# keonlee9420/Comprehensive-Transformer-TTS

Measured on AMD Instinct MI355X. Metric: mel-frames/sec (train step) LJSpeech batch=16, 1/2/4/8 MI355X, higher is better.
Workload: dtype f32; 1 GPU; LJSpeech transformer_fs2 batch=16/GPU seq<=128->mel<=1024x80; full train step fwd+loss+bwd+clip+Adam, dropout on; workload_detail=supervised durations (BASELINE configs[1]), global_batch=16, valid_frames_per_gpu=11992, padded_frames_per_gpu=16384, launch_mode=hipgraph(fwd+bwd | clip+adam), parallelism=dp1

## Files before the change

comprehensive-transformer-tts_amd/_lib.py:

```python
import ctypes as C
import os

_HERE = os.path.dirname(os.path.abspath(__file__))
LIB_PATH = os.environ.get("CTTS_LIB") or os.path.join(_HERE, "csrc", "libctts_hip.so")

_c_f32p = C.c_void_p
_i32, _i64, _f32, _u32, _vp = C.c_int32, C.c_int64, C.c_float, C.c_uint32, C.c_void_p


class GemmDesc(C.Structure):
    _fields_ = [
        ("A", _vp), ("B", _vp), ("C", _vp),
        ("M", _i32), ("N", _i32), ("K", _i32),
        ("lda", _i64), ("ldb", _i64), ("ldc", _i64),
        ("a_kc", _i32), ("b_kc", _i32),
        ("nb0", _i32), ("nb1", _i32),
        ("sA0", _i64), ("sA1", _i64), ("sB0", _i64), ("sB1", _i64), ("sC0", _i64), ("sC1", _i64),
        ("lens", _vp),
        ("lim_m", _i32), ("lim_n", _i32), ("lim_k", _i32),
        ("conv_T", _i32), ("conv_pad", _i32), ("conv_cin", _i32), ("conv_on_b", _i32),
        ("split_k", _i32),
        ("alpha", _f32),
        ("bias", _vp),
        ("Z", _vp), ("ldz", _i64),
        ("act", _i32),
        ("p_drop", _f32), ("seed", _vp), ("drop_offset", _u32),
        ("R", _vp), ("ldr", _i64),
        ("rowscale", _vp),
        ("row_lens", _vp), ("row_T", _i32), ("row_halo", _i32),
        ("tile_map", _vp),
        ("tile_group_n", _i32),
        ("E", _vp), ("rowsub", _vp),
        ("sk_ws", _vp), ("sk_ws_bytes", _i64),
        ("epi_bwd", _i32),
        ("split_out", _vp), ("split_out_floats", _i64),
        ("split_overwrite", _i32),
        ("bf16_split", _i32),
        ("A_planes", _vp),
        ("B_planes", _vp),
        ("C_planes", _vp),
    ]


class GemmRouteInfo(C.Structure):
    _fields_ = [("kind", _i32), ("tile_m", _i32), ("tile_n", _i32), ("split_k", _i32), ("k_granule", _i32)]


GEMM_KINDS = ("none", "planes", "planes_wgrad", "weight_stationary", "x6", "stream_k", "x6tn", "scalar64", "buf128", "buf_k2", "buf_narrow",
              "buf64", "vec128", "vec64")


class VconvDesc(C.Structure):
    _fields_ = [
        ("x", _vp), ("sxb", _i64), ("sxt", _i64), ("sxc", _i64),
        ("B", _i32), ("T", _i32), ("Cin", _i32), ("Cout", _i32), ("k", _i32), ("dil", _i32),
        ("transposed_u", _i32),
        ("act_in", _i32), ("slope", _f32),
        ("w", _vp), ("w_planes", _vp),
        ("bias", _vp),
        ("R", _vp),
        ("out", _vp),
        ("alpha", _f32), ("beta", _f32),
        ("bf16_split", _i32),
        ("lens", _vp), ("len_mul", _i32),
    ]


class VconvHDesc(C.Structure):
    _fields_ = [
        ("x", _vp), ("sxb", _i64), ("sxt", _i64), ("sxc", _i64),
        ("x_f32", _i32),
        ("B", _i32), ("T", _i32), ("Cin", _i32), ("Cout", _i32), ("k", _i32), ("dil", _i32),
        ("transposed_u", _i32),
        ("act_in", _i32), ("slope", _f32),
        ("w", _vp),
        ("bias", _vp),
        ("R", _vp),
        ("out", _vp),
        ("alpha", _f32), ("beta", _f32),
        ("lens", _vp), ("len_mul", _i32),
    ]


class PsumTask(C.Structure):
    _fields_ = [("src", _vp), ("dst", _vp), ("n", _i64), ("stride", _i64), ("count", _i32), ("alpha", _f32)]


class SplitTask(C.Structure):
    _fields_ = [("src", _vp), ("dst", _vp), ("rows", _i64), ("cols", _i64), ("ld", _i64)]


class RepackTask(C.Structure):
    _fields_ = [("src", _vp), ("dst", _vp), ("cout", _i32), ("cin", _i32), ("k", _i32)]


_SIGNATURES = {
    "ctts_conv_dgrad_weights": [C.POINTER(RepackTask), C.c_int, _vp],
    "ctts_gemm_split_plan": [C.POINTER(GemmDesc), C.POINTER(_i32), C.POINTER(_i64)],
    "ctts_gemm_route": [C.POINTER(GemmDesc), C.POINTER(GemmRouteInfo)],
    "ctts_partial_sums": [C.POINTER(PsumTask), C.c_int, _vp],
    "ctts_reduce_parts": [C.c_int, _i64, C.c_int],
    "ctts_xcd_probe": [_vp, C.c_int, _vp],
    "ctts_posembed_fwd": [_vp, _vp, _vp, _vp, _vp, _vp, _i64, C.c_int, _f32, _vp, _u32, _vp],
    "ctts_posembed_bwd": [_vp, _vp, _vp, _vp, _vp, _vp, _i64, C.c_int, _f32, _vp, _u32, C.c_int, _vp, _vp],
    "ctts_gemm": [C.POINTER(GemmDesc), _vp],
    "ctts_gemm_takes_persistent": [C.POINTER(GemmDesc)],
    "ctts_gemm_ws_enable": [C.c_int],
    "ctts_gemm_takes_weight_stationary": [C.POINTER(GemmDesc)],
    "ctts_gemm_takes_bf16_split": [C.POINTER(GemmDesc)],
    "ctts_gemm_takes_planes": [C.POINTER(GemmDesc)],
    "ctts_split_planes": [C.POINTER(SplitTask), C.c_int, _vp],
    "ctts_rowdot_heads": [_vp, _vp, _vp, C.c_int, C.c_int, C.c_int, C.c_int, _vp],
    "ctts_mel_prepare": [_vp, C.c_int, C.c_int, _vp, _vp],
    "ctts_mel_spectrogram": [_vp, _vp, _vp, _vp, _vp, _vp, _vp, _i64, C.c_int, C.c_int, C.c_int, C.c_int, C.c_int, _f32, C.c_int, _vp, _vp],
    "ctts_mha_fwd": [_vp, _vp, _vp, _vp, C.c_int, C.c_int, C.c_int, C.c_int, _f32, _vp],
    "ctts_mha_bwd": [_vp, _vp, _vp, _vp, _vp, _vp, _vp, _vp, _vp, C.c_int, C.c_int, C.c_int, C.c_int, _f32, C.c_int, _vp, _vp],
    "ctts_relmha_fwd": [_vp, _vp, _vp, _vp, _vp, _vp, C.c_int, C.c_int, C.c_int, C.c_int, _f32, _f32, _vp, _u32, _vp],
    "ctts_relmha_bwd": [_vp, _vp, _vp, _vp, _vp, _vp, _vp, _vp, _vp, _vp, _vp, _vp, _vp, C.c_int, C.c_int, C.c_int, C.c_int,
                        _f32, _f32, _vp, _u32, _vp],
    "ctts_weighted_colsum": [_vp, _vp, _vp, _i64, C.c_int, _f32, C.c_int, _vp, _vp, _vp],
    "ctts_epilogue_bwd": [_vp, _vp, _vp, _vp, _vp, _vp, _i64, C.c_int, C.c_int, _f32, _vp, _u32, _f32, C.c_int, _vp, _vp, _vp],
    "ctts_row_tile_map": [_vp, C.c_int, C.c_int, C.c_int, _vp, _vp],
    "ctts_conv_weight_repack": [_vp, _vp, C.c_int, C.c_int, C.c_int, C.c_int, _vp],
    "ctts_lr_index": [_vp, C.c_int, C.c_int, _vp, C.c_int, C.c_int, C.c_int, _vp, _vp, _vp, _vp],
    "ctts_lr_gather_fwd": [_vp, _vp, _vp, C.c_int, C.c_int, C.c_int, C.c_int, _vp],
    "ctts_lr_gather_bwd": [_vp, _vp, _vp, C.c_int, C.c_int, C.c_int, C.c_int, _vp],
    "ctts_embedding_fwd": [_vp, _vp, _vp, _i64, C.c_int, C.c_int, _vp],
    "ctts_embedding_bwd": [_vp, _vp, _vp, _i64, C.c_int, C.c_int, C.c_int, C.c_int, _vp, _vp],
    "ctts_positions": [_vp, C.c_int, _i64, C.c_int, C.c_int, _vp, _vp],
    "ctts_cwt_pitch": [_vp, _i64, C.c_int, _vp, _vp, _f32, _vp, C.c_int, _f32, _f32, _f32, C.c_int, _vp, _vp, _vp, C.c_int, C.c_int, C.c_int, _vp],
    "ctts_layernorm_fwd": [_vp, _vp, _vp, _vp, _vp, _vp, C.c_int, C.c_int, _f32, _f32, _vp, _u32, _vp, _vp, _vp],
    "ctts_layernorm_bwd": [_vp, _vp, _vp, _vp, _vp, _vp, _vp, _vp, C.c_int, C.c_int, _f32, _vp, _u32, _vp, C.c_int, _vp, _vp, _vp, _vp],
    "ctts_colstats": [_vp, _vp, C.c_int, C.c_int, _vp, _vp],
    "ctts_bn_finalize": [_vp, C.c_int, C.c_int, _f32, _f32, _vp, _vp, _vp, _vp, _vp, _vp],
    "ctts_bn_apply": [_vp, _vp, _vp, _vp, _vp, _vp, C.c_int, C.c_int, C.c_int, _f32, _vp, _u32, _vp, _vp],
    "ctts_bn_bwd_reduce": [_vp, _vp, _vp, _vp, _vp, _vp, _vp, C.c_int, C.c_int, C.c_int, _f32, _vp, _u32, _vp, _vp],
    "ctts_bn_bwd_apply": [_vp, _vp, _vp, _vp, _vp, _vp, _vp, _vp, _vp, _vp, C.c_int, C.c_int, C.c_int, _f32, _vp,
                          _u32, C.c_int, _vp, _vp],
    "ctts_softmax_fwd": [_vp, _vp, C.c_int, C.c_int, C.c_int, _i64, _vp],
    "ctts_softmax_bwd": [_vp, _vp, _vp, C.c_int, C.c_int, C.c_int, _i64, _vp],
    "ctts_act_dropout_bwd": [_vp, _vp, _vp, _i64, C.c_int, C.c_int, _f32, _f32, _vp, _u32, _vp],
    "ctts_rowscale_dropout": [_vp, _vp, _i64, C.c_int, _vp, _f32, _vp, _u32, _vp],
    "ctts_colsum": [_vp, _vp, _i64, C.c_int, _i64, _f32, C.c_int, _vp, _vp, _vp],
    "ctts_reflect_pad": [_vp, _vp, C.c_int, C.c_int, C.c_int, _i64, _vp],
    "ctts_stft_magnitude": [_vp, _i64, _vp, _i64, _vp, _i64, C.c_int, _vp],
    "ctts_log_clamp_transpose": [_vp, _vp, C.c_int, C.c_int, C.c_int, _f32, _vp],
    "ctts_relattn_split_fwd": [_vp, _vp, _vp, _vp, _vp, _vp, _i64, C.c_int, _vp],
    "ctts_relattn_split_bwd": [_vp, _vp, _vp, _vp, _i64, C.c_int, _vp],
    "ctts_glu_fwd": [_vp, _vp, _i64, C.c_int, _vp],
    "ctts_glu_bwd": [_vp, _vp, _vp, _i64, C.c_int, _vp],
    "ctts_dwconv_fwd": [_vp, _vp, _vp, C.c_int, C.c_int, C.c_int, C.c_int, C.c_int, _vp],
    "ctts_dwconv_wgrad": [_vp, _vp, _vp, _vp, C.c_int, C.c_int, C.c_int, C.c_int, C.c_int, _vp],
    "ctts_relpos_softmax_fwd": [_vp, _vp, _vp, C.c_int, C.c_int, _f32, _f32, _vp, _u32, _vp],
    "ctts_relpos_softmax_bwd": [_vp, _vp, C.c_int, C.c_int, _f32, _f32, _vp, _u32, _vp],
    "ctts_relshift_bwd": [_vp, _vp, C.c_int, C.c_int, _vp],
    "ctts_neg_sqdist": [_vp, _vp, _vp, C.c_int, C.c_int, C.c_int, C.c_int, _f32, _vp],
    "ctts_mas": [_vp, _vp, _vp, _vp, _vp, _vp, C.c_int, C.c_int, C.c_int, _vp],
    "ctts_forward_sum_fwd": [_vp, _vp, _vp, _f32, _vp, _vp, _vp, C.c_int, C.c_int, C.c_int, _vp],
    "ctts_forward_sum_bwd": [_vp, _vp, _vp, _f32, _vp, _vp, _vp, _vp, _vp, C.c_int, C.c_int, C.c_int, _vp],
    "ctts_var_loss_fwd": [_vp] * 2 + [C.c_int] + [_vp] * 12 + [C.c_int] * 3 + [_vp, C.c_int, _vp] + [_vp] * 4 + [_vp],
    "ctts_var_loss_bwd": [_vp] * 2 + [C.c_int] + [_vp] * 12 + [C.c_int] * 3 + [_vp, C.c_int, _vp] + [_vp] * 4 + [_vp] * 5 + [_vp],
    "ctts_bin_loss_fwd": [_vp, _vp, _i64, _vp, _vp, _vp],
    "ctts_bin_loss_bwd": [_vp, _vp, _vp, _vp, _vp, _i64, _vp],
    "ctts_masked_loss_fwd": [_vp, _vp, _vp, _i64, _i32, _vp, _vp, _vp],
    "ctts_masked_loss_bwd": [_vp, _vp, _vp, _vp, _vp, _vp, _i64, _i32, _vp],
    "ctts_mel_l1_fwd": [_vp, _vp, _vp, _vp, _vp, _vp, _i64, C.c_int, _vp, _vp],
    "ctts_mel_l1_bwd": [_vp, _vp, _vp, _vp, _vp, _vp, _vp, _vp, _i64, C.c_int, _vp],
    "ctts_adam_clip_step": [_vp, _vp, _vp, _vp, C.c_int64, _vp, _f32, _f32, _f32, _f32, _f32, _vp, _vp],
    "ctts_im2col_3x3s2": [_vp, _vp, C.c_int, C.c_int, C.c_int, C.c_int, _vp],
    "ctts_col2im_3x3s2": [_vp, _vp, C.c_int, C.c_int, C.c_int, C.c_int, _vp],
    "ctts_gru_fwd": [_vp, _vp, _vp, _vp, _vp, C.c_int, C.c_int, C.c_int, C.c_int, C.c_int, _vp],
    "ctts_gru_bwd": [_vp, _vp, _vp, _vp, _vp, _vp, _vp, C.c_int, C.c_int, C.c_int, C.c_int, C.c_int, _vp],
    "ctts_softmax_rect_fwd": [_vp, _vp, _vp, C.c_int, C.c_int, C.c_int, _vp],
    "ctts_softmax_rect_bwd": [_vp, _vp, _vp, _vp, C.c_int, C.c_int, C.c_int, _vp],
    "ctts_vocoder_conv": [C.POINTER(VconvDesc), _vp],
    "ctts_vocoder_post": [_vp, C.c_int, C.c_int, C.c_int, C.c_int, _vp, _vp, _f32, _vp, _vp],
    "ctts_vocoder_post_ragged": [_vp, C.c_int, C.c_int, C.c_int, C.c_int, _vp, _vp, _f32, _vp, _vp, C.c_int, _vp],
    "ctts_vocoder_conv_h": [C.POINTER(VconvHDesc), _vp],
    "ctts_vocoder_post_h": [_vp, C.c_int, C.c_int, C.c_int, C.c_int, _vp, _vp, _f32, _vp, _vp, C.c_int, _vp],
    "ctts_fastformer_pool_fwd": [_vp, _i64, _vp, _i64, _vp, _vp, _vp, _vp, C.c_int, C.c_int, C.c_int, C.c_int, _f32, _vp],
    "ctts_fastformer_pool_bwd": [_vp, _vp, _vp, _vp, _i64, _vp, _i64, _vp, _vp, _vp, _vp, C.c_int, C.c_int, C.c_int, C.c_int, _f32, _vp],
    "ctts_fastformer_bcast": [_vp, _i64, _vp, _vp, C.c_int, C.c_int, C.c_int, _vp],
    "ctts_fastformer_bcast_bwd": [_vp, _vp, _vp, _i64, _vp, _vp, _vp, _vp, _vp, C.c_int, C.c_int, C.c_int, _vp],
    "ctts_fastformer_resdrop": [_vp, _vp, _vp, _vp, _i64, C.c_int, _vp, _f32, _vp, _u32, C.c_int, _vp],
    "ctts_griffinlim_prepare": [_vp, C.c_int, C.c_int, _vp, _vp],
    "ctts_stft_transform": [_vp, _vp, _vp, _vp, _vp, _i64, _i64, _i64, C.c_int, C.c_int, C.c_int, C.c_int, _vp],
    "ctts_istft_frames": [_vp, _vp, _i64, _i64, _i64, _vp, _vp, _vp, _vp, C.c_int, C.c_int, C.c_int, C.c_int, _vp],
    "ctts_griffinlim_iter": [_vp, _vp, _vp, _vp, _vp, C.c_int, C.c_int, C.c_int, C.c_int, _vp],
    "ctts_istft_ola": [_vp, _vp, _vp, _vp, _i64, C.c_int, C.c_int, C.c_int, C.c_int, _vp],
    "ctts_griffinlim_iter_momentum": [_vp, _vp, _vp, _vp, _vp, _vp, _f32, C.c_int, C.c_int, C.c_int, C.c_int, C.c_int, _vp],
    "ctts_istft_frames_seeded": [_vp, _i64, _i64, _i64, _vp, _vp, _vp, _vp, _vp, C.c_int, C.c_int, C.c_int, C.c_int, _vp],
    "ctts_pitch_track_prepare": [_vp, _vp],
    "ctts_pitch_track": [_vp, _vp, _vp, _vp, _vp, _vp, C.c_int, C.c_int, C.c_int, C.c_int, _f32, _f32, _f32, _f32, _vp],
    "ctts_f0_targets": [_vp, _vp, _vp, _vp, _vp, _vp, _vp, C.c_int, C.c_int, _vp],
    "ctts_norm_interp_f0": [_vp, _vp, _vp, _vp, C.c_int, C.c_int, _f32, _vp],
    "ctts_trim_silence": [_vp, _vp, _vp, _vp, _vp, C.c_int, C.c_int, _f32, C.c_int, C.c_int, _vp],
    "ctts_attn_prior": [_vp, _vp, _vp, C.c_int, C.c_int, C.c_int, _i64, _i64, _f32, _vp],
    "ctts_outlier_stats": [_vp, _vp, _vp, _vp, _vp, _vp, _vp, _vp, C.c_int, C.c_int, _vp],
    "ctts_mel_cepstrum": [_vp, _vp, _vp, C.c_int, C.c_int, C.c_int, C.c_int, _vp],
    "ctts_dtw": [_vp, _vp, _vp, _vp, _vp, _vp, _vp, _vp, C.c_int, C.c_int, C.c_int, C.c_int, C.c_int, _vp],
    "ctts_path_metrics": [_vp, _vp, _vp, _vp, _vp, C.c_int, C.c_int, C.c_int, C.c_int, _vp],
    "ctts_resample": [_vp, _vp, _vp, _vp, _vp, C.c_int, C.c_int, C.c_int, C.c_int, C.c_int, C.c_int, _vp],
    "ctts_peak_normalize": [_vp, _vp, _vp, _vp, _vp, _vp, C.c_int, C.c_int, _f32, _vp],
    "ctts_resample_tile": [C.c_int, C.c_int, C.c_int, C.c_int],
    "ctts_loudness_chunk": [],
    "ctts_loudness_tile_slots": [],
    "ctts_loudness_coef_doubles": [],
    "ctts_loudness_max_segments": [],
    "ctts_kweight_energy": [_vp, _vp, _vp, _vp, _vp, _vp, _vp, C.c_int, C.c_int, C.c_int, C.c_int, _vp, _vp],
    "ctts_loudness_gate": [_vp, _vp, _vp, _vp, _vp, _vp, _vp, _vp, _vp, _vp, _vp, C.c_int, C.c_int, C.c_int, C.c_int, C.c_int, C.c_double,
                           C.c_double, C.c_int, _vp],
    "ctts_apply_gain": [_vp, _vp, _vp, _vp, C.c_int, C.c_int, _vp],
    "ctts_stoi_max_frames": [],
    "ctts_stoi": [_vp, _vp, _vp, _vp, _vp, _vp, _vp, C.c_int, C.c_int, _vp, _vp],
    "ctts_si_sdr": [_vp, _vp, _vp, _vp, C.c_int, C.c_int, _vp, _vp],
    "ctts_mr_stft": [_vp, _vp, _vp, _vp, _vp, _vp, C.c_int, C.c_int, C.c_int, C.c_int, C.c_int, _vp, _vp],
    "ctts_comm_unique_id": [_vp],
    "ctts_comm_create": [C.POINTER(_vp), _i32, _i32, _vp],
    "ctts_comm_destroy": [_vp],
    "ctts_allreduce_mean": [_vp, _i64, _vp, _vp],
}
COMM_ID_BYTES = 128
EXPORTED_SYMBOLS = sorted(list(_SIGNATURES) + ["ctts_last_error", "ctts_version", "ctts_mha_supported", "ctts_relmha_workspace_floats",
                                               "ctts_mel_spectrogram_workspace_bytes", "ctts_gemm_workspace_bytes", "ctts_workspace_bytes",
                                               "ctts_workspace_error_word", "ctts_fastformer_workspace_floats",
                                               "ctts_griffinlim_workspace_bytes", "ctts_griffinlim_state_floats",
                                               "ctts_pitch_track_workspace_bytes", "ctts_trim_silence_workspace_bytes",
                                               "ctts_dtw_workspace_bytes", "ctts_loudness_workspace_bytes", "ctts_stoi_workspace_bytes",
                                               "ctts_si_sdr_workspace_bytes", "ctts_mr_stft_workspace_bytes"])
ADAM_STATE_FLOATS = 3 + 2048
ABI_VERSION = 2

_lib = None


class CttsError(RuntimeError):
    pass


def load():
    global _lib
    if _lib is not None:
        return _lib
    if not os.path.exists(LIB_PATH):
        raise CttsError(
            f"{LIB_PATH} not found - build it with comprehensive-transformer-tts_amd/csrc/build.sh "
            "(or __graft_entry__.build()).  There is no CPU / PyTorch fallback for the hot path."
        )
    lib = C.CDLL(LIB_PATH)
    lib.ctts_version.restype = C.c_int
    lib.ctts_version.argtypes = []
    if lib.ctts_version() != ABI_VERSION:
        raise CttsError(f"{LIB_PATH} has ABI version {lib.ctts_version()}, this package needs {ABI_VERSION} - rebuild it with "
                        "comprehensive-transformer-tts_amd/csrc/build.sh (or __graft_entry__.build())")
    for name, argtypes in _SIGNATURES.items():
        fn = getattr(lib, name)
        fn.argtypes = argtypes
        fn.restype = C.c_int
# ... 43 lines not shown
```

comprehensive-transformer-tts_amd/csrc/elementwise.hip:

```cpp
#include "ctts_common.h"

namespace {
__global__ void zero_u32_kernel(uint32_t* __restrict__ p, size_t n) {
  for (size_t i = (size_t)blockIdx.x * blockDim.x + threadIdx.x; i < n; i += (size_t)gridDim.x * blockDim.x) p[i] = 0u;
}
}

int ctts_zero_async(void* p, size_t bytes, hipStream_t st) {
  if (bytes == 0) return 0;
  const size_t n = (bytes + 3) / 4;
  const unsigned blocks = (unsigned)((n + 255) / 256 > 2048 ? 2048 : (n + 255) / 256);
  hipLaunchKernelGGL(zero_u32_kernel, dim3(blocks), dim3(256), 0, st, (uint32_t*)p, n);
  return hipGetLastError() == hipSuccess ? 0 : -1;
}

namespace {

__global__ void act_dropout_bwd_kernel(const float* __restrict__ dg, const float* __restrict__ z, float* __restrict__ dz,
                                       long total, int act, float p_drop, const uint64_t* seed, uint32_t drop_offset) {
  const bool do_drop = p_drop > 0.f;
  uint32_t dkey = 0; float inv_keep = 1.f;
  if (do_drop) { dkey = ctts_drop_key(seed, drop_offset); inv_keep = 1.f / (1.f - p_drop); }
  if (total & 3) {
    for (long i = (long)blockIdx.x * blockDim.x + threadIdx.x; i < total; i += (long)gridDim.x * blockDim.x) {
      float g = dg[i];
      if (do_drop) g *= ctts_drop_scale(dkey, (uint32_t)i, p_drop, inv_keep);
      dz[i] = g * ctts_act_grad(z[i], act);
    }
    return;
  }
  const long n4 = total >> 2;
  for (long i = (long)blockIdx.x * blockDim.x + threadIdx.x; i < n4; i += (long)gridDim.x * blockDim.x) {
    const float4 g = reinterpret_cast<const float4*>(dg)[i];
    const float4 zz = reinterpret_cast<const float4*>(z)[i];
    float ga[4] = {g.x, g.y, g.z, g.w};
    const float za[4] = {zz.x, zz.y, zz.z, zz.w};
#pragma unroll
    for (int e = 0; e < 4; ++e) {
      if (do_drop) ga[e] *= ctts_drop_scale(dkey, (uint32_t)(i * 4 + e), p_drop, inv_keep);
      ga[e] *= ctts_act_grad(za[e], act);
    }
    reinterpret_cast<float4*>(dz)[i] = make_float4(ga[0], ga[1], ga[2], ga[3]);
  }
}

__global__ void rowscale_dropout_kernel(const float* __restrict__ x, float* __restrict__ y, long total, int C,
                                        const float* __restrict__ rowscale, float p_drop, const uint64_t* seed,
                                        uint32_t drop_offset) {
  const bool do_drop = p_drop > 0.f;
  uint32_t dkey = 0; float inv_keep = 1.f;
  if (do_drop) { dkey = ctts_drop_key(seed, drop_offset); inv_keep = 1.f / (1.f - p_drop); }
  if (C & 3) {
    for (long i = (long)blockIdx.x * blockDim.x + threadIdx.x; i < total; i += (long)gridDim.x * blockDim.x) {
      float a = x[i];
      if (do_drop) a *= ctts_drop_scale(dkey, (uint32_t)i, p_drop, inv_keep);
      y[i] = a * (rowscale ? rowscale[i / C] : 1.f);
    }
    return;
  }
  const long n4 = total >> 2;
  const int C4 = C >> 2;
  for (long i = (long)blockIdx.x * blockDim.x + threadIdx.x; i < n4; i += (long)gridDim.x * blockDim.x) {
    const float4 v = reinterpret_cast<const float4*>(x)[i];
    float a[4] = {v.x, v.y, v.z, v.w};
    const float sc = rowscale ? rowscale[i / C4] : 1.f;
#pragma unroll
    for (int e = 0; e < 4; ++e) {
      if (do_drop) a[e] *= ctts_drop_scale(dkey, (uint32_t)(i * 4 + e), p_drop, inv_keep);
      a[e] *= sc;
    }
    reinterpret_cast<float4*>(y)[i] = make_float4(a[0], a[1], a[2], a[3]);
  }
}

__device__ __forceinline__ void ctts_colsum_emit(float tot, float* s64, float* __restrict__ out, int c, int C, int creal, float scale,
                                                 int accumulate) {
  const int ty = threadIdx.x >> 6, l = threadIdx.x & 63;
  if (C != creal) {
    __syncthreads();
    if (ty == 0) s64[l] = c < C ? tot : 0.f;
    __syncthreads();
    if (ty == 0 && l < creal) {
      float a = 0.f;
      for (int j = l; j < C; j += creal) a += s64[j];
      out[l] = accumulate ? out[l] + scale * a : scale * a;
    }
    return;
  }
  if (ty == 0 && c < C) out[c] = accumulate ? out[c] + scale * tot : scale * tot;
}

__global__ __launch_bounds__(256) void colsum_kernel(const float* __restrict__ x, float* __restrict__ out, long rows, int C,
                                                      int creal, long ld, float scale, unsigned char* ws, int G, int accumulate,
                                                      float* __restrict__ parts) {
  __shared__ float s[4][64];
  const int c = blockIdx.x * 64 + (threadIdx.x & 63), ty = threadIdx.x >> 6;
  const long stripe = (rows + gridDim.y - 1) / gridDim.y;
  const long r0 = blockIdx.y * stripe, r1 = min(rows, r0 + stripe);
  float a = 0.f;
  if (c < C) {
#pragma unroll 4
    for (long r = r0 + ty; r < r1; r += 4) a += x[r * ld + c];
  }
  s[ty][threadIdx.x & 63] = a;
  __syncthreads();
  float tot[1] = {0.f};
  if (ty == 0) { const int l = threadIdx.x; tot[0] = s[0][l] + s[1][l] + s[2][l] + s[3][l]; }
  if (parts) {
    if (ty == 0 && c < C) parts[(long)blockIdx.y * C + c] = tot[0];
    return;
  }
  if (!ctts_ordered_colsum<float, 1>(tot, ws, blockIdx.x, blockIdx.y, gridDim.y, G)) return;
  ctts_colsum_emit(tot[0], s[0], out, c, C, creal, scale, accumulate);
}

__global__ __launch_bounds__(256) void epilogue_bwd_kernel(const float* __restrict__ dy, const float* __restrict__ rowscale,
                                                            const float* __restrict__ z, float* __restrict__ dz, float* __restrict__ gm,
                                                            float* __restrict__ dbias, long rows, int C, int act, float p_drop,
                                                            const uint64_t* seed, uint32_t drop_offset, float bias_scale,
                                                            unsigned char* ws, int G, int accumulate, float* __restrict__ parts) {
  __shared__ float s[4][64];
  const int c = blockIdx.x * 64 + (threadIdx.x & 63), ty = threadIdx.x >> 6;
  const long stripe = (rows + gridDim.y - 1) / gridDim.y;
  const long r0 = blockIdx.y * stripe, r1 = min(rows, r0 + stripe);
  const bool do_drop = p_drop > 0.f;
  uint32_t dkey = 0; float inv_keep = 1.f;
  if (do_drop) { dkey = ctts_drop_key(seed, drop_offset); inv_keep = 1.f / (1.f - p_drop); }
  float a = 0.f;
  if (c < C) {
#pragma unroll 4
    for (long r = r0 + ty; r < r1; r += 4) {
      const long e = r * C + c;
      float g = dy[e];
      if (rowscale) g *= rowscale[r];
      if (gm) gm[e] = g;
      if (do_drop) g *= ctts_drop_scale(dkey, (uint32_t)e, p_drop, inv_keep);
      if (z) g *= ctts_act_grad(z[e], act);
      dz[e] = g;
      a += g;
    }
  }
  if (!dbias && !parts) return;
  s[ty][threadIdx.x & 63] = a;
  __syncthreads();
  float tot[1] = {0.f};
  if (ty == 0) { const int l = threadIdx.x; tot[0] = s[0][l] + s[1][l] + s[2][l] + s[3][l]; }
  if (parts) {
    if (ty == 0 && c < C) parts[(long)blockIdx.y * C + c] = tot[0];
    return;
  }
  if (!ctts_ordered_colsum<float, 1>(tot, ws, blockIdx.x, blockIdx.y, gridDim.y, G)) return;
  ctts_colsum_emit(tot[0], s[0], dbias, c, C, C, bias_scale, accumulate);
}

__global__ void conv_weight_repack_kernel(const float* __restrict__ src, float* __restrict__ dst, int cout, int cin, int k,
                                          int mode, long total) {
  for (long e = (long)blockIdx.x * blockDim.x + threadIdx.x; e < total; e += (long)gridDim.x * blockDim.x) {
    if (mode == 0) {
      const int ci = (int)(e % cin); const long t = e / cin; const int kk = (int)(t % k); const int co = (int)(t / k);
      dst[e] = src[((long)co * cin + ci) * k + kk];
    } else if (mode == 1) {
      const int co = (int)(e % cout); const long t = e / cout; const int kk = (int)(t % k); const int ci = (int)(t / k);
      dst[e] = src[((long)co * cin + ci) * k + (k - 1 - kk)];
    } else if (mode == 4) {
      const int co = (int)(e % cout); const long t = e / cout; const int kk = (int)(t % k); const int ci = (int)(t / k);
      dst[e] = src[((long)co * k + (k - 1 - kk)) * cin + ci];
    } else {
      const int kk = (int)(e % k); const long t = e / k; const int ci = (int)(t % cin); const int co = (int)(t / cin);
      const float v = src[((long)co * k + kk) * cin + ci];
      dst[e] = mode == 3 ? dst[e] + v : v;
    }
  }
}

__global__ void reflect_pad_kernel(const float* __restrict__ y, float* __restrict__ ypad, int N, int pad, long ld_out,
                                   long total) {
  const int W = N + 2 * pad;
  for (long e = (long)blockIdx.x * blockDim.x + threadIdx.x; e < total; e += (long)gridDim.x * blockDim.x) {
    const long b = e / ld_out;
    const int j = (int)(e - b * ld_out);
    float v = 0.f;
    if (j < W) {
      int i = j - pad;
      if (i < 0) i = -i;
      if (i >= N) i = 2 * (N - 1) - i;
      v = y[b * N + i];
    }
    ypad[e] = v;
  }
}

__global__ __launch_bounds__(256) void stft_magnitude_kernel(const float* __restrict__ reim, long ld_reim,
                                                              float* __restrict__ mag, long ld_mag,
                                                              float* __restrict__ energy, long frames, int nbins) {
  const int lane = threadIdx.x & 63, wave = threadIdx.x >> 6;
  for (long f = (long)blockIdx.x * 4 + wave; f < frames; f += (long)gridDim.x * 4) {
    const float* r = reim + f * ld_reim;
    float acc = 0.f;
    for (int k = lane; k < ld_mag; k += 64) {
      float m = 0.f;
      if (k < nbins) {
        const float re = r[k], im = r[nbins + k];
        const float p = re * re + im * im;
        acc += p;
        m = sqrtf(p);
      }
      mag[f * ld_mag + k] = m;
    }
    acc = ctts_wave_sum(acc);
    if (lane == 0) energy[f] = sqrtf(acc);
  }
}

__global__ void log_clamp_transpose_kernel(const float* __restrict__ in, float* __restrict__ out, int F, int n_mel,
                                           float clip, long total) {
  for (long e = (long)blockIdx.x * blockDim.x + threadIdx.x; e < total; e += (long)gridDim.x * blockDim.x) {
    const int f = (int)(e % F); const long t = e / F; const int m = (int)(t % n_mel); const long b = t / n_mel;
    out[e] = logf(fmaxf(in[(b * F + f) * n_mel + m], clip));
  }
}

inline int grid_for(long n, int cap = 4096) { return (int)min((n + 255) / 256, (long)cap); }

}

extern "C" int ctts_act_dropout_bwd(const float* dg, const float* z, float* dz, int64_t rows, int C, int act,
                                    float alpha_unused, float p_drop, const uint64_t* seed, uint32_t drop_offset,
                                    void* stream) {
  (void)alpha_unused;
  CTTS_REQUIRE(dg && z && dz && C > 0, "ctts_act_dropout_bwd: bad arguments");
  const long total = (long)rows * C;
  if (total == 0) return 0;
  hipLaunchKernelGGL(act_dropout_bwd_kernel, dim3(grid_for((total & 3) ? total : (total >> 2))), dim3(256), 0, (hipStream_t)stream, dg, z, dz, total,
                     act, p_drop, seed, drop_offset);
  CTTS_CHECK_LAUNCH("ctts_act_dropout_bwd");
  return 0;
}

extern "C" int ctts_rowscale_dropout(const float* x, float* y, int64_t rows, int C, const float* rowscale, float p_drop,
                                     const uint64_t* seed, uint32_t drop_offset, void* stream) {
  CTTS_REQUIRE(x && y && C > 0, "ctts_rowscale_dropout: bad arguments");
  const long total = (long)rows * C;
  if (total == 0) return 0;
  hipLaunchKernelGGL(rowscale_dropout_kernel, dim3(grid_for((C & 3) ? total : (total >> 2))), dim3(256), 0, (hipStream_t)stream, x, y, total, C,
                     rowscale, p_drop, seed, drop_offset);
  CTTS_CHECK_LAUNCH("ctts_rowscale_dropout");
  return 0;
}

namespace {
__global__ __launch_bounds__(256) void weighted_colsum_kernel(const float* __restrict__ x, const float* __restrict__ w,
                                                               float* __restrict__ out, long rows, int C, float scale,
                                                               unsigned char* ws, int G, int accumulate, float* __restrict__ parts) {
  __shared__ float s[4][64];
  const int c = blockIdx.x * 64 + (threadIdx.x & 63), ty = threadIdx.x >> 6;
  const long stripe = (rows + gridDim.y - 1) / gridDim.y;
  const long r0 = blockIdx.y * stripe, r1 = min(rows, r0 + stripe);
  float a = 0.f;
  if (c < C) {
#pragma unroll 4
    for (long r = r0 + ty; r < r1; r += 4) a = fmaf(w[r], x[r * C + c], a);
  }
  s[ty][threadIdx.x & 63] = a;
  __syncthreads();
  float tot[1] = {0.f};
  if (ty == 0) { const int l = threadIdx.x; tot[0] = s[0][l] + s[1][l] + s[2][l] + s[3][l]; }
  if (parts) {
    if (ty == 0 && c < C) parts[(long)blockIdx.y * C + c] = tot[0];
    return;
  }
  if (!ctts_ordered_colsum<float, 1>(tot, ws, blockIdx.x, blockIdx.y, gridDim.y, G)) return;
  ctts_colsum_emit(tot[0], s[0], out, c, C, C, scale, accumulate);
}
}

static int colsum_stripes(int gx, long want, bool have_ws) {
  if (!have_ws) return 1;
  const long cap = (long)(CTTS_WS_RED_P1_BYTES / (64 * sizeof(float))) / gx;
  return (int)max((long)1, min(want, min(cap, (long)CTTS_RED_MAX_GROUPS * 64)));
}

int ctts_layernorm_bwd_blocks(int rows, int C);

extern "C" int ctts_reduce_parts(int kind, int64_t rows, int C) {
  if (rows <= 0 || C <= 0) return 0;
  const int gx = (C + 63) / 64;
  if (gx > CTTS_RED_MAX_COLBLOCKS) return 0;
  switch (kind) {
    case 0: if (C * 2 <= 64 && rows % 2 == 0) return 0;
            return colsum_stripes(gx, min((long)max(1, 1024 / gx), (long)rows / 64), true);
    case 1: return colsum_stripes(gx, min((long)max(1, 1024 / gx), (long)rows / 64), true);
    case 2: return colsum_stripes(gx, min((long)max(1, 2048 / gx), (long)rows / 32), true);
    case 3: return ctts_layernorm_bwd_blocks((int)rows, C);
    default: return 0;
  }
}

extern "C" int ctts_weighted_colsum(const float* x, const float* w, float* out, int64_t rows, int C, float scale, int accumulate,
                                    void* ws, float* parts, void* stream) {
  CTTS_REQUIRE(x && w && (out || parts) && C > 0 && (C + 63) / 64 <= CTTS_RED_MAX_COLBLOCKS, "ctts_weighted_colsum: bad arguments");
  CTTS_REQUIRE(!parts || rows > 0, "ctts_weighted_colsum: deferred mode needs rows > 0");
  hipStream_t st = (hipStream_t)stream;
  if (rows == 0) {
    if (!accumulate && ctts_zero_async(out, sizeof(float) * C, st) != 0) { ctts_set_error("ctts_weighted_colsum: zero fill failed"); return -2; }
    return 0;
  }
  const int gx = (C + 63) / 64;
  const int gy = colsum_stripes(gx, min((long)max(1, 1024 / gx), (long)rows / 64), ws != nullptr || parts != nullptr);
  hipLaunchKernelGGL(weighted_colsum_kernel, dim3(gx, gy), dim3(256), 0, st, x, w, out, (long)rows, C, scale, (unsigned char*)ws,
                     ctts_red_group(gy), accumulate, parts);
  CTTS_CHECK_LAUNCH("ctts_weighted_colsum");
  return 0;
}

extern "C" int ctts_colsum(const float* x, float* out, int64_t rows, int C, int64_t ld, float scale, int accumulate, void* ws,
                           float* parts, void* stream) {
  CTTS_REQUIRE(x && (out || parts) && C > 0 && (C + 63) / 64 <= CTTS_RED_MAX_COLBLOCKS, "ctts_colsum: bad arguments");
  CTTS_REQUIRE(!parts || ctts_reduce_parts(0, rows, C) > 0, "ctts_colsum: this shape has no deferred mode (ctts_reduce_parts = 0)");
  hipStream_t st = (hipStream_t)stream;
  if (rows == 0) {
    if (!accumulate && ctts_zero_async(out, sizeof(float) * C, st) != 0) { ctts_set_error("ctts_colsum: zero fill failed"); return -2; }
    return 0;
  }
  int k = 1;
  if (ld == C && !parts)
    while (C * k * 2 <= 64 && rows % (k * 2) == 0) k *= 2;
  const int Cv = C * k, gx = (Cv + 63) / 64;
  const long Rv = rows / k;
  const int gy = colsum_stripes(gx, min((long)max(1, 1024 / gx), Rv / 64), ws != nullptr || parts != nullptr);
  hipLaunchKernelGGL(colsum_kernel, dim3(gx, gy), dim3(256), 0, st, x, out, Rv, Cv, C, (long)ld * k, scale, (unsigned char*)ws,
                     ctts_red_group(gy), accumulate, parts);
  CTTS_CHECK_LAUNCH("ctts_colsum");
  return 0;
}

extern "C" int ctts_epilogue_bwd(const float* dy, const float* rowscale, const float* z, float* dz, float* gm, float* dbias,
                                 int64_t rows, int C, int act, float p_drop, const uint64_t* seed, uint32_t drop_offset, float bias_scale,
                                 int accumulate_bias, void* ws, float* parts, void* stream) {
  CTTS_REQUIRE(dy && dz && rows >= 0 && C > 0 && p_drop >= 0.f && p_drop < 1.f && (p_drop == 0.f || seed), "ctts_epilogue_bwd: bad arguments");
  CTTS_REQUIRE(!dbias || (C + 63) / 64 <= CTTS_RED_MAX_COLBLOCKS, "ctts_epilogue_bwd: C too large for the bias-gradient reduction");
  hipStream_t st = (hipStream_t)stream;
  if (rows == 0) {
    if (dbias && !accumulate_bias && ctts_zero_async(dbias, sizeof(float) * C, st) != 0) { ctts_set_error("ctts_epilogue_bwd: zero fill failed"); return -2; }
    return 0;
  }
  const int gx = (C + 63) / 64;
  const long want = min((long)max(1, 2048 / gx), (long)rows / 32);
  CTTS_REQUIRE(!parts || rows > 0, "ctts_epilogue_bwd: deferred bias gradient needs rows > 0");
  const int gy = (dbias || parts) ? colsum_stripes(gx, want, ws != nullptr || parts != nullptr) : (int)max((long)1, want);
  hipLaunchKernelGGL(epilogue_bwd_kernel, dim3(gx, gy), dim3(256), 0, st, dy, rowscale, act ? z : nullptr, dz, gm, dbias, (long)rows, C, act,
                     p_drop, seed, drop_offset, bias_scale, (unsigned char*)ws, ctts_red_group(gy), accumulate_bias, parts);
  CTTS_CHECK_LAUNCH("ctts_epilogue_bwd");
  return 0;
}

extern "C" int ctts_conv_weight_repack(const float* src, float* dst, int cout, int cin, int k, int mode, void* stream) {
  CTTS_REQUIRE(src && dst && mode >= 0 && mode <= 4, "ctts_conv_weight_repack: bad arguments");
  const long total = (long)cout * cin * k;
  if (total == 0) return 0;
  hipLaunchKernelGGL(conv_weight_repack_kernel, dim3(grid_for(total)), dim3(256), 0, (hipStream_t)stream, src, dst, cout, cin, k,
                     mode, total);
  CTTS_CHECK_LAUNCH("ctts_conv_weight_repack");
  return 0;
}

extern "C" int ctts_reflect_pad(const float* y, float* ypad, int B, int N, int pad, int64_t ld_out, void* stream) {
  CTTS_REQUIRE(y && ypad && N > pad && ld_out >= N + 2 * pad, "ctts_reflect_pad: need N > pad and ld_out >= N + 2*pad");
  const long total = (long)B * ld_out;
  if (total == 0) return 0;
  hipLaunchKernelGGL(reflect_pad_kernel, dim3(grid_for(total)), dim3(256), 0, (hipStream_t)stream, y, ypad, N, pad, (long)ld_out, total);
  CTTS_CHECK_LAUNCH("ctts_reflect_pad");
  return 0;
}

extern "C" int ctts_stft_magnitude(const float* reim, int64_t ld_reim, float* mag, int64_t ld_mag, float* energy,
                                   int64_t frames, int nbins, void* stream) {
  CTTS_REQUIRE(reim && mag && energy && ld_mag >= nbins, "ctts_stft_magnitude: bad arguments");
  if (frames == 0) return 0;
  const int blocks = (int)min((frames + 3) / 4, (int64_t)4096);
  hipLaunchKernelGGL(stft_magnitude_kernel, dim3(blocks), dim3(256), 0, (hipStream_t)stream, reim, (long)ld_reim, mag,
                     (long)ld_mag, energy, (long)frames, nbins);
  CTTS_CHECK_LAUNCH("ctts_stft_magnitude");
  return 0;
}

extern "C" int ctts_log_clamp_transpose(const float* mel_fm, float* out, int B, int F, int n_mel, float clip, void* stream) {
  CTTS_REQUIRE(mel_fm && out, "ctts_log_clamp_transpose: null pointer");
  const long total = (long)B * F * n_mel;
  if (total == 0) return 0;
  hipLaunchKernelGGL(log_clamp_transpose_kernel, dim3(grid_for(total)), dim3(256), 0, (hipStream_t)stream, mel_fm, out, F, n_mel,
                     clip, total);
  CTTS_CHECK_LAUNCH("ctts_log_clamp_transpose");
  return 0;
}


namespace {
constexpr int RPK_BATCH = 32;
struct RepackBatch {
  const float* src[RPK_BATCH];
  float* dst[RPK_BATCH];
  int cout[RPK_BATCH], cin[RPK_BATCH], k[RPK_BATCH];
  int first_block[RPK_BATCH + 1];
  int ntasks;
};

__global__ __launch_bounds__(256) void conv_dgrad_weights_kernel(const RepackBatch b) {
  __shared__ float tile[32][33];
  int t = 0;
  while (t + 1 < b.ntasks && (int)blockIdx.x >= b.first_block[t + 1]) ++t;
  const float* __restrict__ src = b.src[t];
  float* __restrict__ dst = b.dst[t];
  const int cout = b.cout[t], cin = b.cin[t], k = b.k[t];
  const int tco = (cout + 31) / 32, tci = (cin + 31) / 32;
  int blk = (int)blockIdx.x - b.first_block[t];
  const int kk = blk / (tco * tci);
  blk -= kk * tco * tci;
  const int co0 = (blk / tci) * 32, ci0 = (blk % tci) * 32;
  const int tx = threadIdx.x & 31, ty = threadIdx.x >> 5;
#pragma unroll
  for (int r = ty; r < 32; r += 8) {
    const int co = co0 + r, ci = ci0 + tx;
    tile[r][tx] = (co < cout && ci < cin) ? src[((long)co * k + (k - 1 - kk)) * cin + ci] : 0.f;
  }
  __syncthreads();
#pragma unroll
  for (int r = ty; r < 32; r += 8) {
    const int ci = ci0 + r, co = co0 + tx;
    if (ci < cin && co < cout) dst[((long)ci * k + kk) * cout + co] = tile[tx][r];
  }
}
}

extern "C" int ctts_conv_dgrad_weights(const ctts_repack_task* tasks, int ntasks, void* stream) {
  CTTS_REQUIRE(ntasks >= 0 && (tasks || ntasks == 0), "ctts_conv_dgrad_weights: bad arguments");
  hipStream_t st = (hipStream_t)stream;
  for (int t0 = 0; t0 < ntasks; t0 += RPK_BATCH) {
    RepackBatch b;
    b.ntasks = 0;
    int blocks = 0;
    for (int t = t0; t < ntasks && t < t0 + RPK_BATCH; ++t) {
      const ctts_repack_task& q = tasks[t];
      CTTS_REQUIRE(q.src && q.dst && q.cout > 0 && q.cin > 0 && q.k > 0, "ctts_conv_dgrad_weights: bad task %d", t);
      const int i = b.ntasks++;
      b.src[i] = q.src; b.dst[i] = q.dst; b.cout[i] = q.cout; b.cin[i] = q.cin; b.k[i] = q.k;
      b.first_block[i] = blocks;
      blocks += ((q.cout + 31) / 32) * ((q.cin + 31) / 32) * q.k;
    }
    if (b.ntasks == 0) continue;
    b.first_block[b.ntasks] = blocks;
    hipLaunchKernelGGL(conv_dgrad_weights_kernel, dim3(blocks), dim3(256), 0, st, b);
    CTTS_CHECK_LAUNCH("ctts_conv_dgrad_weights");
  }
  return 0;
}

namespace {
__global__ __launch_bounds__(256) void posembed_fwd_kernel(const float4* __restrict__ x, const int32_t* __restrict__ pos, const float4* __restrict__ table,
                                                            const float* __restrict__ alpha, const float* __restrict__ rowscale, float4* __restrict__ y,
                                                            long n4, int C4, float p_drop, const uint64_t* seed, uint32_t drop_offset) {
#pragma clang fp contract(off)
  const bool do_drop = p_drop > 0.f;
  uint32_t dkey = 0; float inv_keep = 1.f;
  if (do_drop) { dkey = ctts_drop_key(seed, drop_offset); inv_keep = 1.f / (1.f - p_drop); }
  const float a = alpha ? alpha[0] : 1.f;
  for (long i = (long)blockIdx.x * blockDim.x + threadIdx.x; i < n4; i += (long)gridDim.x * blockDim.x) {
    const long row = i / C4;
    const int c = (int)(i - row * C4);
    const float4 xv = x[i], tv = table[(long)pos[row] * C4 + c];
    float v[4] = {xv.x + a * tv.x, xv.y + a * tv.y, xv.z + a * tv.z, xv.w + a * tv.w};
    const float sc = rowscale ? rowscale[row] : 1.f;
#pragma unroll
    for (int e = 0; e < 4; ++e) {
      if (do_drop) v[e] *= ctts_drop_scale(dkey, (uint32_t)(i * 4 + e), p_drop, inv_keep);
      v[e] *= sc;
    }
    y[i] = make_float4(v[0], v[1], v[2], v[3]);
  }
}

__global__ __launch_bounds__(256) void posembed_bwd_kernel(const float4* __restrict__ dy, const int32_t* __restrict__ pos, const float4* __restrict__ table,
                                                            const float* __restrict__ rowscale, float4* __restrict__ dx, float* __restrict__ dalpha,
                                                            long n4, int C4, float p_drop, const uint64_t* seed, uint32_t drop_offset,
                                                            unsigned char* ws, int G, int accumulate) {
  __shared__ float s_w[4];
  const bool do_drop = p_drop > 0.f;
  uint32_t dkey = 0; float inv_keep = 1.f;
  if (do_drop) { dkey = ctts_drop_key(seed, drop_offset); inv_keep = 1.f / (1.f - p_drop); }
// ... 139 lines not shown
```

comprehensive-transformer-tts_amd/csrc/gemm.hip:

```cpp
#include "ctts_common.h"
#include "gemm_common.h"
#include <stdlib.h>
#include <type_traits>

namespace {

#ifndef CTTS_BK
#define CTTS_BK 32
#endif
#ifndef CTTS_GEMM_WAVES
#define CTTS_GEMM_WAVES 2
#endif
constexpr int BK = CTTS_BK;
constexpr int KC_LD = BK + 4;
constexpr int KCH = BK / 4;
static_assert(BK == 32 || BK == 64, "BK must be 32 or 64");


__device__ __forceinline__ bool rows_in_padding(const int32_t* row_lens, int row_T, int row_halo, int first, int last) {
  const int b0 = first / row_T;
  return b0 == last / row_T && (first - b0 * row_T) >= row_lens[b0] + row_halo;
}

__device__ __forceinline__ void batch_limits(const ctts_gemm_desc& d, int z0, bool apply, int& Mv, int& Nv, int& Kv) {
  Mv = d.M; Nv = d.N; Kv = d.K;
  if (apply && d.lens) {
    const int L = d.lens[z0];
    if (d.lim_m) Mv = min(Mv, L);
    if (d.lim_n) Nv = min(Nv, L);
    if (d.lim_k) Kv = min(Kv, L);
  }
}

__device__ __forceinline__ bool split_k_range(const ctts_gemm_desc& d, int Kv, int granule, int split, int& k_begin, int& k_end) {
  k_begin = 0; k_end = Kv;
  if (d.split_k > 1) {
    const GemmSplitRange s = gemm_split_range(Kv, d.split_k, granule, split);
    k_begin = s.k_begin; k_end = s.k_end;
    if (k_begin >= k_end) return false;
  }
  return true;
}

__device__ __forceinline__ void xcd_tile_order(int nwg, int tiles_n, bool scramble, int& wg, int& tm) {
  const int q8 = nwg >> 3, r8 = nwg & 7, xcd = blockIdx.x & 7, slot = blockIdx.x >> 3;
  wg = (xcd < r8 ? xcd * (q8 + 1) : r8 * (q8 + 1) + (xcd - r8) * q8) + slot;
  const int tiles_m = nwg / tiles_n;
  tm = wg / tiles_n;
  if (scramble) {
    const int P = (tiles_m % 37) ? 37 : ((tiles_m % 41) ? 41 : 43);
    tm = (int)(((long)tm * P) % tiles_m);
  }
}

__device__ __forceinline__ bool natural_order(const ctts_gemm_desc& d) { return d.tile_map == reinterpret_cast<const int32_t*>(1); }

__device__ __forceinline__ void zero_tile(const ctts_gemm_desc& d, float* C, int row0, int col0, int nrows, int ncols) {
  for (int e = threadIdx.x; e < nrows * ncols; e += 256) {
    const int r = e / ncols, c = e - r * ncols;
    C[(long)(row0 + r) * d.ldc + col0 + c] = 0.f;
    if (d.Z && !d.epi_bwd) d.Z[(long)(row0 + r) * d.ldz + col0 + c] = 0.f;
  }
}

__device__ __forceinline__ bool padded_tile_zeroed(const ctts_gemm_desc& d, float* C, int row0, int col0, int BM, int ncols, int Mv) {
  const int last = min(row0 + BM, Mv) - 1;
  if (!rows_in_padding(d.row_lens, d.row_T, d.row_halo, row0, last)) return false;
  zero_tile(d, C, row0, col0, last - row0 + 1, ncols);
  return true;
}

__device__ __forceinline__ void zero_outside_limits(const ctts_gemm_desc& d, float* C, int row0, int col0, int BM, int BN, int Mv, int Nv,
                                                    bool whole) {
  const int nrows = min(BM, d.M - row0), ncols = min(BN, d.N - col0);
  for (int e = threadIdx.x; e < nrows * ncols; e += 256) {
    const int r = e / ncols, c = e - r * ncols;
    if (whole || row0 + r >= Mv || col0 + c >= Nv) C[(long)(row0 + r) * d.ldc + col0 + c] = 0.f;
  }
}

struct ConvView {
  int T, pad, cin;
};

template <int ROWS, bool CONV>
struct LoaderKC {
  static constexpr int NV = ROWS * BK / 4 / 256;
  const float* base;
  long ld;
  int row0, row_lim, kq, tid;
  ConvView cv;
  int trow[NV];
  __device__ __forceinline__ void init(const float* p, long ld_, int row0_, int row_lim_, ConvView cv_, int tid_) {
    base = CONV ? p - (long)cv_.pad * cv_.cin : p;
    ld = ld_; row0 = row0_; row_lim = row_lim_; cv = cv_; tid = tid_;
    kq = (tid % KCH) << 2;
    if (CONV) {
#pragma unroll
      for (int i = 0; i < NV; ++i) {
        int gr = row0 + ((tid + i * 256) / KCH);
        trow[i] = gr % cv.T;
      }
    }
  }
  __device__ __forceinline__ void load(int k0, int k_end, float4 (&r)[NV]) const {
    const int gk = k0 + kq;
#pragma unroll
    for (int i = 0; i < NV; ++i) {
      const int gr = row0 + ((tid + i * 256) / KCH);
      float4 v = make_float4(0.f, 0.f, 0.f, 0.f);
      if (gr < row_lim && gk < k_end) {
        const float* p = base + (long)gr * ld + gk;
        float e[4] = {0.f, 0.f, 0.f, 0.f};
#pragma unroll
        for (int q = 0; q < 4; ++q) {
          bool okq = (gk + q < k_end);
          if (CONV && okq) { int tt = trow[i] + (gk + q) / cv.cin - cv.pad; okq = (tt >= 0) && (tt < cv.T); }
          if (okq) e[q] = p[q];
        }
        v = make_float4(e[0], e[1], e[2], e[3]);
      }
      r[i] = v;
    }
  }
  __device__ __forceinline__ void store(float* s, const float4 (&r)[NV]) const {
#pragma unroll
    for (int i = 0; i < NV; ++i) {
      const int row = (tid + i * 256) / KCH;
      *reinterpret_cast<float4*>(s + row * KC_LD + kq) = r[i];
    }
  }
};

template <int COLS, bool CONV>
struct LoaderRC {
  static constexpr int NV = COLS * BK / 4 / 256;
  static constexpr int LD = COLS + 4;
  const float* base;
  long ld;
  int col0, col_lim, tid;
  ConvView cv;
  __device__ __forceinline__ void init(const float* p, long ld_, int col0_, int col_lim_, ConvView cv_, int tid_) {
    base = CONV ? p - (long)cv_.pad * cv_.cin : p;
    ld = ld_; col0 = col0_; col_lim = col_lim_; cv = cv_; tid = tid_;
  }
  __device__ __forceinline__ void load(int k0, int k_end, float4 (&r)[NV]) const {
#pragma unroll
    for (int i = 0; i < NV; ++i) {
      const int f = tid + i * 256;
      const int k = f / (COLS / 4);
      const int cq = (f % (COLS / 4)) << 2;
      const int gk = k0 + k, gc = col0 + cq;
      float4 v = make_float4(0.f, 0.f, 0.f, 0.f);
      if (gk < k_end && gc < col_lim) {
        const float* p = base + (long)gk * ld + gc;
        int trow = 0;
        if (CONV) trow = gk % cv.T;
        float e[4] = {0.f, 0.f, 0.f, 0.f};
#pragma unroll
        for (int q = 0; q < 4; ++q) {
          bool okq = (gc + q < col_lim);
          if (CONV && okq) { int tt = trow + (gc + q) / cv.cin - cv.pad; okq = (tt >= 0) && (tt < cv.T); }
          if (okq) e[q] = p[q];
        }
        v = make_float4(e[0], e[1], e[2], e[3]);
      }
      r[i] = v;
    }
  }
  __device__ __forceinline__ void store(float* s, const float4 (&r)[NV]) const {
#pragma unroll
    for (int i = 0; i < NV; ++i) {
      const int f = tid + i * 256;
      const int k = f / (COLS / 4);
      const int cq = (f % (COLS / 4)) << 2;
      *reinterpret_cast<float4*>(s + k * LD + cq) = r[i];
    }
  }
};


__device__ __forceinline__ float4 mask4(float4 v, int nv) {
  v.x = nv > 0 ? v.x : 0.f; v.y = nv > 1 ? v.y : 0.f; v.z = nv > 2 ? v.z : 0.f; v.w = nv > 3 ? v.w : 0.f;
  return v;
}

template <int ROWS, bool CONV>
struct VLoaderKC {
  static constexpr int NV = ROWS * BK / 4 / 256;
  const float* base; const float* safe;
  long ld;
  int row0, row_lim, kq, tid;
  ConvView cv;
  int trow[NV];
  int nval[NV];
  __device__ __forceinline__ void init(const float* p, long ld_, int row0_, int row_lim_, ConvView cv_, int tid_) {
    safe = p;
    base = CONV ? p - (long)cv_.pad * cv_.cin : p;
// ... 62 lines not shown
    }
  }
  __device__ __forceinline__ void store(float* s, const float4 (&r)[NV]) const {
#pragma unroll
    for (int i = 0; i < NV; ++i) {
      const int f = tid + i * 256;
      const int k = f / (COLS / 4);
      const int cq = (f % (COLS / 4)) << 2;
      *reinterpret_cast<float4*>(s + k * LD + cq) = mask4(r[i], nval[i]);
    }
  }
};

typedef unsigned int ctts_u32x4 __attribute__((ext_vector_type(4)));
constexpr unsigned CTTS_OOB = 0x80000000u;

__device__ __forceinline__ float4 buf_load16(__amdgpu_buffer_rsrc_t rsrc, unsigned off) {
  ctts_u32x4 v = __builtin_amdgcn_raw_buffer_load_b128(rsrc, off, 0, 0);
  return *reinterpret_cast<float4*>(&v);
}

template <int ROWS, bool CONV, bool PARTIAL>
struct BLoaderKC {
  static constexpr int NV = ROWS * BK / 4 / 256;
  __amdgpu_buffer_rsrc_t rsrc;
  unsigned boff[NV];
  int trow[NV];
  int kq, tid, T, cin, pad;
  int nk_cur;
  __device__ __forceinline__ void init(const float* p, long ld, int row0, int row_lim, ConvView cv, int tid_) {
    rsrc = __builtin_amdgcn_make_buffer_rsrc((void*)p, 0, 0x7FFFFFFE, 0x00020000);
    tid = tid_; T = cv.T; cin = cv.cin; pad = cv.pad;
    kq = (tid % KCH) << 2;
#pragma unroll
    for (int i = 0; i < NV; ++i) {
      const int gr = row0 + ((tid + i * 256) / KCH);
      const long e = (long)(CONV ? gr - cv.pad : gr) * ld + kq;
      boff[i] = gr < row_lim ? (unsigned)(e * 4) : CTTS_OOB;
      trow[i] = CONV ? gr % cv.T : 0;
    }
    nk_cur = 4;
  }
  __device__ __forceinline__ void load(int k0, int k_end, float4 (&r)[NV]) {
    const int gk = k0 + kq;
    const bool kok = gk < k_end;
    if (PARTIAL) nk_cur = min(4, k_end - gk);
    const unsigned koff = (unsigned)k0 * 4u;
    int tap = 0;
    if (CONV) tap = gk / cin - pad;
#pragma unroll
    for (int i = 0; i < NV; ++i) {
      bool ok = kok && (boff[i] != CTTS_OOB);
      if (CONV) ok = ok && ((unsigned)(trow[i] + tap) < (unsigned)T);
      const unsigned off = ok ? boff[i] + koff : CTTS_OOB;
      r[i] = buf_load16(rsrc, off);
    }
  }
  __device__ __forceinline__ void store(float* s, const float4 (&r)[NV]) const {
#pragma unroll
    for (int i = 0; i < NV; ++i) {
      const int row = (tid + i * 256) / KCH;
      *reinterpret_cast<float4*>(s + row * KC_LD + kq) = PARTIAL ? mask4(r[i], nk_cur) : r[i];
    }
  }
};

template <int COLS, bool CONV, bool PARTIAL>
struct BLoaderRC {
  static constexpr int NV = COLS * BK / 4 / 256;
  static constexpr int LD = COLS + 4;
  __amdgpu_buffer_rsrc_t rsrc;
  unsigned boff[NV];
  int ctap[NV];
  unsigned ldb4;
  int tid, T;
  int ncol[NV];
  __device__ __forceinline__ void init(const float* p, long ld, int col0, int col_lim, ConvView cv, int tid_) {
    rsrc = __builtin_amdgcn_make_buffer_rsrc((void*)p, 0, 0x7FFFFFFE, 0x00020000);
    tid = tid_; T = cv.T; ldb4 = (unsigned)(ld * 4);
#pragma unroll
    for (int i = 0; i < NV; ++i) {
      const int f = tid + i * 256;
      const int k = f / (COLS / 4);
      const int gc = col0 + ((f % (COLS / 4)) << 2);
      const long e = (long)(CONV ? k - cv.pad : k) * ld + gc;
      boff[i] = gc < col_lim ? (unsigned)(e * 4) : CTTS_OOB;
      ctap[i] = CONV ? gc / cv.cin - cv.pad : 0;
      ncol[i] = PARTIAL ? min(4, col_lim - gc) : 4;
    }
  }
  __device__ __forceinline__ void load(int k0, int k_end, float4 (&r)[NV]) const {
    const unsigned k0off = (unsigned)k0 * ldb4;
#pragma unroll
    for (int i = 0; i < NV; ++i) {
      const int gk = k0 + (tid + i * 256) / (COLS / 4);
      unsigned off = boff[i] + k0off;
      bool ok = (boff[i] != CTTS_OOB) && (gk < k_end);
      if (CONV) ok = ok && ((unsigned)(gk % T + ctap[i]) < (unsigned)T);
      r[i] = buf_load16(rsrc, ok ? off : CTTS_OOB);
    }
  }
  __device__ __forceinline__ void store(float* s, const float4 (&r)[NV]) const {
#pragma unroll
    for (int i = 0; i < NV; ++i) {
      const int f = tid + i * 256;
      *reinterpret_cast<float4*>(s + (f / (COLS / 4)) * LD + ((f % (COLS / 4)) << 2)) = PARTIAL ? mask4(r[i], ncol[i]) : r[i];
    }
  }
};

enum class Fetch {
  Scalar,
  Vec,
  Buffer,
  BufferPartial,
};

template <Fetch F>
struct FetchTraits {
  static constexpr bool kBuffer = F == Fetch::Buffer || F == Fetch::BufferPartial;
  static constexpr bool kLensLimits = F != Fetch::Buffer;
  static constexpr bool kLensGiven = F == Fetch::BufferPartial;
  static constexpr bool kTileOrders = kBuffer;
  static constexpr bool kNaturalOrder = F == Fetch::BufferPartial;
  static constexpr bool kTrustSchedule = kTileOrders;
  static constexpr bool kMaskAtStore = F == Fetch::Vec || F == Fetch::BufferPartial;
  static constexpr bool kPadFillOwnSplit = kBuffer;
};

template <Fetch F, bool KC, int EXT, bool CONV>
using Loader = std::conditional_t<
    FetchTraits<F>::kBuffer,
    std::conditional_t<KC, BLoaderKC<EXT, CONV, FetchTraits<F>::kMaskAtStore>, BLoaderRC<EXT, CONV, FetchTraits<F>::kMaskAtStore>>,
    std::conditional_t<F == Fetch::Vec, std::conditional_t<KC, VLoaderKC<EXT, CONV>, VLoaderRC<EXT, CONV>>,
                       std::conditional_t<KC, LoaderKC<EXT, CONV>, LoaderRC<EXT, CONV>>>>;

template <bool KC, int LD>
__device__ __forceinline__ void fetch_frag(const float* s, int ext0, int l31, int h, int ksub, float (&f)[16]) {
  if (KC) {
    const float4* p = reinterpret_cast<const float4*>(s + (ext0 + l31) * LD + ksub + h * 16);
#pragma unroll
    for (int q = 0; q < 4; ++q) {
      float4 v = p[q];
      f[4 * q + 0] = v.x; f[4 * q + 1] = v.y; f[4 * q + 2] = v.z; f[4 * q + 3] = v.w;
    }
  } else {
    const float* p = s + (ksub + h * 16) * LD + ext0 + l31;
#pragma unroll
    for (int j = 0; j < 16; ++j) f[j] = p[j * LD];
  }
}

template <int BM, int BN, bool A_KC, bool B_KC, bool CONV, Fetch FETCH>
__global__ __launch_bounds__(256, CTTS_GEMM_WAVES) void gemm_tile_kernel(const ctts_gemm_desc d) {
  using FT = FetchTraits<FETCH>;
  constexpr int WAVES_N = BN >= 64 ? 2 : 1, WAVES_M = 4 / WAVES_N;
  constexpr int WM = BM / WAVES_M, WN = BN / WAVES_N, MT = WM / 32, NT = WN / 32;
  constexpr int A_LD = A_KC ? KC_LD : BM + 4;
  constexpr int B_LD = B_KC ? KC_LD : BN + 4;
  constexpr int A_SZ = A_KC ? BM * KC_LD : BK * (BM + 4);
  constexpr int B_SZ = B_KC ? BN * KC_LD : BK * (BN + 4);
  __shared__ __attribute__((aligned(16))) float smem[A_SZ + B_SZ];
  float* sA = smem;
  float* sB = smem + A_SZ;
  const int z = blockIdx.z;
  const int split = blockIdx.y;
  const int z0 = z / d.nb1, z1 = z - z0 * d.nb1;
  const bool limited = FT::kLensLimits && (FT::kLensGiven || d.lens);
  int Mv, Nv, Kv;
  batch_limits(d, z0, limited, Mv, Nv, Kv);
  const int tiles_n = (d.N + BN - 1) / BN;
  int wg, tm;
  bool scheduled_active = false;
  if (FT::kTileOrders && BM == 64 && A_KC && d.tile_map && !natural_order(d)) {
    wg = blockIdx.x;
    int r = wg / tiles_n;
    if (d.tile_group_n > 0) {
      const int g = d.tile_group_n, ngroups = tiles_n / g, mways = 8 / ngroups;
      const int x = blockIdx.x & 7, i = blockIdx.x >> 3;
      r = (i / g) * mways + x / ngroups;
      wg = r * tiles_n + (x % ngroups) * g + i % g;
    }
    tm = d.tile_map[1 + r];
    scheduled_active = FT::kTrustSchedule && r < d.tile_map[0];
  } else if (FT::kNaturalOrder || (FT::kTileOrders && natural_order(d))) {
    wg = blockIdx.x;
    tm = wg / tiles_n;
  } else {
    xcd_tile_order(gridDim.x, tiles_n, true, wg, tm);
  }
  const int row0 = tm * BM, col0 = (wg % tiles_n) * BN;
  float* Cb = d.C + z0 * d.sC0 + z1 * d.sC1;
  const bool zero_outside = limited && d.split_overwrite && d.split_k <= 1;
  if (row0 >= Mv || col0 >= Nv) {
    if (zero_outside && row0 < d.M && col0 < d.N) zero_outside_limits(d, Cb, row0, col0, BM, BN, Mv, Nv, true);
    return;
  }
  if (zero_outside && (row0 + BM > Mv || col0 + BN > Nv)) zero_outside_limits(d, Cb, row0, col0, BM, BN, Mv, Nv, false);
  float* Cs = Cb;
  if (d.split_k > 1) Cs += (long)split * d.M * d.ldc;
  if (A_KC && d.row_lens && !scheduled_active &&
      padded_tile_zeroed(d, FT::kPadFillOwnSplit ? Cs : Cb, row0, col0, BM, min(BN, Nv - col0), Mv)) return;
  int k_begin, k_end;
  if (!split_k_range(d, Kv, BK, split, k_begin, k_end)) return;

  ConvView cv{d.conv_T, d.conv_pad, d.conv_cin};
  ConvView nocv{1, 0, 1};
  constexpr bool CONV_A = CONV && A_KC;
  constexpr bool CONV_B = CONV && !A_KC && !B_KC;
  using LA = Loader<FETCH, A_KC, BM, CONV_A>;
  using LB = Loader<FETCH, B_KC, BN, CONV_B>;
  LA la; LB lb;
  la.init(d.A + z0 * d.sA0 + z1 * d.sA1, d.lda, row0, Mv, CONV_A ? cv : nocv, threadIdx.x);
  lb.init(d.B + z0 * d.sB0 + z1 * d.sB1, d.ldb, col0, Nv, CONV_B ? cv : nocv, threadIdx.x);

  const int lane = threadIdx.x & 63, wave = threadIdx.x >> 6;
  const int l31 = lane & 31, h = lane >> 5;
  const int wm0 = (wave / WAVES_N) * WM, wn0 = (wave % WAVES_N) * WN;
  floatx16 acc[MT][NT];
#pragma unroll
  for (int i = 0; i < MT; ++i)
#pragma unroll
    for (int j = 0; j < NT; ++j)
#pragma unroll
      for (int r = 0; r < 16; ++r) acc[i][j][r] = 0.f;

  constexpr bool KSKIP = !A_KC && !B_KC;
  auto kblock_active = [&](int k0) -> bool {
    if (!KSKIP || !d.row_lens) return true;
    return !rows_in_padding(d.row_lens, d.row_T, d.row_halo, k0, min(k0 + BK, k_end) - 1);
  };
  float4 ra[LA::NV], rb[LB::NV];
  bool act_cur = kblock_active(k_begin);
  if (act_cur) {
    la.load(k_begin, k_end, ra);
    lb.load(k_begin, k_end, rb);
    la.store(sA, ra);
    lb.store(sB, rb);
  }
  __syncthreads();
  for (int k0 = k_begin; k0 < k_end; k0 += BK) {
    const bool has_next = (k0 + BK) < k_end;
    const bool act_next = has_next && kblock_active(k0 + BK);
    if (act_next) {
      la.load(k0 + BK, k_end, ra);
      lb.load(k0 + BK, k_end, rb);
    }
    if (act_cur) {
#pragma unroll
      for (int ksub = 0; ksub < BK; ksub += 32) {
        float fa[MT][16], fb[NT][16];
#pragma unroll
        for (int i = 0; i < MT; ++i) fetch_frag<A_KC, A_LD>(sA, wm0 + i * 32, l31, h, ksub, fa[i]);
#pragma unroll
        for (int j = 0; j < NT; ++j) fetch_frag<B_KC, B_LD>(sB, wn0 + j * 32, l31, h, ksub, fb[j]);
#ifdef CTTS_GEMM_SETPRIO
        __builtin_amdgcn_s_setprio(CTTS_GEMM_SETPRIO);
#endif
#pragma unroll
        for (int kk = 0; kk < 16; ++kk)
#pragma unroll
          for (int i = 0; i < MT; ++i)
#pragma unroll
            for (int j = 0; j < NT; ++j)
              acc[i][j] = __builtin_amdgcn_mfma_f32_32x32x2f32(fa[i][kk], fb[j][kk], acc[i][j], 0, 0, 0);
#ifdef CTTS_GEMM_SETPRIO
        __builtin_amdgcn_s_setprio(0);
#endif
      }
    }
    if (KSKIP && !act_cur && !act_next) continue;
    __syncthreads();
    if (act_next) {
      la.store(sA, ra);
      lb.store(sB, rb);
    }
    __syncthreads();
    act_cur = act_next;
  }
  gemm_epilogue_auto<MT, NT>(d, acc, Cs, z, row0, col0, wm0, wn0, l31, h, Mv, Nv);
}

constexpr int X6_PROW = 64, X6_PLANE = 128 * X6_PROW;
__device__ __forceinline__ int x6_chunk(int row, int c) { return c ^ ((row >> 2) & 3); }
typedef __bf16 x6_bf16x8 __attribute__((ext_vector_type(8)));

typedef __bf16 x6_bf16x2 __attribute__((ext_vector_type(2)));
typedef float x6_floatx2 __attribute__((ext_vector_type(2)));
__device__ __forceinline__ unsigned x6_round_pair(float& a, float& b) {
  const x6_floatx2 v = {a, b};
  const unsigned p = __builtin_bit_cast(unsigned, __builtin_convertvector(v, x6_bf16x2));
  a -= __uint_as_float(p << 16);
  b -= __uint_as_float(p & 0xFFFF0000u);
  return p;
}

__device__ __forceinline__ void x6_split_store(const float4 v, unsigned char* base) {
  float x0 = v.x, x1 = v.y, x2 = v.z, x3 = v.w;
  uint2 hi, mid, lo;
  hi.x = x6_round_pair(x0, x1);  hi.y = x6_round_pair(x2, x3);
  mid.x = x6_round_pair(x0, x1); mid.y = x6_round_pair(x2, x3);
  lo.x = x6_round_pair(x0, x1);  lo.y = x6_round_pair(x2, x3);
  *reinterpret_cast<uint2*>(base) = hi;
  *reinterpret_cast<uint2*>(base + X6_PLANE) = mid;
  *reinterpret_cast<uint2*>(base + 2 * X6_PLANE) = lo;
}

__device__ __forceinline__ floatx16 x6_mma(const ctts_u32x4 a, const ctts_u32x4 b, const floatx16 c) {
  return __builtin_amdgcn_mfma_f32_32x32x16_bf16(__builtin_bit_cast(x6_bf16x8, a), __builtin_bit_cast(x6_bf16x8, b), c, 0, 0, 0);
}

template <bool CONV>
__global__ __launch_bounds__(256, 2) void gemm_x6_kernel(const ctts_gemm_desc d) {
  static_assert(BK == 32, "the bf16 planes hold 32-deep K-blocks");
  constexpr int BM = 128, BN = 128, MT = 2, NT = 2;
  __shared__ __attribute__((aligned(16))) unsigned char smem[6 * X6_PLANE];
  const int Mv = d.M, Nv = d.N, Kv = d.K;
  const int tiles_n = d.N / BN;
  int wg, tm;
  if (natural_order(d)) {
    wg = blockIdx.x; tm = wg / tiles_n;
  } else {
    xcd_tile_order(gridDim.x, tiles_n, true, wg, tm);
  }
  const int row0 = tm * BM, col0 = (wg % tiles_n) * BN;
  float* Cb = d.C;
  if (d.row_lens && padded_tile_zeroed(d, Cb, row0, col0, BM, BN, Mv)) return;
  const bool pad_hi = d.row_lens && row0 + 64 < Mv && rows_in_padding(d.row_lens, d.row_T, d.row_halo, row0 + 64, min(row0 + BM, Mv) - 1);
  ConvView cv{d.conv_T, d.conv_pad, d.conv_cin};
  ConvView nocv{1, 0, 1};
  Loader<Fetch::Buffer, true, BM, CONV> la;
  Loader<Fetch::Buffer, true, BN, false> lb;
  la.init(d.A, d.lda, row0, Mv, CONV ? cv : nocv, threadIdx.x);
  lb.init(d.B, d.ldb, col0, Nv, nocv, threadIdx.x);
  const int lane = threadIdx.x & 63, wave = threadIdx.x >> 6;
  const int l31 = lane & 31, h = lane >> 5;
  const int wm0 = (wave >> 1) * 64, wn0 = (wave & 1) * 64;
  floatx16 acc[MT][NT];
#pragma unroll
  for (int i = 0; i < MT; ++i)
#pragma unroll
    for (int j = 0; j < NT; ++j)
#pragma unroll
      for (int r = 0; r < 16; ++r) acc[i][j][r] = 0.f;
  float4 ra[4], rb[4];
  const int srow = threadIdx.x >> 3, sc8 = threadIdx.x & 7;
  unsigned char* st_a = smem + srow * X6_PROW + x6_chunk(srow, sc8 >> 1) * 16 + (sc8 & 1) * 8;
  unsigned char* st_b = st_a + 3 * X6_PLANE;
  const unsigned char* fr_a = smem + (wm0 + l31) * X6_PROW;
  const unsigned char* fr_b = smem + 3 * X6_PLANE + (wn0 + l31) * X6_PROW;
  const int fc0 = x6_chunk(l31, h) * 16, fc1 = x6_chunk(l31, 2 + h) * 16;
  la.load(0, Kv, ra);
  lb.load(0, Kv, rb);
#pragma unroll
  for (int i = 0; i < 4; ++i) { x6_split_store(ra[i], st_a + 32 * i * X6_PROW); x6_split_store(rb[i], st_b + 32 * i * X6_PROW); }
  __syncthreads();
  for (int k0 = 0; k0 < Kv; k0 += BK) {
    {
      const int kn = k0 + BK < Kv ? k0 + BK : k0;
      la.load(kn, Kv, ra);
      lb.load(kn, Kv, rb);
    }
    ctts_u32x4 fa[2][MT][3], fb[2][NT][3];
#pragma unroll
    for (int ks = 0; ks < 2; ++ks) {
#pragma unroll
      for (int i = 0; i < MT; ++i)
#pragma unroll
        for (int p = 0; p < 3; ++p) fa[ks][i][p] = *reinterpret_cast<const ctts_u32x4*>(fr_a + p * X6_PLANE + 32 * i * X6_PROW + (ks ? fc1 : fc0));
#pragma unroll
      for (int j = 0; j < NT; ++j)
#pragma unroll
        for (int p = 0; p < 3; ++p) fb[ks][j][p] = *reinterpret_cast<const ctts_u32x4*>(fr_b + p * X6_PLANE + 32 * j * X6_PROW + (ks ? fc1 : fc0));
    }
#pragma unroll
    for (int ks = 0; ks < 2; ++ks)
#pragma unroll
      for (int t = 0; t < 6; ++t) {
        constexpr int PA[6] = {2, 0, 1, 1, 0, 0}, PB[6] = {0, 2, 1, 0, 1, 0};
#pragma unroll
        for (int i = 0; i < MT; ++i)
#pragma unroll
          for (int j = 0; j < NT; ++j) acc[i][j] = x6_mma(fa[ks][i][PA[t]], fb[ks][j][PB[t]], acc[i][j]);
      }
    __syncthreads();
#pragma unroll
    for (int i = 0; i < 4; ++i) { x6_split_store(ra[i], st_a + 32 * i * X6_PROW); x6_split_store(rb[i], st_b + 32 * i * X6_PROW); }
    __syncthreads();
  }
  if (pad_hi && wm0 == 64) {
    const int nrows = min(row0 + BM, Mv) - (row0 + 64);
    for (int e = lane; e < nrows * 64; e += 64) {
      const int r = e >> 6, c = e & 63;
      Cb[(long)(row0 + 64 + r) * d.ldc + col0 + wn0 + c] = 0.f;
      if (d.Z && !d.epi_bwd) d.Z[(long)(row0 + 64 + r) * d.ldz + col0 + wn0 + c] = 0.f;
    }
    return;
  }
  gemm_epilogue_auto<MT, NT>(d, acc, Cb, 0, row0, col0, wm0, wn0, l31, h, Mv, Nv);
}

template <bool CONV>
__global__ __launch_bounds__(256, 2) void gemm_x6tn_kernel(const ctts_gemm_desc d) {
  static_assert(BK == 32, "the bf16 planes hold 32-deep K-blocks");
  constexpr int BM = 128, BN = 128, MT = 2, NT = 2;
  __shared__ __attribute__((aligned(16))) unsigned char smem[6 * X6_PLANE];
  const int Mv = d.M, Nv = d.N, Kv = d.K;
  const int tiles_n = d.N / BN, split = blockIdx.y;
  int wg, tm;
  xcd_tile_order(gridDim.x, tiles_n, false, wg, tm);
  const int row0 = tm * BM, col0 = (wg % tiles_n) * BN;
  float* Cb = d.C;
  if (d.split_k > 1) Cb += (long)split * d.M * d.ldc;
  int k_begin, k_end;
  if (!split_k_range(d, Kv, BK, split, k_begin, k_end)) return;
  auto kblock_active = [&](int k0) -> bool {
    return !d.row_lens || !rows_in_padding(d.row_lens, d.row_T, d.row_halo, k0, min(k0 + BK, k_end) - 1);
  };
  auto next_active = [&](int k0) -> int { while (k0 < k_end && !kblock_active(k0)) k0 += BK; return k0; };
  const __amdgpu_buffer_rsrc_t ra_src = __builtin_amdgcn_make_buffer_rsrc((void*)d.A, 0, 0x7FFFFFFE, 0x00020000);
  const __amdgpu_buffer_rsrc_t rb_src = __builtin_amdgcn_make_buffer_rsrc((void*)d.B, 0, 0x7FFFFFFE, 0x00020000);
  const int lane = threadIdx.x & 63, wave = threadIdx.x >> 6;
  const int l31 = lane & 31, h = lane >> 5;
  const int wm0 = (wave >> 1) * 64, wn0 = (wave & 1) * 64;
  const int scol = threadIdx.x & 127, og = threadIdx.x >> 7;
  const unsigned a_col = (unsigned)(row0 + scol) * 4u, b_col = (unsigned)(col0 + scol) * 4u;
  const unsigned lda4 = (unsigned)(d.lda * 4), ldb4 = (unsigned)(d.ldb * 4);
  const int tapb = CONV ? (col0 + scol) / d.conv_cin - d.conv_pad : 0;
  floatx16 acc[MT][NT];
#pragma unroll
  for (int i = 0; i < MT; ++i)
#pragma unroll
    for (int j = 0; j < NT; ++j)
#pragma unroll
      for (int r = 0; r < 16; ++r) acc[i][j][r] = 0.f;
  float va[2][8], vb[2][8];
  auto gload = [&](int k0) {
#pragma unroll
    for (int o = 0; o < 2; ++o) {
      const int kk0 = k0 + (og + 2 * o) * 8;
      const int t0 = CONV ? kk0 % d.conv_T + tapb : 0;
#pragma unroll
      for (int j = 0; j < 8; ++j) {
        const int k = kk0 + j;
        const bool ok = k < k_end;
        const unsigned offa = ok ? (unsigned)k * lda4 + a_col : CTTS_OOB;
        bool okb = ok;
        if (CONV) okb = okb && ((unsigned)(t0 + j) < (unsigned)d.conv_T);
        const unsigned offb = okb ? (unsigned)(CONV ? k - d.conv_pad : k) * ldb4 + b_col : CTTS_OOB;
        va[o][j] = __builtin_bit_cast(float, __builtin_amdgcn_raw_buffer_load_b32(ra_src, offa, 0, 0));
        vb[o][j] = __builtin_bit_cast(float, __builtin_amdgcn_raw_buffer_load_b32(rb_src, offb, 0, 0));
      }
    }
  };
  auto split_store8 = [&](const float (&xin)[8], unsigned char* base) {
    float x[8];
#pragma unroll
    for (int i = 0; i < 8; ++i) x[i] = xin[i];
    ctts_u32x4 hi, mid, lo;
#pragma unroll
    for (int q = 0; q < 4; ++q) hi[q] = x6_round_pair(x[2 * q], x[2 * q + 1]);
#pragma unroll
    for (int q = 0; q < 4; ++q) mid[q] = x6_round_pair(x[2 * q], x[2 * q + 1]);
#pragma unroll
    for (int q = 0; q < 4; ++q) lo[q] = x6_round_pair(x[2 * q], x[2 * q + 1]);
    *reinterpret_cast<ctts_u32x4*>(base) = hi;
    *reinterpret_cast<ctts_u32x4*>(base + X6_PLANE) = mid;
    *reinterpret_cast<ctts_u32x4*>(base + 2 * X6_PLANE) = lo;
  };
  auto lstore = [&]() {
#pragma unroll
    for (int o = 0; o < 2; ++o) {
      unsigned char* pa = smem + scol * X6_PROW + x6_chunk(scol, og + 2 * o) * 16;
      split_store8(va[o], pa);
      split_store8(vb[o], pa + 3 * X6_PLANE);
    }
  };
  const unsigned char* fr_a = smem + (wm0 + l31) * X6_PROW;
  const unsigned char* fr_b = smem + 3 * X6_PLANE + (wn0 + l31) * X6_PROW;
  const int fc0 = x6_chunk(l31, h) * 16, fc1 = x6_chunk(l31, 2 + h) * 16;
  int k_cur = next_active(k_begin);
  if (k_cur < k_end) {
    gload(k_cur);
    lstore();
  }
  __syncthreads();
  while (k_cur < k_end) {
    const int k_nxt = next_active(k_cur + BK);
    gload(k_nxt < k_end ? k_nxt : k_cur);
    ctts_u32x4 fa[2][MT][3], fb[2][NT][3];
#pragma unroll
    for (int ks = 0; ks < 2; ++ks) {
#pragma unroll
      for (int i = 0; i < MT; ++i)
#pragma unroll
        for (int p = 0; p < 3; ++p) fa[ks][i][p] = *reinterpret_cast<const ctts_u32x4*>(fr_a + p * X6_PLANE + 32 * i * X6_PROW + (ks ? fc1 : fc0));
#pragma unroll
      for (int j = 0; j < NT; ++j)
#pragma unroll
        for (int p = 0; p < 3; ++p) fb[ks][j][p] = *reinterpret_cast<const ctts_u32x4*>(fr_b + p * X6_PLANE + 32 * j * X6_PROW + (ks ? fc1 : fc0));
    }
#pragma unroll
    for (int ks = 0; ks < 2; ++ks)
#pragma unroll
      for (int t = 0; t < 6; ++t) {
        constexpr int PA[6] = {2, 0, 1, 1, 0, 0}, PB[6] = {0, 2, 1, 0, 1, 0};
#pragma unroll
        for (int i = 0; i < MT; ++i)
#pragma unroll
          for (int j = 0; j < NT; ++j) acc[i][j] = x6_mma(fa[ks][i][PA[t]], fb[ks][j][PB[t]], acc[i][j]);
      }
    __syncthreads();
    lstore();
    __syncthreads();
    k_cur = k_nxt;
  }
  gemm_epilogue_auto<MT, NT>(d, acc, Cb, 0, row0, col0, wm0, wn0, l31, h, Mv, Nv);
}

template <bool A_KC, bool B_KC, bool CONV>
__global__ __launch_bounds__(256, CTTS_GEMM_WAVES) void gemm_buf_k2_kernel(const ctts_gemm_desc d) {
  constexpr int BM = 32, BN = 64;
  constexpr int A_LD = A_KC ? KC_LD : BM + 4;
  constexpr int B_LD = B_KC ? KC_LD : BN + 4;
  constexpr int A_SZ = A_KC ? BM * KC_LD : BK * (BM + 4);
  constexpr int B_SZ = B_KC ? BN * KC_LD : BK * (BN + 4);
  static_assert(BK == 32, "the two-group kernel stages two 32-deep K-blocks per round");
  __shared__ __attribute__((aligned(16))) float smem[2 * (A_SZ + B_SZ)];
  const int z = blockIdx.z, split = blockIdx.y;
  const int z0 = z / d.nb1, z1 = z - z0 * d.nb1;
  const int Mv = d.M, Nv = d.N, Kv = d.K;
  const int tiles_n = (d.N + BN - 1) / BN;
  const int tm = blockIdx.x / tiles_n;
  const int row0 = tm * BM, col0 = (blockIdx.x - tm * tiles_n) * BN;
  if (row0 >= Mv || col0 >= Nv) return;
  float* Cb = d.C + z0 * d.sC0 + z1 * d.sC1;
  if (d.split_k > 1) Cb += (long)split * d.M * d.ldc;
  if (A_KC && d.row_lens && padded_tile_zeroed(d, Cb, row0, col0, BM, min(BN, Nv - col0), Mv)) return;
  int k_begin, k_end;
  if (!split_k_range(d, Kv, 2 * BK, split, k_begin, k_end)) return;
  ConvView cv{d.conv_T, d.conv_pad, d.conv_cin};
  ConvView nocv{1, 0, 1};
  constexpr bool CONV_A = CONV && A_KC;
  constexpr bool CONV_B = CONV && !A_KC && !B_KC;
  using LA = Loader<Fetch::Buffer, A_KC, BM, CONV_A>;
  using LB = Loader<Fetch::Buffer, B_KC, BN, CONV_B>;
  LA la; LB lb;
  la.init(d.A + z0 * d.sA0 + z1 * d.sA1, d.lda, row0, Mv, CONV_A ? cv : nocv, threadIdx.x);
  lb.init(d.B + z0 * d.sB0 + z1 * d.sB1, d.ldb, col0, Nv, CONV_B ? cv : nocv, threadIdx.x);
  const int lane = threadIdx.x & 63, wave = threadIdx.x >> 6;
  const int l31 = lane & 31, h = lane >> 5;
  const int grp = wave >> 1, wn0 = (wave & 1) * 32;
  float* sA = smem + grp * (A_SZ + B_SZ);
  float* sB = sA + A_SZ;
  floatx16 acc[1][1];
#pragma unroll
  for (int r = 0; r < 16; ++r) acc[0][0][r] = 0.f;
  float4 ra[2][LA::NV], rb[2][LB::NV];
  auto load_round = [&](int k0) {
    la.load(k0, k_end, ra[0]);      lb.load(k0, k_end, rb[0]);
    la.load(k0 + BK, k_end, ra[1]); lb.load(k0 + BK, k_end, rb[1]);
  };
  auto store_round = [&]() {
    la.store(smem, ra[0]);                  lb.store(smem + A_SZ, rb[0]);
    la.store(smem + A_SZ + B_SZ, ra[1]);    lb.store(smem + 2 * A_SZ + B_SZ, rb[1]);
  };
  load_round(k_begin);
  store_round();
  __syncthreads();
  for (int k0 = k_begin; k0 < k_end; k0 += 2 * BK) {
    const bool has_next = (k0 + 2 * BK) < k_end;
    if (has_next) load_round(k0 + 2 * BK);
    {
      float fa[16], fb[16];
      fetch_frag<A_KC, A_LD>(sA, 0, l31, h, 0, fa);
      fetch_frag<B_KC, B_LD>(sB, wn0, l31, h, 0, fb);
#pragma unroll
      for (int kk = 0; kk < 16; ++kk) acc[0][0] = __builtin_amdgcn_mfma_f32_32x32x2f32(fa[kk], fb[kk], acc[0][0], 0, 0, 0);
    }
    __syncthreads();
    if (has_next) store_round();
    __syncthreads();
  }
  float* red = smem + (wave & 1) * 1024 + lane;
  if (grp == 1) {
#pragma unroll
    for (int r = 0; r < 16; ++r) red[r * 64] = acc[0][0][r];
  }
  __syncthreads();
  if (grp == 0) {
#pragma unroll
    for (int r = 0; r < 16; ++r) acc[0][0][r] += red[r * 64];
  }
  if (grp == 0) gemm_epilogue_auto<1, 1>(d, acc, Cb, z, row0, col0, 0, wn0, l31, h, Mv, Nv);
}

template <bool A_KC, bool B_KC, bool CONV>
int launch_buf_k2(const ctts_gemm_desc& d, hipStream_t st) {
  const int tiles = ((d.M + 31) / 32) * ((d.N + 63) / 64);
  const int nz = d.nb0 * d.nb1, ny = d.split_k > 1 ? d.split_k : 1;
  hipLaunchKernelGGL((gemm_buf_k2_kernel<A_KC, B_KC, CONV>), dim3(tiles, ny, nz), dim3(256), 0, st, d);
  CTTS_CHECK_LAUNCH("ctts_gemm(buf,k2)");
  return 0;
}

template <bool WITH_CONV, class F>
int for_layout(const ctts_gemm_desc& d, F f) {
  auto go = [&](auto a, auto b) {
    if constexpr (WITH_CONV) {
      if (d.conv_T > 0) return f(a, b, std::true_type{});
    }
    return f(a, b, std::false_type{});
  };
  if (d.a_kc && d.b_kc) return go(std::true_type{}, std::true_type{});
  if (d.a_kc && !d.b_kc) return go(std::true_type{}, std::false_type{});
  if (!d.a_kc && !d.b_kc) return go(std::false_type{}, std::false_type{});
  ctts_set_error("ctts_gemm: layout a_kc=0,b_kc=1 is not instantiated");
  return -1;
}

template <int BM, int BN, bool A_KC, bool B_KC, bool CONV, Fetch FETCH>
int launch_tile(const ctts_gemm_desc& d, hipStream_t st) {
  if constexpr (FETCH == Fetch::Buffer) {
    if (d.lens && (d.lim_m || d.lim_n || d.lim_k)) {
      if constexpr (!CONV) {
        return launch_tile<BM, BN, A_KC, B_KC, false, Fetch::BufferPartial>(d, st);
      } else {
        ctts_set_error("ctts_gemm: per-batch length limits together with a conv view are not supported");
        return -1;
      }
    }
  }
  const int tiles = ((d.M + BM - 1) / BM) * ((d.N + BN - 1) / BN);
  const int nz = d.nb0 * d.nb1, ny = d.split_k > 1 ? d.split_k : 1;
  hipLaunchKernelGGL((gemm_tile_kernel<BM, BN, A_KC, B_KC, CONV, FETCH>), dim3(tiles, ny, nz), dim3(256), 0, st, d);
  CTTS_CHECK_LAUNCH(FETCH == Fetch::BufferPartial ? "ctts_gemm(buf,partial)" : FETCH == Fetch::Buffer ? "ctts_gemm(buf)" : "ctts_gemm");
  return 0;
}

bool buf_ok(const ctts_gemm_desc& d) {
  if (d.lens && (d.lim_m || d.lim_n || d.lim_k) && d.conv_T > 0) return false;
  const long a_ext = d.a_kc ? ((long)d.M * d.lda + d.K) : ((long)d.K * d.lda + d.M);
  const long b_ext = d.b_kc ? ((long)d.N * d.ldb + d.K) : ((long)d.K * d.ldb + d.N);
  return a_ext * 4 < 0x7FFF0000L && b_ext * 4 < 0x7FFF0000L;
}

bool chunks_ok(const ctts_gemm_desc& d) {
  const bool a_ext = d.a_kc ? (d.K % 4 == 0) : (d.M % 4 == 0);
  const bool b_ext = d.b_kc ? (d.K % 4 == 0) : (d.N % 4 == 0);
  return a_ext && b_ext;
}
bool vec_ok(const ctts_gemm_desc& d) {
  auto al16 = [](const void* p) { return (reinterpret_cast<uintptr_t>(p) & 15) == 0; };
  const bool strides = !((d.lda | d.ldb | d.sA0 | d.sA1 | d.sB0 | d.sB1) & 3);
  return strides && chunks_ok(d) && al16(d.A) && al16(d.B);
}

__global__ __launch_bounds__(64) void row_tile_map_kernel(const int32_t* __restrict__ row_lens, int row_T, int row_halo, int M,
                                                            int32_t* __restrict__ map) {
  const int tiles = (M + 63) / 64, lane = threadIdx.x;
  auto inactive = [&](int tm) -> bool { return rows_in_padding(row_lens, row_T, row_halo, tm * 64, min(tm * 64 + 64, M) - 1); };
  int n_act = 0;
  for (int base = 0; base < tiles; base += 64) {
    const int tm = base + lane;
    const bool a = tm < tiles && !inactive(tm);
    const unsigned long long m = __ballot(a);
    if (a) map[1 + n_act + __popcll(m & ((1ULL << lane) - 1ULL))] = tm;
    n_act += __popcll(m);
  }
  int n_in = 0;
  for (int base = 0; base < tiles; base += 64) {
    const int tm = base + lane;
    const bool a = tm < tiles && inactive(tm);
    const unsigned long long m = __ballot(a);
    if (a) map[1 + n_act + n_in + __popcll(m & ((1ULL << lane) - 1ULL))] = tm;
    n_in += __popcll(m);
  }
  if (lane == 0) map[0] = n_act;
}

__global__ __launch_bounds__(256) void splitk_reduce_kernel(const ctts_gemm_desc d, int BM, int kround) {
  const int z = blockIdx.z, z0 = z / d.nb1, z1 = z - z0 * d.nb1;
  int Mv, Nv, Kv;
  batch_limits(d, z0, true, Mv, Nv, Kv);
  const bool ow = d.split_overwrite != 0;
  const int nact = Kv > 0 ? gemm_split_range(Kv, d.split_k, kround, 0).nonempty : 0;
  if (nact == 0 && !ow) return;
  const long ldp = gemm_partial_ld(d.N);
  const int n4 = (int)(ldp >> 2);
  const long e = (long)blockIdx.x * 256 + threadIdx.x;
  const int m = (int)(e / n4), n = (int)(e - (long)m * n4) * 4;
  if (m >= d.M || n >= d.N) return;
  bool live = m < Mv && n < Nv && nact > 0;
  if (live && d.a_kc && d.row_lens) {
    const int row0 = m / BM * BM;
    if (rows_in_padding(d.row_lens, d.row_T, d.row_halo, row0, min(row0 + BM, Mv) - 1)) live = false;
  }
  if (!live && !ow) return;
  float4 a = make_float4(0.f, 0.f, 0.f, 0.f);
  if (live) {
    const float4* P = reinterpret_cast<const float4*>(gemm_partial_base(d, z, 0) + (long)m * ldp + n);
    const long sstride = (long)d.M * ldp / 4;
    for (int s = 0; s < nact; s += 8) {
      float4 v[8];
#pragma unroll
      for (int u = 0; u < 8; ++u) v[u] = (s + u < nact) ? P[(long)(s + u) * sstride] : make_float4(0.f, 0.f, 0.f, 0.f);
#pragma unroll
      for (int u = 0; u < 8; ++u) { a.x += v[u].x; a.y += v[u].y; a.z += v[u].z; a.w += v[u].w; }
    }
  }
  float* Cr = d.C + z0 * d.sC0 + z1 * d.sC1 + (long)m * d.ldc + n;
  const float al = d.alpha;
  const int ncols = ow ? d.N : Nv;
  if (n + 4 <= Nv && ((reinterpret_cast<uintptr_t>(Cr) & 15) == 0)) {
    float4 c = ow ? make_float4(0.f, 0.f, 0.f, 0.f) : *reinterpret_cast<float4*>(Cr);
    c.x += al * a.x; c.y += al * a.y; c.z += al * a.z; c.w += al * a.w;
    *reinterpret_cast<float4*>(Cr) = c;
  } else {
    const float av[4] = {a.x, a.y, a.z, a.w};
#pragma unroll
    for (int q = 0; q < 4; ++q)
      if (n + q < ncols) Cr[q] = (ow ? 0.f : Cr[q]) + ((live && n + q < Nv) ? al * av[q] : 0.f);
  }
}

int splitk_reduce(const ctts_gemm_desc& d, int BM, int kround, hipStream_t st) {
  const long e = (long)d.M * (gemm_partial_ld(d.N) / 4);
  hipLaunchKernelGGL(splitk_reduce_kernel, dim3((unsigned)((e + 255) / 256), 1, d.nb0 * d.nb1), dim3(256), 0, st, d, BM, kround);
  CTTS_CHECK_LAUNCH("ctts_gemm(split-K reduce)");
  return 0;
}
}

extern "C" int ctts_row_tile_map(const int32_t* row_lens, int row_T, int row_halo, int M, int32_t* tile_map, void* stream) {
  CTTS_REQUIRE(row_lens && tile_map && row_T > 0 && M >= 0, "ctts_row_tile_map: bad arguments");
  hipLaunchKernelGGL(row_tile_map_kernel, dim3(1), dim3(64), 0, (hipStream_t)stream, row_lens, row_T, row_halo, M, tile_map);
  CTTS_CHECK_LAUNCH("ctts_row_tile_map");
  return 0;
}

static bool x6_plan(const ctts_gemm_desc& d) {
  const int on = d.bf16_split;
  static const long min_tiles = ctts_env_int("CTTS_X6_MIN_TILES", 384);
  if (on < 1 || !d.a_kc || !d.b_kc || d.nb0 * d.nb1 != 1 || d.split_k > 1 || d.E || d.lens || d.conv_on_b) return false;
  if (d.K < 256 || d.K % BK || d.N % 128 || d.M < 1024) return false;
  if (d.conv_T > 0 && d.conv_cin % 4) return false;
  if (on != 2 && on != 4 && (long)((d.M + 127) / 128) * (d.N / 128) < min_tiles) return false;
  return vec_ok(d) && buf_ok(d);
}

static bool x6tn_plan(const ctts_gemm_desc& d) {
  static const int tn = ctts_env_int("CTTS_X6_TN", 1);
  static const long min_wg = ctts_env_int("CTTS_X6_TN_MIN_WG", 384);
  if (d.bf16_split < 1 || !tn || d.a_kc || d.b_kc || d.nb0 * d.nb1 != 1 || d.E || d.lens || d.epi_bwd) return false;
  if (d.M % 128 || d.N % 128 || d.K % BK || d.K < 2048) return false;
  if (d.conv_T > 0 && (!d.conv_on_b || d.conv_T % 8 || d.conv_cin % 4)) return false;
  if (d.bf16_split != 2 && d.bf16_split != 4 && (long)(d.M / 128) * (d.N / 128) * (d.split_k > 1 ? d.split_k : 1) < min_wg) return false;
  return vec_ok(d) && buf_ok(d);
}

static int x6tn_launch(const ctts_gemm_desc& d, hipStream_t st) {
  const dim3 grid((d.M / 128) * (d.N / 128), d.split_k > 1 ? d.split_k : 1, 1);
  if (d.conv_T > 0) hipLaunchKernelGGL(gemm_x6tn_kernel<true>, grid, dim3(256), 0, st, d);
  else hipLaunchKernelGGL(gemm_x6tn_kernel<false>, grid, dim3(256), 0, st, d);
  CTTS_CHECK_LAUNCH("ctts_gemm(x6tn)");
  return 0;
}

static int x6_launch(const ctts_gemm_desc& d, hipStream_t st) {
  const int tiles = ((d.M + 127) / 128) * (d.N / 128);
  if (d.conv_T > 0) hipLaunchKernelGGL(gemm_x6_kernel<true>, dim3(tiles), dim3(256), 0, st, d);
  else hipLaunchKernelGGL(gemm_x6_kernel<false>, dim3(tiles), dim3(256), 0, st, d);
  CTTS_CHECK_LAUNCH("ctts_gemm(x6)");
  return 0;
}

struct GemmRoute {
  ctts_gemm_route_info info;
  bool split_fits;
  int tile_group_n;
  bool natural_order;
  union { PlArgs pl; PlwArgs plw; WsArgs ws; SkArgs sk; };
  GemmGrid grid;
};

static void tile_plan(const ctts_gemm_desc& d, bool x6tn, GemmRoute& r) {
  const long tiles128 = (long)((d.M + 127) / 128) * ((d.N + 127) / 128) * (d.split_k > 1 ? d.split_k : 1) * d.nb0 * d.nb1;
  static const int force_tile = ctts_env_int("CTTS_FORCE_TILE", 0);
  static const bool natural = getenv("CTTS_NATURAL_ORDER") != nullptr;
  static const int tile_group = ctts_env_int("CTTS_TILE_GROUP", -1);
  if (tile_group != 0 && d.tile_map && d.tile_map != reinterpret_cast<const int32_t*>(1)) {
    const int tn = (d.N + 63) / 64, tmn = (d.M + 63) / 64;
    const int g = tile_group > 0 ? tile_group : ((tn >= 8 && tn % 4 == 0) ? tn / 4 : 0);
    if (g > 0 && tn % g == 0) {
      const int ng = tn / g;
      if ((ng == 1 || ng == 2 || ng == 4 || ng == 8) && tmn % (8 / ng) == 0 && ((long)tmn * tn) % 8 == 0) r.tile_group_n = g;
    }
  }
  static const bool tn_natural = getenv("CTTS_TN_NATURAL") != nullptr;
  r.natural_order = (natural || (tn_natural && !d.a_kc && !d.b_kc)) && !d.tile_map;
  const bool aligned = vec_ok(d);
#ifdef CTTS_NO_BUF
  const bool buf_unaligned = false;
#else
  const bool buf_unaligned = !aligned && chunks_ok(d) && d.conv_T <= 0 && !(d.lens && (d.lim_m || d.lim_n || d.lim_k));
#endif
  r.info.tile_m = r.info.tile_n = 64;
  if (x6tn) { r.info.kind = CTTS_GEMM_X6TN; r.info.tile_m = r.info.tile_n = 128; }
  else if (!aligned && !(buf_unaligned && buf_ok(d))) r.info.kind = CTTS_GEMM_SCALAR64;
#ifndef CTTS_NO_BUF
  else if (buf_ok(d)) {
    static const int k2 = ctts_env_int("CTTS_K2_TILE", 640);
    static const int k2_mink = ctts_env_int("CTTS_K2_MIN_K", 256);
    static const int k2_tn = ctts_env_int("CTTS_K2_TN", 1);
    static const bool narrow = ctts_env_int("CTTS_NARROW_TILE", 1) != 0;
    if (force_tile == 128) { r.info.kind = CTTS_GEMM_BUF128; r.info.tile_m = r.info.tile_n = 128; }
    else if (k2 && (d.a_kc || (k2_tn && !d.b_kc)) && d.nb0 * d.nb1 == 1 && !d.lens && d.N >= 64 && d.M >= 256 && d.K >= k2_mink &&
             (long)((d.M + 63) / 64) * ((d.N + 63) / 64) * (d.split_k > 1 ? d.split_k : 1) <= k2) { r.info.kind = CTTS_GEMM_BUF_K2; r.info.tile_m = 32; }
    else if (narrow && d.N <= 32 && d.M >= 256 && d.conv_T <= 0 && !d.tile_map && !r.natural_order && !d.row_lens) { r.info.kind = CTTS_GEMM_BUF_NARROW; r.info.tile_m = 128; r.info.tile_n = 32; }
    else r.info.kind = CTTS_GEMM_BUF64;
  }
#endif
  else if (tiles128 >= 256 && d.N > 64 && (d.a_kc || d.b_kc)) { r.info.kind = CTTS_GEMM_VEC128; r.info.tile_m = r.info.tile_n = 128; }
  else r.info.kind = CTTS_GEMM_VEC64;
  r.info.k_granule = r.info.kind == CTTS_GEMM_BUF_K2 ? 2 * BK : BK;
}

static void gemm_route(const ctts_gemm_desc& d, GemmRoute& r, bool unbounded_room = false) {
  r.info = ctts_gemm_route_info{CTTS_GEMM_NONE, 128, 128, 1, 32};
  r.split_fits = true;
  r.tile_group_n = 0;
  r.natural_order = false;
  bool x6tn = false;
  if (ctts_gemm_pl_plan(d, r.pl, r.grid)) r.info.kind = CTTS_GEMM_PLANES;
  else if (ctts_gemm_plw_plan(d, r.plw, r.grid)) r.info.kind = CTTS_GEMM_PLANES_WGRAD;
  else if (ctts_gemm_ws_plan(d, r.ws, r.grid)) r.info.kind = CTTS_GEMM_WEIGHT_STATIONARY;
  else if (x6_plan(d)) { r.info.kind = CTTS_GEMM_X6; return; }
  else if (!(x6tn = x6tn_plan(d)) && ctts_gemm_sk_plan(d, r.sk, r.grid)) r.info.kind = CTTS_GEMM_STREAM_K;
  if (r.info.kind != CTTS_GEMM_NONE) { r.info.tile_m = r.grid.tile_m; r.info.tile_n = r.grid.tile_n; return; }
  tile_plan(d, x6tn, r);
  if (d.split_k > 1) {
    const long per_split = (long)d.nb0 * d.nb1 * d.M * gemm_partial_ld(d.N);
    const long room = unbounded_room ? (1L << 60) : (d.split_out ? d.split_out_floats : (long)CTTS_WS_SLAB_FLOATS);
    const long cap = per_split > 0 ? room / per_split : 0;
    r.split_fits = cap >= 2 && (long)d.M * gemm_partial_ld(d.N) * 4 < 0x7FFF0000L;
    r.info.split_k = d.split_k > cap ? (int)cap : d.split_k;
  }
}

static int gemm_validate(const ctts_gemm_desc* dp, ctts_gemm_desc& d) {
  CTTS_REQUIRE(dp != nullptr, "ctts_gemm: null descriptor");
  d = gemm_normalized(*dp);
  CTTS_REQUIRE(d.A && d.B && d.C, "ctts_gemm: null operand pointer");
  CTTS_REQUIRE(d.M >= 0 && d.N >= 0 && d.K >= 0, "ctts_gemm: negative dimension");
  if (d.M == 0 || d.N == 0) return 1;
  if (d.conv_T > 0) {
    CTTS_REQUIRE(d.conv_cin > 0 && (d.conv_cin % 4) == 0, "ctts_gemm: conv view needs cin %% 4 == 0 (got %d)", d.conv_cin);
    CTTS_REQUIRE(d.conv_on_b ? (!d.a_kc && !d.b_kc) : (d.a_kc != 0), "ctts_gemm: conv view on an unsupported operand layout");
  }
  CTTS_REQUIRE(d.p_drop >= 0.f && d.p_drop < 1.f, "ctts_gemm: p_drop out of range");
  CTTS_REQUIRE(!d.epi_bwd || (d.split_k <= 1 && !d.bias && !d.R && !d.rowscale && !d.E && (!d.act || d.Z)),
               "ctts_gemm: epi_bwd excludes bias, residual, rowscale, E and split-K, and needs Z when an activation is given");
  CTTS_REQUIRE(!d.E || (d.rowsub && d.split_k <= 1 && !d.bias && !d.act && d.p_drop == 0.f && !d.R && !d.rowscale && !d.Z),
               "ctts_gemm: the E/rowsub epilogue excludes bias, activation, dropout, residual, rowscale and split-K");
  return 0;
}

static int gemm_plan(const ctts_gemm_desc* dp, ctts_gemm_desc& d, GemmRoute& r) {
  const int rc = gemm_validate(dp, d);
  if (rc != 0) return rc;
  gemm_route(d, r);
  if (r.info.kind < CTTS_GEMM_X6TN || d.split_k <= 1) return 0;
  CTTS_REQUIRE(d.split_out || (d.sk_ws && d.sk_ws_bytes >= (int64_t)CTTS_WS_BYTES),
               "ctts_gemm: split_k > 1 needs the workspace (ctts_workspace_bytes() bytes, zero-filled once) in sk_ws - partial sums "
               "are added in a fixed order through it, the library has no floating-point atomics");
  CTTS_REQUIRE(r.split_fits, "ctts_gemm: split-K output [%d, %d] x %d batches does not fit the %s", d.M, d.N, d.nb0 * d.nb1,
               d.split_out ? "caller's split_out buffer" : "workspace");
  return 0;
}

extern "C" int ctts_gemm(const ctts_gemm_desc* dp, void* stream) {
  ctts_gemm_desc d;
  GemmRoute r;
  int rc = gemm_plan(dp, d, r);
  if (rc != 0) return rc < 0 ? rc : 0;
  hipStream_t st = reinterpret_cast<hipStream_t>(stream);
  const bool split = r.info.split_k > 1;
  ctts_gemm_desc t = d;
  t.tile_group_n = r.tile_group_n;
  if (r.natural_order) t.tile_map = reinterpret_cast<const int32_t*>(1);
  if (d.split_k > 1) t.split_k = r.info.split_k;
  const ctts_gemm_desc d_user = t;
  if (split) {
    const long ldp = gemm_partial_ld(d.N);
    t.C = d.split_out ? d.split_out : reinterpret_cast<float*>(reinterpret_cast<unsigned char*>(d.sk_ws) + CTTS_WS_SLABS);
    t.ldc = ldp;
    t.sC1 = (long)t.split_k * d.M * ldp;
    t.sC0 = (long)d.nb1 * t.sC1;
    t.alpha = 1.f; t.bias = nullptr; t.Z = nullptr; t.act = 0; t.p_drop = 0.f; t.R = nullptr; t.rowscale = nullptr;
  }
  switch (r.info.kind) {
    case CTTS_GEMM_PLANES: return ctts_gemm_pl_launch(d, r.pl, r.grid, st);
    case CTTS_GEMM_PLANES_WGRAD: return ctts_gemm_plw_launch(d, r.plw, r.grid, st);
    case CTTS_GEMM_WEIGHT_STATIONARY: return ctts_gemm_ws_launch(d, r.ws, r.grid, st);
    case CTTS_GEMM_X6: return x6_launch(d, st);
    case CTTS_GEMM_STREAM_K: return ctts_gemm_sk_launch(d, r.sk, r.grid, st);
    case CTTS_GEMM_SCALAR64: rc = for_layout<true>(t, [&](auto a, auto b, auto c) { return launch_tile<64, 64, a(), b(), c(), Fetch::Scalar>(t, st); }); break;
#ifndef CTTS_NO_BUF
    case CTTS_GEMM_BUF128: rc = for_layout<true>(t, [&](auto a, auto b, auto c) { return launch_tile<128, 128, a(), b(), c(), Fetch::Buffer>(t, st); }); break;
    case CTTS_GEMM_BUF_K2: rc = for_layout<true>(t, [&](auto a, auto b, auto c) { return launch_buf_k2<a(), b(), c()>(t, st); }); break;
    case CTTS_GEMM_BUF_NARROW: rc = for_layout<false>(t, [&](auto a, auto b, auto c) { return launch_tile<128, 32, a(), b(), c(), Fetch::Buffer>(t, st); }); break;
    case CTTS_GEMM_BUF64: rc = for_layout<true>(t, [&](auto a, auto b, auto c) { return launch_tile<64, 64, a(), b(), c(), Fetch::Buffer>(t, st); }); break;
#endif
    case CTTS_GEMM_VEC128: rc = for_layout<true>(t, [&](auto a, auto b, auto c) { return launch_tile<128, 128, a(), b(), c(), Fetch::Vec>(t, st); }); break;
    case CTTS_GEMM_X6TN: rc = x6tn_launch(t, st); break;
    default: rc = for_layout<true>(t, [&](auto a, auto b, auto c) { return launch_tile<64, 64, a(), b(), c(), Fetch::Vec>(t, st); }); break;
  }
  if (rc != 0 || !split || d.split_out) return rc;
  return splitk_reduce(d_user, r.info.tile_m, r.info.k_granule, st);
}

extern "C" int ctts_gemm_route(const ctts_gemm_desc* dp, ctts_gemm_route_info* info) {
  CTTS_REQUIRE(info != nullptr, "ctts_gemm_route: null info");
  *info = ctts_gemm_route_info{CTTS_GEMM_NONE, 0, 0, 0, 0};
  ctts_gemm_desc d;
  GemmRoute r;
  const int rc = gemm_plan(dp, d, r);
  if (rc == 0) *info = r.info;
  return rc < 0 ? rc : 0;
}

static int route_kind(const ctts_gemm_desc* dp) {
  if (!dp) return CTTS_GEMM_NONE;
  const ctts_gemm_desc d = gemm_normalized(*dp);
  GemmRoute r;
  gemm_route(d, r);
  return r.info.kind;
}
extern "C" int ctts_gemm_takes_planes(const ctts_gemm_desc* d) {
  const int kind = route_kind(d);
  return kind == CTTS_GEMM_PLANES || kind == CTTS_GEMM_PLANES_WGRAD;
}
extern "C" int ctts_gemm_takes_bf16_split(const ctts_gemm_desc* d) {
  const int kind = route_kind(d);
  return kind == CTTS_GEMM_X6 || kind == CTTS_GEMM_X6TN;
}

extern "C" int ctts_gemm_split_plan(const ctts_gemm_desc* dp, int32_t* count, int64_t* stride) {
  ctts_gemm_desc d;
  GemmRoute r;
  if (gemm_validate(dp, d) != 0 || d.split_k <= 1) return 0;
  d.split_out = nullptr;
  if (d.a_kc) d.A_planes = nullptr;
  gemm_route(d, r, true);
  if (r.info.kind < CTTS_GEMM_X6TN || !r.split_fits) return 0;
  if (d.nb0 * d.nb1 != 1 || d.lens || d.K <= 0 || (d.a_kc && d.row_lens)) return 0;
  if (count) *count = gemm_split_range(d.K, r.info.split_k, r.info.k_granule, 0).nonempty;
  if (stride) *stride = (long)d.M * gemm_partial_ld(d.N);
  return 1;
}
```

comprehensive-transformer-tts_amd/kernels.py:

```python
import collections
import ctypes as C

import torch

from . import _lib
from ._lib import GemmDesc

ACT_NONE, ACT_RELU, ACT_GELU, ACT_TANH, ACT_SWISH = 0, 1, 2, 3, 4


def _stream():
    return C.c_void_p(torch.cuda.current_stream().cuda_stream)


def _p(t, offset=0):
    if t is None:
        return None
    if not t.is_cuda:
        raise _lib.CttsError("ctts kernels need device (HIP) tensors; got a CPU tensor - no CPU fallback exists")
    return t.data_ptr() + offset * t.element_size()


def _f32c(t, name):
    if t.dtype != torch.float32 or not t.is_contiguous():
        raise _lib.CttsError(f"{name}: expected contiguous float32 tensor, got {t.dtype} contiguous={t.is_contiguous()}")
    return t


def _dp_rank():
    import os
    import torch.distributed as dist
    if dist.is_available() and dist.is_initialized():
        return dist.get_rank()
    return int(os.environ.get("RANK", "0"))


class DropCtx:

    def __init__(self, device, seed=None):
        if seed is None:
            seed = (torch.initial_seed() + 0x51ED27 * _dp_rank()) & 0x3FFFFFFFFFFF
        self.seed = torch.tensor([(int(seed) * 0x9E3779B1 + 0x7F4A7C15) & 0x7FFFFFFFFFFFFFFF], dtype=torch.int64, device=device)
        self.counter = 0

    def next_offset(self):
        self.counter = (self.counter + 1) & 0x7FFFFFFF
        return self.counter

    def begin_step(self):
        self.counter = 0

    def advance(self):
        self.seed.add_(0x632BE5AB)


import os as _os

SK_ENABLED = _os.environ.get("CTTS_SK", "1") != "0"
BF16_SPLIT = 0 if _os.environ.get("CTTS_X6", "1") == "0" else 1
PLW_ENABLED = _os.environ.get("CTTS_PLW", "1") != "0"
PLANES_ENABLED = _os.environ.get("CTTS_PL", "1") != "0"
PLANES_MIN_UNITS = int(_os.environ.get("CTTS_PL_MIN_UNITS", "4096"))
PLANES_MIN_TILES = int(_os.environ.get("CTTS_PL_MIN_TILES", "64"))
_SK_WS = {}


def gemm_workspace(device):
    key = (device.index if device.index is not None else torch.cuda.current_device(), torch.cuda.current_stream().cuda_stream)
    ws = _SK_WS.get(key)
    if ws is None:
        if SK_ENABLED and not torch.cuda.is_current_stream_capturing():
            check_xcd_dispatch(device)
        ws = torch.zeros(_lib.load().ctts_workspace_bytes(), dtype=torch.uint8, device=device)
        _SK_WS[key] = ws
    return ws


_XCD_OK = {}


def check_xcd_dispatch(device):
    global SK_ENABLED
    idx = device.index if device.index is not None else torch.cuda.current_device()
    if idx in _XCD_OK:
        return _XCD_OK[idx]
    out = torch.full((64,), -1, dtype=torch.int32, device=device)
    _lib.check(_lib.load().ctts_xcd_probe(_p(out), 64, _stream()), "ctts_xcd_probe")
    got = out.cpu().tolist()
    ok = got == [b % 8 for b in range(64)]
    _XCD_OK[idx] = ok
    if not ok:
        import warnings
        SK_ENABLED = False
        warnings.warn(f"ctts_amd: workgroups are not dispatched round-robin over 8 XCDs on cuda:{idx} (XCC_ID of workgroups 0..15: {got[:16]}) - "
                      "not the SPX partition mode; the persistent stream-K GEMM is disabled, the tile kernels take its launches")
    return ok


workspace = gemm_workspace


def _ws(t):
    return gemm_workspace(t.device).data_ptr()


class WorkspaceErrorProbe:

    def __init__(self):
        self._pending = []

    def poll(self):
        lib = _lib.load()
        self._pending = []
        for ws in list(_SK_WS.values()):
            off = lib.ctts_workspace_error_word(C.c_void_p(ws.data_ptr())) - ws.data_ptr()
            host = torch.empty(4, dtype=torch.uint8, pin_memory=True)
            with torch.cuda.device(ws.device):
                host.copy_(ws[off:off + 4], non_blocking=True)
                ev = torch.cuda.Event()
                ev.record()
            self._pending.append((ws, host, ev))

    def check(self):
        bad = []
        for ws, host, ev in self._pending:
            ev.synchronize()
            word = int(host.view(torch.int32)[0])
            if word != 0:
                bad.append((ws, word))
        self._pending = []
        for ws, word in bad:
            torch.cuda.synchronize(ws.device)
            ws.zero_()
        if bad:
            raise _lib.CttsError("stream-K GEMM hand-off failed: an owner workgroup gave up waiting for workgroup "
                                 f"{bad[0][1] - 1}'s partial tile - the results of that launch are invalid (workspace re-zeroed)")

    def poll_and_check(self):
        self.poll()
        self.check()


class PartialSink:

    FLUSH_BYTES = int(float(_os.environ.get("CTTS_DEFER_FLUSH_MB", "256")) * (1 << 20))

    def __init__(self):
        self.tasks = []
        self.keep = []
        self.pending = 0
        self.streams = []

    def add(self, src, count, stride, n, dst, alpha, src_off=0, dst_off=0):
        d0 = dst.data_ptr() + 4 * int(dst_off)
        if any(d0 < t[1] + 4 * t[2] and t[1] < d0 + 4 * int(n) for t in self.tasks):
            self.flush()
        self.tasks.append((src.data_ptr() + 4 * int(src_off), d0, int(n), int(stride), int(count), float(alpha)))
        self.keep.append((src, dst))
        if src.is_cuda:
            st = torch.cuda.current_stream(src.device)
            if st not in self.streams:
                self.streams.append(st)
        self.pending += 4 * int(count) * int(n)
        if self.FLUSH_BYTES and self.pending >= self.FLUSH_BYTES:
            self.flush()

    def flush(self):
        if not self.tasks:
            return
        arr = (_lib.PsumTask * len(self.tasks))()
        for t, (src, dst, n, stride, count, alpha) in zip(arr, self.tasks):
            t.src, t.dst, t.n, t.stride, t.count, t.alpha = src, dst, n, stride, count, alpha
        self.tasks = []
        self.pending = 0
        producers, self.streams = self.streams, []
        try:
            cur = torch.cuda.current_stream()
            for st in producers:
                if st != cur:
                    cur.wait_stream(st)
            _lib.check(_lib.load().ctts_partial_sums(arr, len(arr), _stream()), "ctts_partial_sums")
            for src, _ in self.keep:
                if src.is_cuda:
                    src.record_stream(cur)
        finally:
            self.keep = []


WEIGHTS_EPOCH = [0]

_SINK = None
DEFER_ENABLED = _os.environ.get("CTTS_DEFER_SUMS", "1") != "0"


def set_partial_sink(sink):
    global _SINK
    prev, _SINK = _SINK, (sink if DEFER_ENABLED else None)
    return prev


def _sink_for(dst):
    if _SINK is None or dst is None or not dst.is_contiguous():
        return None
    return _SINK


def _gemm_desc(A, B, Cout, M, N, K, lda, ldb, ldc, a_kc=True, b_kc=True, a_off=0, b_off=0, c_off=0, nb0=1, nb1=1,
               sA=(0, 0), sB=(0, 0), sC=(0, 0), lens=None, lim=(0, 0, 0), conv=None, conv_on_b=False, split_k=1, alpha=1.0,
               bias=None, Z=None, ldz=0, act=ACT_NONE, p_drop=0.0, seed=None, drop_offset=0, R=None, ldr=0, rowscale=None,
               row_lens=None, row_T=0, row_halo=0, tile_map=None, E=None, rowsub=None, use_sk=None, epi_bwd=False, split_overwrite=False,
               bf16_split=None, a_planes=None, b_planes=None, c_planes=None):
    d = GemmDesc()
    if c_planes is not None:
        d.C_planes = c_planes.data_ptr()
    d.bf16_split = int(BF16_SPLIT if bf16_split is None else bf16_split)
    if a_planes is not None and b_planes is not None:
        d.A_planes, d.B_planes = a_planes.data_ptr(), b_planes.data_ptr()
    d.A, d.B, d.C = _p(A, a_off), _p(B, b_off), _p(Cout, c_off)
    d.M, d.N, d.K = int(M), int(N), int(K)
    d.lda, d.ldb, d.ldc = int(lda), int(ldb), int(ldc)
    d.a_kc, d.b_kc = int(a_kc), int(b_kc)
    d.nb0, d.nb1 = int(nb0), int(nb1)
    d.sA0, d.sA1 = int(sA[0]), int(sA[1])
    d.sB0, d.sB1 = int(sB[0]), int(sB[1])
    d.sC0, d.sC1 = int(sC[0]), int(sC[1])
    d.lens = _p(lens)
    d.lim_m, d.lim_n, d.lim_k = int(lim[0]), int(lim[1]), int(lim[2])
    if conv is not None:
        d.conv_T, d.conv_pad, d.conv_cin = int(conv[0]), int(conv[1]), int(conv[2])
        d.conv_on_b = int(conv_on_b)
    d.split_k = int(split_k)
    d.alpha = float(alpha)
    d.bias = _p(bias)
    d.Z, d.ldz = _p(Z), int(ldz)
    d.act = int(act)
    d.p_drop = float(p_drop)
    d.seed = _p(seed)
    d.drop_offset = int(drop_offset)
    d.R, d.ldr = _p(R), int(ldr)
    d.rowscale = _p(rowscale)
    if row_lens is not None:
        d.row_lens, d.row_T, d.row_halo = _p(row_lens), int(row_T), int(row_halo)
        d.tile_map = _p(tile_map)
    d.E, d.rowsub = _p(E), _p(rowsub)
    d.epi_bwd = int(bool(epi_bwd))
    d.split_overwrite = int(bool(split_overwrite))
    if int(split_k) > 1 or a_planes is not None or ((SK_ENABLED if use_sk is None else use_sk) and nb0 * nb1 == 1 and M * N * K >= (1 << 24)):
        ws = gemm_workspace(A.device)
        d.sk_ws, d.sk_ws_bytes = ws.data_ptr(), ws.numel()
    return d


def gemm(A, B, Cout, M, N, K, lda, ldb, ldc, a_kc=True, b_kc=True, defer=False, **kw):
    d = _gemm_desc(A, B, Cout, M, N, K, lda, ldb, ldc, a_kc, b_kc, **kw)
    lib = _lib.load()
    if defer and _SINK is not None and d.split_k > 1 and d.nb0 * d.nb1 == 1 and ldc == N and N % 4 == 0:
        cnt, stride = C.c_int32(0), C.c_int64(0)
        if lib.ctts_gemm_split_plan(C.byref(d), C.byref(cnt), C.byref(stride)) == 1:
            P = torch.empty(d.split_k * stride.value, dtype=torch.float32, device=A.device)
            d.split_out, d.split_out_floats = P.data_ptr(), P.numel()
            _lib.check(lib.ctts_gemm(C.byref(d), _stream()), "ctts_gemm")
            _SINK.add(P, cnt.value, stride.value, M * N, Cout, d.alpha, dst_off=kw.get("c_off", 0))
            return Cout
    _lib.check(lib.ctts_gemm(C.byref(d), _stream()), "ctts_gemm")
    return Cout


def _matrix_view(t, name, nb):
    if t.dtype != torch.float32 or t.dim() < 2 or t.dim() - 2 > len(nb):
        raise _lib.CttsError(f"{name}: expected a float32 matrix view with at most {len(nb)} batch dimensions, got {t.dtype} {tuple(t.shape)}")
    (R, Cc), (sr, sc), lead = t.shape[-2:], t.stride()[-2:], t.shape[:-2]
    if sc == 1 or Cc == 1:
        row_major, ld = True, (sr if R > 1 else Cc)
    elif sr == 1 or R == 1:
        row_major, ld = False, sc
    else:
        raise _lib.CttsError(f"{name}: neither rows nor columns are contiguous (shape {tuple(t.shape)}, strides {t.stride()})")
    if any(n not in (1, want) for n, want in zip(lead, nb[len(nb) - len(lead):])):
        raise _lib.CttsError(f"{name}: batch sizes {tuple(lead)} neither equal nor broadcast to the output's {tuple(nb)}")
    strides = [0] * (len(nb) - len(lead)) + [s if n > 1 else 0 for n, s in zip(lead, t.stride())]
    return row_major, ld, tuple(strides + [0] * (2 - len(nb)))


def gemm_views(A, B, Cout, E=None, lens=None):
    nb = tuple(Cout.shape[:-2])
    if len(nb) > 2:
        raise _lib.CttsError(f"C: at most two batch dimensions, got shape {tuple(Cout.shape)}")
    (a_rm, lda, sA), (b_rm, ldb, sB), (c_rm, ldc, sC) = (_matrix_view(t, n, nb) for t, n in ((A, "A"), (B, "B"), (Cout, "C")))
    (M, Kd), N = A.shape[-2:], B.shape[-1]
    if B.shape[-2] != Kd or tuple(Cout.shape[-2:]) != (M, N):
        raise _lib.CttsError(f"inner extents disagree: A {tuple(A.shape)} @ B {tuple(B.shape)} -> C {tuple(Cout.shape)}")
    if not c_rm or (N > 1 and Cout.stride(-1) != 1):
        raise _lib.CttsError(f"C: the output needs unit column stride, got strides {Cout.stride()}")
    if E is not None and (E.shape != Cout.shape or _matrix_view(E, "E", nb) != (c_rm, ldc, sC)):
        raise _lib.CttsError(f"E: must be laid out exactly like C {tuple(Cout.shape)} {Cout.stride()}, got {tuple(E.shape)} {E.stride()}")
    nb0, nb1 = nb + (1,) * (2 - len(nb))
    if lens is not None and lens.numel() != nb0:
        raise _lib.CttsError(f"lens: {lens.numel()} lengths for nb0 = {nb0} batches")
    return (A, B, Cout, M, N, Kd, lda, ldb, ldc, a_rm, not b_rm), dict(nb0=nb0, nb1=nb1, sA=sA, sB=sB, sC=sC)


def bgemm(A, B, Cout, **kw):
    args, views = gemm_views(A, B, Cout, kw.get("E"), kw.get("lens"))
    return gemm(*args, **views, **kw)


GemmRoute =collections.namedtuple("GemmRoute", "kind tile_m tile_n split_k k_granule")


def gemm_route(A, B, Cout, M, N, K, lda, ldb, ldc, a_kc=True, b_kc=True, **kw):
    d, info = _gemm_desc(A, B, Cout, M, N, K, lda, ldb, ldc, a_kc, b_kc, **kw), _lib.GemmRouteInfo()
    _lib.check(_lib.load().ctts_gemm_route(C.byref(d), C.byref(info)), "ctts_gemm_route")
    return GemmRoute(_lib.GEMM_KINDS[info.kind], info.tile_m, info.tile_n, info.split_k, info.k_granule)


def _gemm_takes(what, args, kw):
    return bool(getattr(_lib.load(), "ctts_gemm_takes_" + what)(C.byref(_gemm_desc(*args, **kw))))


def gemm_takes_persistent(A, B, Cout, M, N, K, lda, ldb, ldc, a_kc=True, b_kc=True, **kw):
    return SK_ENABLED and _gemm_takes("persistent", (A, B, Cout, M, N, K, lda, ldb, ldc, a_kc, b_kc), kw)


def gemm_takes_bf16_split(A, B, Cout, M, N, K, lda, ldb, ldc, a_kc=True, b_kc=True, **kw):
    return _gemm_takes("bf16_split", (A, B, Cout, M, N, K, lda, ldb, ldc, a_kc, b_kc), kw)


def gemm_bf16_split_enable(on):
    global BF16_SPLIT
    prev = BF16_SPLIT
    BF16_SPLIT = 3 if on == "amp" else (int(on) if on in (2, 3, 4) else int(bool(on)))
    return prev


def amp_split():
    if BF16_SPLIT < 1:
        return None
    return 4 if BF16_SPLIT in (2, 4) else 3


def gemm_takes_planes(A, B, Cout, M, N, K, lda, ldb, ldc, a_kc=True, b_kc=True, **kw):
    return _gemm_takes("planes", (A, B, Cout, M, N, K, lda, ldb, ldc, a_kc, b_kc), kw)


def plane_shape_ok(M, N, K, conv_cin=None):
    if not PLANES_ENABLED or BF16_SPLIT < 1 or not SK_ENABLED:
        return False
    if K % 32 or K < 64 or N % 128 or N < 256 or M < 128:
        return False
    if conv_cin is not None and (conv_cin % 32 or K % conv_cin):
        return False
    tiles = -(-M // 128) * -(-N // 256)
    return BF16_SPLIT in (2, 4) or (tiles * (K // 32) >= PLANES_MIN_UNITS and tiles >= PLANES_MIN_TILES)


def plane_wgrad_shape_ok(Mo, No, Kred, cin=None):
    if not PLANES_ENABLED or not PLW_ENABLED or BF16_SPLIT < 1 or not SK_ENABLED:
        return False
    if Mo % 128 or No % 256 or Kred < 64:
        return False
    if cin is not None and (cin % 256 or No % cin):
        return False
    tiles = (Mo // 128) * (No // 256)
    return BF16_SPLIT in (2, 4) or (tiles >= 32 and tiles * (-(-Kred // 32)) >= PLANES_MIN_UNITS)


def split_planes(mats):
    if not mats:
        return []
    outs = []
    arr = (_lib.SplitTask * len(mats))()
    for t, m in zip(arr, mats):
        _f32c(m, "split_planes operand")
        rows, cols = m.shape
        if cols % 32:
            raise _lib.CttsError(f"split_planes: cols = {cols} is not a multiple of 32")
        o = torch.empty(rows, cols // 32, 3, 32, dtype=torch.bfloat16, device=m.device)
        outs.append(o)
        t.src, t.dst, t.rows, t.cols, t.ld = _p(m), o.data_ptr(), int(rows), int(cols), int(cols)
    _lib.check(_lib.load().ctts_split_planes(arr, len(arr), _stream()), "ctts_split_planes")
    return outs


PRODUCER_PLANES = _os.environ.get("CTTS_PRODUCER_PLANES", "1") != "0"


def _al16(*ts):
    return all(t.data_ptr() % 16 == 0 for t in ts)


def new_planes(rows, cols, device):
    return torch.empty(rows, cols // 32, 3, 32, dtype=torch.bfloat16, device=device)


def attach_planes(t, pl):
    t._ctts_planes = (pl, t.data_ptr(), t._version, t.numel())
    return t


def planes_of(t):
    ent = getattr(t, "_ctts_planes", None)
    if ent is None:
        return None
    pl, ptr, ver, n = ent
    if ptr != t.data_ptr() or ver != t._version or n != t.numel() or pl.numel() != 3 * n:
        return None
    return pl


def planes_piece(pl, q):
    return pl[:, :, q, :].reshape(pl.shape[0], -1)


def gemm_takes_weight_stationary(A, B, Cout, M, N, K, lda, ldb, ldc, a_kc=True, b_kc=True, **kw):
# ... 96 lines not shown
    rows = x.numel() // Cc
    y = torch.empty_like(x)
    mean = torch.empty(rows, dtype=torch.float32, device=x.device)
    rstd = torch.empty(rows, dtype=torch.float32, device=x.device)
    pl = new_planes(rows, Cc, x.device) if (want_planes and PRODUCER_PLANES and Cc % 32 == 0 and x.is_cuda) else None
    lib = _lib.load()
    _lib.check(lib.ctts_layernorm_fwd(_p(_f32c(x, "x")), _p(gamma), _p(beta), _p(y), _p(mean), _p(rstd), rows, Cc, eps,
                                      p_drop, _p(seed), drop_offset, _p(rowscale), _p(pl), _stream()), "ctts_layernorm_fwd")
    if pl is not None:
        attach_planes(y, pl)
    return y, mean, rstd


def layernorm_bwd(dy, x, gamma, mean, rstd, p_drop=0.0, seed=None, drop_offset=0, rowscale=None, acc_into=None, dres=None):
    Cc = x.shape[-1]
    rows = x.numel() // Cc
    dx = torch.empty_like(x)
    if acc_into is None:
        dgamma = torch.empty(Cc, dtype=torch.float32, device=x.device)
        dbeta = torch.empty(Cc, dtype=torch.float32, device=x.device)
    else:
        dgamma, dbeta = acc_into
    lib = _lib.load()
    sink = _sink_for(dgamma) if (acc_into is not None and dbeta.is_contiguous()) else None
    nparts = lib.ctts_reduce_parts(3, rows, Cc) if sink is not None else 0
    if nparts > 1:
        parts = torch.empty(nparts, 2 * Cc, dtype=torch.float32, device=x.device)
        _lib.check(lib.ctts_layernorm_bwd(_p(_f32c(dy, "dy")), _p(x), _p(gamma), _p(mean), _p(rstd), _p(dx), None, None, rows, Cc, p_drop,
                                          _p(seed), drop_offset, _p(rowscale), 1, _p(dres), None, _p(parts), _stream()), "ctts_layernorm_bwd")
        sink.add(parts, nparts, 2 * Cc, Cc, dgamma, 1.0)
        sink.add(parts, nparts, 2 * Cc, Cc, dbeta, 1.0, src_off=Cc)
        return dx, dgamma, dbeta
    _lib.check(lib.ctts_layernorm_bwd(_p(_f32c(dy, "dy")), _p(x), _p(gamma), _p(mean), _p(rstd), _p(dx), _p(dgamma),
                                      _p(dbeta), rows, Cc, p_drop, _p(seed), drop_offset, _p(rowscale), int(acc_into is not None),
                                      _p(dres), _ws(dy), None, _stream()), "ctts_layernorm_bwd")
    return dx, dgamma, dbeta


def colstats(x2d):
    rows, Cc = x2d.shape
    sums = torch.empty(2 * Cc, dtype=torch.float64, device=x2d.device)
    lib = _lib.load()
    _lib.check(lib.ctts_colstats(_p(_f32c(x2d, "x")), _p(sums), rows, Cc, _ws(x2d), _stream()), "ctts_colstats")
    return sums


def bn_batch_stats(x2d, eps, momentum, running_mean, running_var, num_batches):
    rows, Cc = x2d.shape
    sums = colstats(x2d)
    mean = torch.empty(Cc, dtype=torch.float32, device=x2d.device)
    rstd = torch.empty_like(mean)
    lib = _lib.load()
    _lib.check(lib.ctts_bn_finalize(_p(sums), rows, Cc, float(eps), float(momentum), _p(mean), _p(rstd), _p(running_mean),
                                    _p(running_var), _p(num_batches), _stream()), "ctts_bn_finalize")
    return mean, rstd


def bn_apply(x2d, mean, rstd, gamma, beta, act, p_drop=0.0, seed=None, drop_offset=0, want_planes=False):
    rows, Cc = x2d.shape
    y = torch.empty_like(x2d)
    pl = (new_planes(rows, Cc, x2d.device) if (want_planes and PRODUCER_PLANES and Cc % 32 == 0 and x2d.is_cuda and rows > 0
                                               and _al16(x2d, mean, rstd, gamma, beta)) else None)
    lib = _lib.load()
    _lib.check(lib.ctts_bn_apply(_p(_f32c(x2d, "x")), _p(mean), _p(rstd), _p(gamma), _p(beta), _p(y), rows, Cc, act, p_drop,
                                 _p(seed), drop_offset, _p(pl), _stream()), "ctts_bn_apply")
    return (y, pl) if want_planes else y


def bn_bwd(dy, x2d, mean, rstd, gamma, beta, act, p_drop, seed, drop_offset, batch_stats, acc_into=None, want_planes=False):
    rows, Cc = x2d.shape
    pl = (new_planes(rows, Cc, x2d.device) if (want_planes and PRODUCER_PLANES and Cc % 32 == 0 and x2d.is_cuda and rows > 0
                                               and _al16(dy, x2d, mean, rstd, gamma, beta)) else None)
    sums = torch.empty(2 * Cc, dtype=torch.float64, device=x2d.device)
    dx = torch.empty_like(x2d)
    if acc_into is not None:
        dgamma, dbeta = _f32c(acc_into[0], "dgamma"), _f32c(acc_into[1], "dbeta")
        batch_stats = int(batch_stats) | 2
    else:
        dgamma = torch.empty(Cc, dtype=torch.float32, device=x2d.device)
        dbeta = torch.empty(Cc, dtype=torch.float32, device=x2d.device)
    lib = _lib.load()
    _lib.check(lib.ctts_bn_bwd_reduce(_p(_f32c(dy, "dy")), _p(x2d), _p(mean), _p(rstd), _p(gamma), _p(beta), _p(sums), rows,
                                      Cc, act, p_drop, _p(seed), drop_offset, _ws(dy), _stream()), "ctts_bn_bwd_reduce")
    _lib.check(lib.ctts_bn_bwd_apply(_p(dy), _p(x2d), _p(mean), _p(rstd), _p(gamma), _p(beta), _p(sums), _p(dx), _p(dgamma),
                                     _p(dbeta), rows, Cc, act, p_drop, _p(seed), drop_offset, int(batch_stats), _p(pl), _stream()),
               "ctts_bn_bwd_apply")
    if pl is not None:
        attach_planes(dx, pl)
    return (dx, None, None) if acc_into is not None else (dx, dgamma, dbeta)


def softmax_fwd(S, lens, nb0, nb1, T):
    lib = _lib.load()
    _lib.check(lib.ctts_softmax_fwd(_p(S), _p(lens), nb0, nb1, T, T, _stream()), "ctts_softmax_fwd")
    return S


def softmax_bwd(P, dP, lens, nb0, nb1, T):
    lib = _lib.load()
    _lib.check(lib.ctts_softmax_bwd(_p(P), _p(dP), _p(lens), nb0, nb1, T, T, _stream()), "ctts_softmax_bwd")
    return dP


def act_dropout_bwd(dg, z, act, p_drop=0.0, seed=None, drop_offset=0):
    Cc = z.shape[-1]
    rows = z.numel() // Cc
    dz = torch.empty_like(z)
    lib = _lib.load()
    _lib.check(lib.ctts_act_dropout_bwd(_p(_f32c(dg, "dg")), _p(z), _p(dz), rows, Cc, act, 1.0, p_drop, _p(seed),
                                        drop_offset, _stream()), "ctts_act_dropout_bwd")
    return dz


def rowscale_dropout(x, rowscale=None, p_drop=0.0, seed=None, drop_offset=0):
    Cc = x.shape[-1]
    rows = x.numel() // Cc
    y = torch.empty_like(x)
    lib = _lib.load()
    _lib.check(lib.ctts_rowscale_dropout(_p(_f32c(x, "x")), _p(y), rows, Cc, _p(rowscale), p_drop, _p(seed), drop_offset,
                                         _stream()), "ctts_rowscale_dropout")
    return y


def posembed_fwd(x, pos, table, alpha=None, rowscale=None, p_drop=0.0, seed=None, drop_offset=0):
    Cc = x.shape[-1]
    rows = x.numel() // Cc
    y = torch.empty_like(x)
    _lib.check(_lib.load().ctts_posembed_fwd(_p(_f32c(x, "x")), _p(pos), _p(_f32c(table, "table")), _p(alpha), _p(rowscale), _p(y), rows, Cc,
                                             float(p_drop), _p(seed), int(drop_offset), _stream()), "ctts_posembed_fwd")
    return y


def posembed_bwd(dy, pos, table, rowscale=None, p_drop=0.0, seed=None, drop_offset=0, want_alpha=True, alpha_acc_into=None):
    Cc = dy.shape[-1]
    rows = dy.numel() // Cc
    dx = torch.empty_like(dy)
    dalpha = None
    if want_alpha:
        dalpha = alpha_acc_into if alpha_acc_into is not None else torch.empty(1, dtype=torch.float32, device=dy.device)
    _lib.check(_lib.load().ctts_posembed_bwd(_p(_f32c(dy, "dy")), _p(pos), _p(table), _p(rowscale), _p(dx), _p(dalpha), rows, Cc, float(p_drop),
                                             _p(seed), int(drop_offset), int(alpha_acc_into is not None), _ws(dy) if want_alpha else None,
                                             _stream()), "ctts_posembed_bwd")
    return dx, dalpha


def colsum(x2d, ld=None, scale=1.0, acc_into=None):
    rows, Cc = x2d.shape
    out = torch.empty(Cc, dtype=torch.float32, device=x2d.device) if acc_into is None else acc_into
    lib = _lib.load()
    sink = _sink_for(acc_into)
    nparts = lib.ctts_reduce_parts(0, rows, Cc) if sink is not None else 0
    if nparts > 1:
        parts = torch.empty(nparts, Cc, dtype=torch.float32, device=x2d.device)
        _lib.check(lib.ctts_colsum(_p(x2d), None, rows, Cc, ld if ld is not None else Cc, 1.0, 1, None, _p(parts), _stream()), "ctts_colsum")
        sink.add(parts, nparts, Cc, Cc, out, scale)
        return out
    ldv = ld if ld is not None else Cc
    CH = 65536
    for c0 in range(0, Cc, CH):
        _lib.check(lib.ctts_colsum(_p(x2d, c0), _p(out, c0), rows, min(CH, Cc - c0), ldv, float(scale), int(acc_into is not None),
                                   _ws(x2d), None, _stream()), "ctts_colsum")
    return out


def reflect_pad(y, pad):
    B, N = y.shape
    ld = (N + 2 * pad + 3) // 4 * 4
    out = torch.empty(B, ld, dtype=torch.float32, device=y.device)
    lib = _lib.load()
    _lib.check(lib.ctts_reflect_pad(_p(_f32c(y, "y")), _p(out), B, N, pad, ld, _stream()), "ctts_reflect_pad")
    return out


def stft_magnitude(reim, frames, nbins, ld_mag):
    mag = torch.empty(frames, ld_mag, dtype=torch.float32, device=reim.device)
    energy = torch.empty(frames, dtype=torch.float32, device=reim.device)
    lib = _lib.load()
    _lib.check(lib.ctts_stft_magnitude(_p(reim), reim.shape[-1], _p(mag), ld_mag, _p(energy), frames, nbins, _stream()),
               "ctts_stft_magnitude")
    return mag, energy


def log_clamp_transpose(mel_fm, B, F, n_mel, clip):
    out = torch.empty(B, n_mel, F, dtype=torch.float32, device=mel_fm.device)
    lib = _lib.load()
    _lib.check(lib.ctts_log_clamp_transpose(_p(mel_fm), _p(out), B, F, n_mel, clip, _stream()), "ctts_log_clamp_transpose")
    return out


def glu_fwd(a):
    C2 = a.shape[-1]
    rows = a.numel() // C2
    out = torch.empty(*a.shape[:-1], C2 // 2, dtype=torch.float32, device=a.device)
    lib = _lib.load()
    _lib.check(lib.ctts_glu_fwd(_p(_f32c(a, "a")), _p(out), rows, C2 // 2, _stream()), "ctts_glu_fwd")
    return out


def glu_bwd(a, dout):
    C2 = a.shape[-1]
    rows = a.numel() // C2
    da = torch.empty_like(a)
    lib = _lib.load()
    _lib.check(lib.ctts_glu_bwd(_p(a), _p(_f32c(dout, "dout")), _p(da), rows, C2 // 2, _stream()), "ctts_glu_bwd")
    return da


def dwconv_fwd(x, wT, flip=False):
    B, T, Cc = x.shape
    Kk = wT.shape[0]
    y = torch.empty_like(x)
    lib = _lib.load()
    _lib.check(lib.ctts_dwconv_fwd(_p(_f32c(x, "x")), _p(_f32c(wT, "wT")), _p(y), B, T, Cc, Kk, int(flip), _stream()),
               "ctts_dwconv_fwd")
    return y


def dwconv_wgrad(dy, x, Kk, acc_into=None):
    B, T, Cc = x.shape
    dw = _f32c(acc_into, "dw") if acc_into is not None else torch.empty(Cc, Kk, dtype=torch.float32, device=x.device)
    partials = torch.empty(128 * Cc * 32, dtype=torch.float32, device=x.device)
    lib = _lib.load()
    _lib.check(lib.ctts_dwconv_wgrad(_p(_f32c(dy, "dy")), _p(x), _p(dw), _p(partials), B, T, Cc, Kk, int(acc_into is not None), _stream()),
               "ctts_dwconv_wgrad")
    return None if acc_into is not None else dw


def relpos_softmax_fwd(S, PS, T, scale, p_drop=0.0, seed=None, drop_offset=0, want_dropped=True):
    nb = S.numel() // (T * T)
    Pd = torch.empty_like(S) if want_dropped else None
    lib = _lib.load()
    _lib.check(lib.ctts_relpos_softmax_fwd(_p(S), _p(PS), _p(Pd), nb, T, scale, p_drop, _p(seed), drop_offset, _stream()),
               "ctts_relpos_softmax_fwd")
    return Pd


def relpos_softmax_bwd(P, dPd, T, scale, p_drop=0.0, seed=None, drop_offset=0):
    nb = P.numel() // (T * T)
    lib = _lib.load()
    _lib.check(lib.ctts_relpos_softmax_bwd(_p(P), _p(dPd), nb, T, scale, p_drop, _p(seed), drop_offset, _stream()),
               "ctts_relpos_softmax_bwd")
    return dPd


def relshift_bwd(dS, T):
    nb = dS.numel() // (T * T)
    dPS = torch.empty_like(dS)
    lib = _lib.load()
    _lib.check(lib.ctts_relshift_bwd(_p(dS), _p(dPS), nb, T, _stream()), "ctts_relshift_bwd")
    return dPS


def neg_sqdist(q, k, temp):
    B, Tq, Cc = q.shape
    Tk = k.shape[1]
    out = torch.empty(B, Tq, Tk, dtype=torch.float32, device=q.device)
    lib = _lib.load()
    _lib.check(lib.ctts_neg_sqdist(_p(_f32c(q, "q")), _p(_f32c(k, "k")), _p(out), B, Tq, Tk, Cc, float(temp), _stream()),
               "ctts_neg_sqdist")
    return out


def mas(attn, in_lens, out_lens):
    B, Tq, Tk = attn.shape
    opt = torch.empty_like(attn)
    dur = torch.empty(B, Tk, dtype=torch.float32, device=attn.device)
    back = torch.empty(B, Tq, Tk, dtype=torch.uint8, device=attn.device)
    lib = _lib.load()
    in32 = in_lens.to(torch.int32).contiguous()
    out32 = out_lens.to(torch.int32).contiguous()
    _lib.check(lib.ctts_mas(_p(_f32c(attn, "attn")), _p(in32), _p(out32), _p(opt), _p(dur), _p(back), B, Tq, Tk, _stream()), "ctts_mas")
    return opt, dur


def im2col_3x3s2(x):
    B, T, W, Cc = x.shape
    Wo = (W - 1) // 2 + 1
    col = torch.empty(B * T * Wo, 9 * Cc, dtype=torch.float32, device=x.device)
    lib = _lib.load()
    _lib.check(lib.ctts_im2col_3x3s2(_p(_f32c(x, "x")), _p(col), B, T, W, Cc, _stream()), "ctts_im2col_3x3s2")
    return col


def col2im_3x3s2(dcol, B, T, W, Cc):
    dx = torch.empty(B, T, W, Cc, dtype=torch.float32, device=dcol.device)
    lib = _lib.load()
    _lib.check(lib.ctts_col2im_3x3s2(_p(_f32c(dcol, "dcol")), _p(dx), B, T, W, Cc, _stream()), "ctts_col2im_3x3s2")
    return dx


def gru_fwd(gi, whh, bhh, H, ndir, save_gates=True, rev_mask=None):
    B, T = gi.shape[0], gi.shape[1]
    out = torch.empty(B, T, ndir * H, dtype=torch.float32, device=gi.device)
    gates = torch.empty(B, T, ndir * 4 * H, dtype=torch.float32, device=gi.device) if save_gates else None
    rev_mask = (2 if ndir == 2 else 0) if rev_mask is None else int(rev_mask)
    lib = _lib.load()
    _lib.check(lib.ctts_gru_fwd(_p(_f32c(gi, "gi")), _p(_f32c(whh, "whh")), _p(_f32c(bhh, "bhh")), _p(out), _p(gates), B, T, H, ndir,
                                rev_mask, _stream()), "ctts_gru_fwd")
    return out, gates


def gru_bwd(dout, out, gates, whh, H, ndir, rev_mask=None):
    B, T = out.shape[0], out.shape[1]
    dgi = torch.empty(B, T, ndir * 3 * H, dtype=torch.float32, device=out.device)
    dgh = torch.empty_like(dgi)
    hprev = torch.empty_like(out)
    rev_mask = (2 if ndir == 2 else 0) if rev_mask is None else int(rev_mask)
# ... 1105 lines not shown
```

include/ctts.h:

```cpp
#ifndef CTTS_H
#define CTTS_H
#include <stddef.h>
#include <stdint.h>

#ifdef __cplusplus
extern "C" {
#endif

const char* ctts_last_error(void);
int ctts_version(void);

typedef struct ctts_gemm_desc {
  const float* A; const float* B; float* C;
  int32_t M, N, K;
  int64_t lda, ldb, ldc;
  int32_t a_kc, b_kc;
  int32_t nb0, nb1;
  int64_t sA0, sA1, sB0, sB1, sC0, sC1;
  const int32_t* lens;
  int32_t lim_m, lim_n, lim_k;
  int32_t conv_T, conv_pad, conv_cin, conv_on_b;
  int32_t split_k;
  float alpha;
  const float* bias;
  float* Z; int64_t ldz;
  int32_t act;
  float p_drop; const uint64_t* seed; uint32_t drop_offset;
  const float* R; int64_t ldr;
  const float* rowscale;
  const int32_t* row_lens; int32_t row_T; int32_t row_halo;
  const int32_t* tile_map;
  int32_t tile_group_n;
  const float* E; const float* rowsub;
  void* sk_ws; int64_t sk_ws_bytes;
  int32_t epi_bwd;
  float* split_out; int64_t split_out_floats;
  int32_t split_overwrite;
  int32_t bf16_split;
  const uint16_t* A_planes;
  const uint16_t* B_planes;
  uint16_t* C_planes;
} ctts_gemm_desc;

int ctts_gemm(const ctts_gemm_desc* d, void* stream);
int ctts_gemm_split_plan(const ctts_gemm_desc* d, int32_t* count, int64_t* stride);
typedef enum ctts_gemm_kind {
  CTTS_GEMM_NONE = 0,
  CTTS_GEMM_PLANES, CTTS_GEMM_PLANES_WGRAD,
  CTTS_GEMM_WEIGHT_STATIONARY,
  CTTS_GEMM_X6,
  CTTS_GEMM_STREAM_K,
  CTTS_GEMM_X6TN,
  CTTS_GEMM_SCALAR64, CTTS_GEMM_BUF128, CTTS_GEMM_BUF_K2, CTTS_GEMM_BUF_NARROW, CTTS_GEMM_BUF64, CTTS_GEMM_VEC128, CTTS_GEMM_VEC64
} ctts_gemm_kind;
typedef struct ctts_gemm_route_info { int32_t kind, tile_m, tile_n, split_k, k_granule; } ctts_gemm_route_info;
int ctts_gemm_route(const ctts_gemm_desc* d, ctts_gemm_route_info* info);
typedef struct ctts_repack_task { const float* src; float* dst; int32_t cout, cin, k; } ctts_repack_task;
int ctts_conv_dgrad_weights(const ctts_repack_task* tasks, int ntasks, void* stream);
int ctts_posembed_fwd(const float* x, const int32_t* pos, const float* table, const float* alpha, const float* rowscale, float* y,
                      int64_t rows, int C, float p_drop, const uint64_t* seed, uint32_t drop_offset, void* stream);
int ctts_posembed_bwd(const float* dy, const int32_t* pos, const float* table, const float* rowscale, float* dx, float* dalpha,
                      int64_t rows, int C, float p_drop, const uint64_t* seed, uint32_t drop_offset, int accumulate, void* ws, void* stream);
typedef struct ctts_psum_task { const float* src; float* dst; int64_t n; int64_t stride; int32_t count; float alpha; } ctts_psum_task;
int ctts_partial_sums(const ctts_psum_task* tasks, int ntasks, void* stream);
int ctts_reduce_parts(int kind, int64_t rows, int C);
size_t ctts_workspace_bytes(void);
size_t ctts_gemm_workspace_bytes(void);
const uint32_t* ctts_workspace_error_word(const void* ws);
int ctts_xcd_probe(int32_t* out, int nblocks, void* stream);
int ctts_gemm_takes_persistent(const ctts_gemm_desc* d);
int ctts_gemm_ws_enable(int on);
int ctts_gemm_takes_weight_stationary(const ctts_gemm_desc* d);
int ctts_gemm_takes_bf16_split(const ctts_gemm_desc* d);
int ctts_gemm_takes_planes(const ctts_gemm_desc* d);
typedef struct ctts_split_task { const float* src; uint16_t* dst; int64_t rows, cols, ld; } ctts_split_task;
int ctts_split_planes(const ctts_split_task* tasks, int ntasks, void* stream);

int ctts_rowdot_heads(const float* a, const float* b, float* out, int B, int T, int H, int dh, void* stream);

int ctts_weighted_colsum(const float* x, const float* w, float* out, int64_t rows, int C, float scale, int accumulate, void* ws, float* parts,
                         void* stream);

int ctts_epilogue_bwd(const float* dy, const float* rowscale, const float* z, float* dz, float* gm, float* dbias, int64_t rows, int C,
                      int act, float p_drop, const uint64_t* seed, uint32_t drop_offset, float bias_scale, int accumulate_bias,
                      void* ws, float* parts, void* stream);

int ctts_row_tile_map(const int32_t* row_lens, int row_T, int row_halo, int M, int32_t* tile_map, void* stream);

int ctts_conv_weight_repack(const float* src, float* dst, int cout, int cin, int k, int mode, void* stream);

int ctts_lr_index(const void* dur, int dur_is_float, int round_mode, const uint8_t* pad, int B, int Ts, int Tm,
                  int32_t* mel2ph, int64_t* mel_len, int32_t* cum, void* stream);
int ctts_lr_gather_fwd(const float* x, const int32_t* mel2ph, float* out, int B, int Ts, int Tm, int C, void* stream);
int ctts_lr_gather_bwd(const float* dy, const int32_t* cum, float* dx, int B, int Ts, int Tm, int C, void* stream);

int ctts_cwt_pitch(const float* spec, int64_t ld_spec, int nscale, const float* f0_mean, const float* f0_std, float std_scale,
                   const float* uv, int uv_chan, float eps, float mel_min, float mel_max, int f0_bin, float* f0, float* f0_denorm,
                   int64_t* ids, int B, int T, int width, void* stream);

int ctts_positions(const void* src, int src_is_float, int64_t stride, int B, int T, int32_t* pos, void* stream);

int ctts_layernorm_fwd(const float* x, const float* gamma, const float* beta, float* y, float* mean, float* rstd,
                       int rows, int C, float eps, float p_drop, const uint64_t* seed, uint32_t drop_offset,
                       const float* rowscale, uint16_t* planes, void* stream);
int ctts_layernorm_bwd(const float* dy, const float* x, const float* gamma, const float* mean, const float* rstd,
                       float* dx, float* dgamma, float* dbeta, int rows, int C, float p_drop, const uint64_t* seed,
                       uint32_t drop_offset, const float* rowscale, int accumulate, const float* dres, void* ws, float* parts,
                       void* stream);

int ctts_colstats(const float* x, double* sums, int rows, int C, void* ws, void* stream);
int ctts_bn_finalize(const double* sums, int rows, int C, float eps, float momentum, float* mean, float* rstd, float* running_mean,
                     float* running_var, int64_t* num_batches, void* stream);
int ctts_bn_apply(const float* x, const float* mean, const float* rstd, const float* gamma, const float* beta,
                  float* y, int rows, int C, int act, float p_drop, const uint64_t* seed, uint32_t drop_offset,
                  uint16_t* planes , void* stream);
int ctts_bn_bwd_reduce(const float* dy, const float* x, const float* mean, const float* rstd, const float* gamma,
                       const float* beta, double* sums, int rows, int C, int act, float p_drop, const uint64_t* seed,
                       uint32_t drop_offset, void* ws, void* stream);
int ctts_bn_bwd_apply(const float* dy, const float* x, const float* mean, const float* rstd, const float* gamma,
                      const float* beta, const double* sums, float* dx, float* dgamma, float* dbeta, int rows, int C,
                      int act, float p_drop, const uint64_t* seed, uint32_t drop_offset, int batch_stats,
                      uint16_t* planes , void* stream);

int ctts_softmax_fwd(float* S, const int32_t* lens, int nb0, int nb1, int T, int64_t ld, void* stream);
int ctts_softmax_bwd(const float* P, float* dP, const int32_t* lens, int nb0, int nb1, int T, int64_t ld,
                     void* stream);

int ctts_act_dropout_bwd(const float* dg, const float* z, float* dz, int64_t rows, int C, int act, float alpha_unused,
                         float p_drop, const uint64_t* seed, uint32_t drop_offset, void* stream);
int ctts_rowscale_dropout(const float* x, float* y, int64_t rows, int C, const float* rowscale, float p_drop,
                          const uint64_t* seed, uint32_t drop_offset, void* stream);
int ctts_colsum(const float* x, float* out, int64_t rows, int C, int64_t ld, float scale, int accumulate, void* ws, float* parts, void* stream);

int ctts_reflect_pad(const float* y, float* ypad, int B, int N, int pad, int64_t ld_out, void* stream);
int ctts_stft_magnitude(const float* reim, int64_t ld_reim, float* mag, int64_t ld_mag, float* energy, int64_t frames,
                        int nbins, void* stream);
int ctts_log_clamp_transpose(const float* mel_fm, float* out, int B, int F, int n_mel, float clip, void* stream);

int ctts_relattn_split_fwd(const float* qkv, const float* u_bias, const float* v_bias, float* qu, float* qv, float* kv, int64_t rows,
                           int C, void* stream);
int ctts_relattn_split_bwd(const float* dqu, const float* dqv, const float* dkv, float* dqkv, int64_t rows, int C, void* stream);
int ctts_glu_fwd(const float* a, float* out, int64_t rows, int C, void* stream);
int ctts_glu_bwd(const float* a, const float* dout, float* da, int64_t rows, int C, void* stream);
int ctts_dwconv_fwd(const float* x, const float* wT, float* y, int B, int T, int C, int K, int flip, void* stream);
int ctts_dwconv_wgrad(const float* dy, const float* x, float* dw, float* partials, int B, int T, int C, int K, int accumulate,
                      void* stream);
int ctts_relpos_softmax_fwd(float* S, const float* PS, float* Pd, int nbatch, int T, float scale, float p_drop,
                            const uint64_t* seed, uint32_t drop_offset, void* stream);
int ctts_relpos_softmax_bwd(const float* P, float* dPd, int nbatch, int T, float scale, float p_drop, const uint64_t* seed,
                            uint32_t drop_offset, void* stream);
int ctts_relshift_bwd(const float* dS, float* dPS, int nbatch, int T, void* stream);

int ctts_embedding_fwd(const int64_t* ids, const float* weight, float* out, int64_t n, int C, int V, void* stream);
int ctts_embedding_bwd(const int64_t* ids, const float* dy, float* dweight, int64_t n, int C, int V, int padding_idx, int accumulate,
                       void* ws, void* stream);

int ctts_neg_sqdist(const float* q, const float* k, float* out, int B, int Tq, int Tk, int C, float temp, void* stream);
int ctts_mas(const float* attn, const int32_t* in_lens, const int32_t* out_lens, float* opt, float* dur, uint8_t* back, int B,
             int Tq, int Tk, void* stream);
int ctts_forward_sum_fwd(const float* attn_logprob, const int32_t* in_lens, const int32_t* out_lens, float blank_logprob, float* lse,
                         float* alpha, float* nll, int B, int Tq, int Tk, void* stream);
int ctts_forward_sum_bwd(const float* attn_logprob, const int32_t* in_lens, const int32_t* out_lens, float blank_logprob,
                         const float* lse, const float* alpha, const float* nll, const float* gscale, float* grad, int B, int Tq,
                         int Tk, void* stream);

int ctts_im2col_3x3s2(const float* x, float* col, int B, int T, int W, int C, void* stream);
int ctts_col2im_3x3s2(const float* dcol, float* dx, int B, int T, int W, int C, void* stream);
int ctts_gru_fwd(const float* gi, const float* whh, const float* bhh, float* out, float* gates, int B, int T, int H, int ndir,
                 int rev_mask, void* stream);
int ctts_gru_bwd(const float* dout, const float* out, const float* gates, const float* whh, float* dgi, float* dgh, float* hprev,
                 int B, int T, int H, int ndir, int rev_mask, void* stream);
int ctts_softmax_rect_fwd(float* S, const int32_t* klens, const int32_t* qlens, int nb, int Tq, int Tk, void* stream);
int ctts_softmax_rect_bwd(const float* P, float* dP, const int32_t* klens, const int32_t* qlens, int nb, int Tq, int Tk,
                          void* stream);

size_t ctts_mel_spectrogram_workspace_bytes(int n_fft, int n_mel);
int ctts_mel_prepare(const float* mel_basis, int n_fft, int n_mel, float* workspace, void* stream);
int ctts_mel_spectrogram(const float* y, const int32_t* lens, const float* window, const float* workspace, float* mel, float* energy, float* mag,
                         int64_t ld_mag, int B, int N, int n_fft, int hop, int n_mel, float clip, int kmax, uint32_t* range_flag,
                         void* stream);

int ctts_mha_supported(int C, int H);
int ctts_mha_fwd(const float* qkv, const int32_t* lens, float* out, float* lse, int B, int T, int H, int C, float scale, void* stream);
int ctts_mha_bwd(const float* qkv, const int32_t* lens, const float* out, const float* dout, const float* lse, float* Dws, float* dS,
                 float* kv_part, float* dqkv, int B, int T, int H, int C, float scale, int q_split, void* ws, void* stream);
size_t ctts_relmha_workspace_floats(int B, int T, int H);
int ctts_relmha_fwd(const float* qu, const float* qv, const float* kv, const float* pos, float* out, float* lse, int B, int T,
                    int H, int C, float scale, float p_drop, const uint64_t* seed, uint32_t drop_offset, void* stream);
int ctts_relmha_bwd(const float* qu, const float* qv, const float* kv, const float* pos, const float* out,
                    const float* dout, const float* lse, float* Dws, float* dS, float* dqu, float* dqv, float* dkv,
                    float* dpos_b, int B, int T, int H, int C, float scale, float p_drop, const uint64_t* seed, uint32_t drop_offset,
                    void* stream);

int ctts_var_loss_fwd(const float* log_d, const void* dur, int dur_is_float, const int64_t* texts, const uint8_t* src_pad, const float* cwt,
                      const float* cwt_spec, const float* uv, const uint8_t* mel_pad, const float* f0m_p, const float* f0m_t,
                      const float* f0s_p, const float* f0s_t, const float* e_pred, const float* e_tgt, int B, int Ts, int Tm,
                      const float* lambdas5, int cwt_l2, const int64_t* sil_ids3, float* partials, float* wsum, float* terms, float* denoms,
                      void* stream);
int ctts_var_loss_bwd(const float* log_d, const void* dur, int dur_is_float, const int64_t* texts, const uint8_t* src_pad, const float* cwt,
                      const float* cwt_spec, const float* uv, const uint8_t* mel_pad, const float* f0m_p, const float* f0m_t,
                      const float* f0s_p, const float* f0s_t, const float* e_pred, const float* e_tgt, int B, int Ts, int Tm,
                      const float* lambdas5, int cwt_l2, const int64_t* sil_ids3, const float* partials, const float* wsum,
                      const float* denoms, const float* g8, float* d_log_d, float* d_cwt, float* d_f0m, float* d_f0s, float* d_e,
                      void* stream);
int ctts_bin_loss_fwd(const float* soft, const float* hard, int64_t n, float* partials, float* out2, void* stream);
int ctts_bin_loss_bwd(const float* soft, const float* hard, const float* out2, const float* g, float* dsoft, int64_t n, void* stream);
int ctts_masked_loss_fwd(const float* pred, const float* target, const float* weight, int64_t n, int kind, float* partials, float* out2,
                         void* stream);
int ctts_masked_loss_bwd(const float* pred, const float* target, const float* weight, const float* out2, const float* g, float* dpred,
                         int64_t n, int kind, void* stream);

#define CTTS_ADAM_PARTIALS 2048
#define CTTS_ADAM_STATE_FLOATS (3 + CTTS_ADAM_PARTIALS)
int ctts_adam_clip_step(float* p, const float* g, float* m, float* v, int64_t n, const float* lr, float beta1, float beta2, float eps,
                        float weight_decay, float max_norm, float* state, void* stream);

int ctts_mel_l1_fwd(const float* p1, const float* p2, const float* tgt, const uint8_t* pad, float* sums, float* roww, int64_t rows,
// ... 132 lines not shown
```

Before: 675,800 mel-frames/s.

## Defer underfilled split-K GEMMs and column sums into grouped batched launches

Adds grouped GEMM and batched column-sum kernels. Each packs several independent problems into one grid and finds its problem from a per-task block offset table held in the kernel arguments. Split-K weight-gradient GEMMs that would underfill the chip, and deferred column sums, are queued in the partial-sum sink and launched together at flush. The goal is to fill more CUs and cut per-launch overhead from many small backward kernels. In exchange, work is delayed until flush, with in-place write checks, a linear search per block, and possible interaction with the hipgraph capture.

```diff
diff --git a/comprehensive-transformer-tts_amd/_lib.py b/comprehensive-transformer-tts_amd/_lib.py
--- a/comprehensive-transformer-tts_amd/_lib.py
+++ b/comprehensive-transformer-tts_amd/_lib.py
@@ -86,6 +86,10 @@
     _fields_ = [("src", _vp), ("dst", _vp), ("n", _i64), ("stride", _i64), ("count", _i32), ("alpha", _f32)]
 
 
+class ColsumTask(C.Structure):
+    _fields_ = [("src", _vp), ("parts", _vp), ("rows", _i64), ("ld", _i64), ("C", _i32)]
+
+
 class SplitTask(C.Structure):
     _fields_ = [("src", _vp), ("dst", _vp), ("rows", _i64), ("cols", _i64), ("ld", _i64)]
 
@@ -104,6 +108,9 @@
     "ctts_posembed_fwd": [_vp, _vp, _vp, _vp, _vp, _vp, _i64, C.c_int, _f32, _vp, _u32, _vp],
     "ctts_posembed_bwd": [_vp, _vp, _vp, _vp, _vp, _vp, _i64, C.c_int, _f32, _vp, _u32, C.c_int, _vp, _vp],
     "ctts_gemm": [C.POINTER(GemmDesc), _vp],
+    "ctts_gemm_group": [C.POINTER(GemmDesc), C.c_int, _vp],
+    "ctts_gemm_group_max": [],
+    "ctts_colsum_batch": [C.POINTER(ColsumTask), C.c_int, _vp],
     "ctts_gemm_takes_persistent": [C.POINTER(GemmDesc)],
     "ctts_gemm_ws_enable": [C.c_int],
     "ctts_gemm_takes_weight_stationary": [C.POINTER(GemmDesc)],
diff --git a/comprehensive-transformer-tts_amd/csrc/elementwise.hip b/comprehensive-transformer-tts_amd/csrc/elementwise.hip
--- a/comprehensive-transformer-tts_amd/csrc/elementwise.hip
+++ b/comprehensive-transformer-tts_amd/csrc/elementwise.hip
@@ -90,28 +90,55 @@
   if (ty == 0 && c < C) out[c] = accumulate ? out[c] + scale * tot : scale * tot;
 }
 
+__device__ __forceinline__ float colsum_stripe(const float* __restrict__ x, long rows, int C, long ld, int bx, int by, int gy, float (*s)[64]) {
+  const int c = bx * 64 + (threadIdx.x & 63), ty = threadIdx.x >> 6;
+  const long stripe = (rows + gy - 1) / gy;
+  const long r0 = by * stripe, r1 = min(rows, r0 + stripe);
+  float a = 0.f;
+  if (c < C) {
+#pragma unroll 4
+    for (long r = r0 + ty; r < r1; r += 4) a += x[r * ld + c];
+  }
+  s[ty][threadIdx.x & 63] = a;
+  __syncthreads();
+  float tot = 0.f;
+  if (ty == 0) { const int l = threadIdx.x; tot = s[0][l] + s[1][l] + s[2][l] + s[3][l]; }
+  return tot;
+}
+
 __global__ __launch_bounds__(256) void colsum_kernel(const float* __restrict__ x, float* __restrict__ out, long rows, int C,
                                                       int creal, long ld, float scale, unsigned char* ws, int G, int accumulate,
                                                       float* __restrict__ parts) {
   __shared__ float s[4][64];
   const int c = blockIdx.x * 64 + (threadIdx.x & 63), ty = threadIdx.x >> 6;
-  const long stripe = (rows + gridDim.y - 1) / gridDim.y;
-  const long r0 = blockIdx.y * stripe, r1 = min(rows, r0 + stripe);
-  float a = 0.f;
-  if (c < C) {
-#pragma unroll 4
-    for (long r = r0 + ty; r < r1; r += 4) a += x[r * ld + c];
-  }
-  s[ty][threadIdx.x & 63] = a;
-  __syncthreads();
-  float tot[1] = {0.f};
-  if (ty == 0) { const int l = threadIdx.x; tot[0] = s[0][l] + s[1][l] + s[2][l] + s[3][l]; }
+  float tot[1] = {colsum_stripe(x, rows, C, ld, blockIdx.x, blockIdx.y, gridDim.y, s)};
   if (parts) {
     if (ty == 0 && c < C) parts[(long)blockIdx.y * C + c] = tot[0];
     return;
   }
   if (!ctts_ordered_colsum<float, 1>(tot, ws, blockIdx.x, blockIdx.y, gridDim.y, G)) return;
   ctts_colsum_emit(tot[0], s[0], out, c, C, creal, scale, accumulate);
+}
+
+constexpr int COLSUM_BATCH = 32;
+struct ColsumBatch {
+  const float* src[COLSUM_BATCH];
+  float* parts[COLSUM_BATCH];
+  long rows[COLSUM_BATCH], ld[COLSUM_BATCH];
+  int C[COLSUM_BATCH], gx[COLSUM_BATCH], gy[COLSUM_BATCH];
+  int first_block[COLSUM_BATCH + 1];
+  int ntasks;
+};
+static_assert(sizeof(ColsumBatch) <= 4096, "a batch must fit the 4 KiB kernel-argument segment");
+
+__global__ __launch_bounds__(256) void colsum_batch_kernel(const ColsumBatch b) {
+  __shared__ float s[4][64];
+  int t = 0;
+  while (t + 1 < b.ntasks && (int)blockIdx.x >= b.first_block[t + 1]) ++t;
+  const int l = blockIdx.x - b.first_block[t], gx = b.gx[t], by = l / gx, bx = l - by * gx, C = b.C[t];
+  const float tot = colsum_stripe(b.src[t], b.rows[t], C, b.ld[t], bx, by, b.gy[t], s);
+  const int c = bx * 64 + (threadIdx.x & 63);
+  if ((threadIdx.x >> 6) == 0 && c < C) b.parts[t][(long)by * C + c] = tot;
 }
 
 __global__ __launch_bounds__(256) void epilogue_bwd_kernel(const float* __restrict__ dy, const float* __restrict__ rowscale,
@@ -334,6 +361,32 @@
   return 0;
 }
 
+extern "C" int ctts_colsum_batch(const ctts_colsum_task* tasks, int ntasks, void* stream) {
+  CTTS_REQUIRE(ntasks >= 0 && (tasks || ntasks == 0), "ctts_colsum_batch: bad arguments");
+  hipStream_t st = (hipStream_t)stream;
+  for (int t0 = 0; t0 < ntasks; t0 += COLSUM_BATCH) {
+    ColsumBatch b;
+    b.ntasks = 0;
+    int blocks = 0;
+    for (int t = t0; t < ntasks && t < t0 + COLSUM_BATCH; ++t) {
+      const ctts_colsum_task& k = tasks[t];
+      CTTS_REQUIRE(k.src && k.parts && k.rows > 0 && k.C > 0 && k.ld >= k.C, "ctts_colsum_batch: bad task %d", t);
+      const int gy = ctts_reduce_parts(0, k.rows, k.C);
+      CTTS_REQUIRE(gy > 0, "ctts_colsum_batch: task %d: this shape has no deferred mode (ctts_reduce_parts = 0)", t);
+      const int i = b.ntasks++;
+      b.src[i] = k.src; b.parts[i] = k.parts; b.rows[i] = k.rows; b.ld[i] = k.ld; b.C[i] = k.C;
+      b.gx[i] = (k.C + 63) / 64; b.gy[i] = gy;
+      b.first_block[i] = blocks;
+      blocks += b.gx[i] * gy;
+    }
+    if (b.ntasks == 0) continue;
+    b.first_block[b.ntasks] = blocks;
+    hipLaunchKernelGGL(colsum_batch_kernel, dim3(blocks), dim3(256), 0, st, b);
+    CTTS_CHECK_LAUNCH("ctts_colsum_batch");
+  }
+  return 0;
+}
+
 extern "C" int ctts_epilogue_bwd(const float* dy, const float* rowscale, const float* z, float* dz, float* gm, float* dbias,
                                  int64_t rows, int C, int act, float p_drop, const uint64_t* seed, uint32_t drop_offset, float bias_scale,
                                  int accumulate_bias, void* ws, float* parts, void* stream) {
diff --git a/comprehensive-transformer-tts_amd/csrc/gemm.hip b/comprehensive-transformer-tts_amd/csrc/gemm.hip
--- a/comprehensive-transformer-tts_amd/csrc/gemm.hip
+++ b/comprehensive-transformer-tts_amd/csrc/gemm.hip
@@ -2,6 +2,7 @@
 #include "gemm_common.h"
 #include <stdlib.h>
 #include <type_traits>
+#include <vector>
 
 namespace {
 
@@ -42,8 +43,8 @@
   return true;
 }
 
-__device__ __forceinline__ void xcd_tile_order(int nwg, int tiles_n, bool scramble, int& wg, int& tm) {
-  const int q8 = nwg >> 3, r8 = nwg & 7, xcd = blockIdx.x & 7, slot = blockIdx.x >> 3;
+__device__ __forceinline__ void xcd_tile_order(int bx, int nwg, int tiles_n, bool scramble, int& wg, int& tm) {
+  const int q8 = nwg >> 3, r8 = nwg & 7, xcd = bx & 7, slot = bx >> 3;
   wg = (xcd < r8 ? xcd * (q8 + 1) : r8 * (q8 + 1) + (xcd - r8) * q8) + slot;
   const int tiles_m = nwg / tiles_n;
   tm = wg / tiles_n;
@@ -412,7 +413,7 @@
 }
 
 template <int BM, int BN, bool A_KC, bool B_KC, bool CONV, Fetch FETCH>
-__global__ __launch_bounds__(256, CTTS_GEMM_WAVES) void gemm_tile_kernel(const ctts_gemm_desc d) {
+__device__ __forceinline__ void gemm_tile_body(const ctts_gemm_desc& d, const int bx, const int split, const int z, const int nwg) {
   using FT = FetchTraits<FETCH>;
   constexpr int WAVES_N = BN >= 64 ? 2 : 1, WAVES_M = 4 / WAVES_N;
   constexpr int WM = BM / WAVES_M, WN = BN / WAVES_N, MT = WM / 32, NT = WN / 32;
@@ -423,8 +424,6 @@
   __shared__ __attribute__((aligned(16))) float smem[A_SZ + B_SZ];
   float* sA = smem;
   float* sB = smem + A_SZ;
-  const int z = blockIdx.z;
-  const int split = blockIdx.y;
   const int z0 = z / d.nb1, z1 = z - z0 * d.nb1;
   const bool limited = FT::kLensLimits && (FT::kLensGiven || d.lens);
   int Mv, Nv, Kv;
@@ -433,21 +432,21 @@
   int wg, tm;
   bool scheduled_active = false;
   if (FT::kTileOrders && BM == 64 && A_KC && d.tile_map && !natural_order(d)) {
-    wg = blockIdx.x;
+    wg = bx;
     int r = wg / tiles_n;
     if (d.tile_group_n > 0) {
       const int g = d.tile_group_n, ngroups = tiles_n / g, mways = 8 / ngroups;
-      const int x = blockIdx.x & 7, i = blockIdx.x >> 3;
+      const int x = bx & 7, i = bx >> 3;
       r = (i / g) * mways + x / ngroups;
       wg = r * tiles_n + (x % ngroups) * g + i % g;
     }
     tm = d.tile_map[1 + r];
     scheduled_active = FT::kTrustSchedule && r < d.tile_map[0];
   } else if (FT::kNaturalOrder || (FT::kTileOrders && natural_order(d))) {
-    wg = blockIdx.x;
+    wg = bx;
     tm = wg / tiles_n;
   } else {
-    xcd_tile_order(gridDim.x, tiles_n, true, wg, tm);
+    xcd_tile_order(bx, nwg, tiles_n, true, wg, tm);
   }
   const int row0 = tm * BM, col0 = (wg % tiles_n) * BN;
   float* Cb = d.C + z0 * d.sC0 + z1 * d.sC1;
@@ -541,6 +540,38 @@
   gemm_epilogue_auto<MT, NT>(d, acc, Cs, z, row0, col0, wm0, wn0, l31, h, Mv, Nv);
 }
 
+template <int BM, int BN, bool A_KC, bool B_KC, bool CONV, Fetch FETCH>
+__global__ __launch_bounds__(256, CTTS_GEMM_WAVES) void gemm_tile_kernel(const ctts_gemm_desc d) {
+  gemm_tile_body<BM, BN, A_KC, B_KC, CONV, FETCH>(d, blockIdx.x, blockIdx.y, blockIdx.z, gridDim.x);
+}
+
+constexpr int GEMM_GROUP_MAX = (4096 - 2 * (int)sizeof(int)) / ((int)sizeof(ctts_gemm_desc) + 3 * (int)sizeof(int));
+struct GemmGroup {
+  ctts_gemm_desc d[GEMM_GROUP_MAX];
+  int first[GEMM_GROUP_MAX + 1];
+  int tiles[GEMM_GROUP_MAX], ny[GEMM_GROUP_MAX];
+  int n;
+};
+static_assert(sizeof(GemmGroup) <= 4096, "a group must fit the 4 KiB kernel-argument segment");
+static_assert(GEMM_GROUP_MAX >= 2, "ctts_gemm_desc has outgrown the grouped launch");
+
+__device__ __forceinline__ int group_locate(const GemmGroup& g, int& bx, int& split, int& z) {
+  int p = 0;
+  while (p + 1 < g.n && (int)blockIdx.x >= g.first[p + 1]) ++p;
+  const int l = blockIdx.x - g.first[p], tiles = g.tiles[p], r = l / tiles;
+  bx = l - r * tiles;
+  z = r / g.ny[p];
+  split = r - z * g.ny[p];
+  return p;
+}
+
+template <int BM, int BN, bool A_KC, bool B_KC, bool CONV, Fetch FETCH>
+__global__ __launch_bounds__(256, CTTS_GEMM_WAVES) void gemm_tile_group_kernel(const GemmGroup g) {
+  int bx, split, z;
+  const int p = group_locate(g, bx, split, z);
+  gemm_tile_body<BM, BN, A_KC, B_KC, CONV, FETCH>(g.d[p], bx, split, z, g.tiles[p]);
+}
+
 constexpr int X6_PROW = 64, X6_PLANE = 128 * X6_PROW;
 __device__ __forceinline__ int x6_chunk(int row, int c) { return c ^ ((row >> 2) & 3); }
 typedef __bf16 x6_bf16x8 __attribute__((ext_vector_type(8)));
@@ -581,7 +612,7 @@
   if (natural_order(d)) {
     wg = blockIdx.x; tm = wg / tiles_n;
   } else {
-    xcd_tile_order(gridDim.x, tiles_n, true, wg, tm);
+    xcd_tile_order(blockIdx.x, gridDim.x, tiles_n, true, wg, tm);
   }
   const int row0 = tm * BM, col0 = (wg % tiles_n) * BN;
   float* Cb = d.C;
@@ -668,7 +699,7 @@
   const int Mv = d.M, Nv = d.N, Kv = d.K;
   const int tiles_n = d.N / BN, split = blockIdx.y;
   int wg, tm;
-  xcd_tile_order(gridDim.x, tiles_n, false, wg, tm);
+  xcd_tile_order(blockIdx.x, gridDim.x, tiles_n, false, wg, tm);
   const int row0 = tm * BM, col0 = (wg % tiles_n) * BN;
   float* Cb = d.C;
   if (d.split_k > 1) Cb += (long)split * d.M * d.ldc;
@@ -779,7 +810,7 @@
 }
 
 template <bool A_KC, bool B_KC, bool CONV>
-__global__ __launch_bounds__(256, CTTS_GEMM_WAVES) void gemm_buf_k2_kernel(const ctts_gemm_desc d) {
+__device__ __forceinline__ void gemm_buf_k2_body(const ctts_gemm_desc& d, const int bx, const int split, const int z) {
   constexpr int BM = 32, BN = 64;
   constexpr int A_LD = A_KC ? KC_LD : BM + 4;
   constexpr int B_LD = B_KC ? KC_LD : BN + 4;
@@ -787,12 +818,11 @@
   constexpr int B_SZ = B_KC ? BN * KC_LD : BK * (BN + 4);
   static_assert(BK == 32, "the two-group kernel stages two 32-deep K-blocks per round");
   __shared__ __attribute__((aligned(16))) float smem[2 * (A_SZ + B_SZ)];
-  const int z = blockIdx.z, split = blockIdx.y;
   const int z0 = z / d.nb1, z1 = z - z0 * d.nb1;
   const int Mv = d.M, Nv = d.N, Kv = d.K;
   const int tiles_n = (d.N + BN - 1) / BN;
-  const int tm = blockIdx.x / tiles_n;
-  const int row0 = tm * BM, col0 = (blockIdx.x - tm * tiles_n) * BN;
+  const int tm = bx / tiles_n;
+  const int row0 = tm * BM, col0 = (bx - tm * tiles_n) * BN;
   if (row0 >= Mv || col0 >= Nv) return;
   float* Cb = d.C + z0 * d.sC0 + z1 * d.sC1;
   if (d.split_k > 1) Cb += (long)split * d.M * d.ldc;
@@ -856,13 +886,51 @@
 }
 
 template <bool A_KC, bool B_KC, bool CONV>
-int launch_buf_k2(const ctts_gemm_desc& d, hipStream_t st) {
+__global__ __launch_bounds__(256, CTTS_GEMM_WAVES) void gemm_buf_k2_kernel(const ctts_gemm_desc d) {
+  gemm_buf_k2_body<A_KC, B_KC, CONV>(d, blockIdx.x, blockIdx.y, blockIdx.z);
+}
+
+template <bool A_KC, bool B_KC, bool CONV>
+__global__ __launch_bounds__(256, CTTS_GEMM_WAVES) void gemm_buf_k2_group_kernel(const GemmGroup g) {
+  int bx, split, z;
+  const int p = group_locate(g, bx, split, z);
+  gemm_buf_k2_body<A_KC, B_KC, CONV>(g.d[p], bx, split, z);
+}
+
+template <class L>
+int launch_group(const ctts_gemm_desc* const* ds, int n, int BM, int BN, L launch) {
+  GemmGroup g;
+  long wgs = 0;
+  for (int i = 0; i < n; ++i) {
+    const ctts_gemm_desc& d = *ds[i];
+    g.d[i] = d;
+    g.first[i] = (int)wgs;
+    g.tiles[i] = ((d.M + BM - 1) / BM) * ((d.N + BN - 1) / BN);
+    g.ny[i] = d.split_k > 1 ? d.split_k : 1;
+    wgs += (long)g.tiles[i] * g.ny[i] * d.nb0 * d.nb1;
+  }
+  CTTS_REQUIRE(wgs < (1L << 31), "ctts_gemm_group: too many workgroups in one grouped launch");
+  g.first[n] = (int)wgs;
+  g.n = n;
+  launch(g, dim3((unsigned)wgs));
+  CTTS_CHECK_LAUNCH("ctts_gemm_group");
+  return 0;
+}
+
+template <bool A_KC, bool B_KC, bool CONV>
+int launch_buf_k2(const ctts_gemm_desc* const* ds, int n, hipStream_t st) {
+  if (n > 1)
+    return launch_group(ds, n, 32, 64, [&](const GemmGroup& g, dim3 grid) {
+      hipLaunchKernelGGL((gemm_buf_k2_group_kernel<A_KC, B_KC, CONV>), grid, dim3(256), 0, st, g); });
+  const ctts_gemm_desc& d = *ds[0];
   const int tiles = ((d.M + 31) / 32) * ((d.N + 63) / 64);
   const int nz = d.nb0 * d.nb1, ny = d.split_k > 1 ? d.split_k : 1;
   hipLaunchKernelGGL((gemm_buf_k2_kernel<A_KC, B_KC, CONV>), dim3(tiles, ny, nz), dim3(256), 0, st, d);
   CTTS_CHECK_LAUNCH("ctts_gemm(buf,k2)");
   return 0;
 }
+
+bool lens_limited(const ctts_gemm_desc& d) { return d.lens && (d.lim_m || d.lim_n || d.lim_k); }
 
 template <bool WITH_CONV, class F>
 int for_layout(const ctts_gemm_desc& d, F f) {
@@ -880,17 +948,21 @@
 }
 
 template <int BM, int BN, bool A_KC, bool B_KC, bool CONV, Fetch FETCH>
-int launch_tile(const ctts_gemm_desc& d, hipStream_t st) {
+int launch_tile(const ctts_gemm_desc* const* ds, int n, hipStream_t st) {
+  const ctts_gemm_desc& d = *ds[0];
   if constexpr (FETCH == Fetch::Buffer) {
-    if (d.lens && (d.lim_m || d.lim_n || d.lim_k)) {
+    if (lens_limited(d)) {
       if constexpr (!CONV) {
-        return launch_tile<BM, BN, A_KC, B_KC, false, Fetch::BufferPartial>(d, st);
+        return launch_tile<BM, BN, A_KC, B_KC, false, Fetch::BufferPartial>(ds, n, st);
       } else {
         ctts_set_error("ctts_gemm: per-batch length limits together with a conv view are not supported");
         return -1;
       }
     }
   }
+  if (n > 1)
+    return launch_group(ds, n, BM, BN, [&](const GemmGroup& g, dim3 grid) {
+      hipLaunchKernelGGL((gemm_tile_group_kernel<BM, BN, A_KC, B_KC, CONV, FETCH>), grid, dim3(256), 0, st, g); });
   const int tiles = ((d.M + BM - 1) / BM) * ((d.N + BN - 1) / BN);
   const int nz = d.nb0 * d.nb1, ny = d.split_k > 1 ? d.split_k : 1;
   hipLaunchKernelGGL((gemm_tile_kernel<BM, BN, A_KC, B_KC, CONV, FETCH>), dim3(tiles, ny, nz), dim3(256), 0, st, d);
@@ -1139,19 +1211,25 @@
   return 0;
 }
 
-extern "C" int ctts_gemm(const ctts_gemm_desc* dp, void* stream) {
-  ctts_gemm_desc d;
+struct GemmLaunch {
+  ctts_gemm_desc d, t, d_user;
   GemmRoute r;
-  int rc = gemm_plan(dp, d, r);
-  if (rc != 0) return rc < 0 ? rc : 0;
-  hipStream_t st = reinterpret_cast<hipStream_t>(stream);
-  const bool split = r.info.split_k > 1;
-  ctts_gemm_desc t = d;
+  bool split;
+};
+
+static int gemm_prepare(const ctts_gemm_desc* dp, GemmLaunch& L) {
+  const int rc = gemm_plan(dp, L.d, L.r);
+  if (rc != 0) return rc;
+  const ctts_gemm_desc& d = L.d;
+  const GemmRoute& r = L.r;
+  L.split = r.info.split_k > 1;
+  ctts_gemm_desc& t = L.t;
+  t = d;
   t.tile_group_n = r.tile_group_n;
   if (r.natural_order) t.tile_map = reinterpret_cast<const int32_t*>(1);
   if (d.split_k > 1) t.split_k = r.info.split_k;
-  const ctts_gemm_desc d_user = t;
-  if (split) {
+  L.d_user = t;
+  if (L.split) {
     const long ldp = gemm_partial_ld(d.N);
     t.C = d.split_out ? d.split_out : reinterpret_cast<float*>(reinterpret_cast<unsigned char*>(d.sk_ws) + CTTS_WS_SLABS);
     t.ldc = ldp;
@@ -1159,26 +1237,86 @@
     t.sC0 = (long)d.nb1 * t.sC1;
     t.alpha = 1.f; t.bias = nullptr; t.Z = nullptr; t.act = 0; t.p_drop = 0.f; t.R = nullptr; t.rowscale = nullptr;
   }
+  return 0;
+}
+
+static int tile_instance(const GemmLaunch& L) {
+  const int kind = L.r.info.kind;
+  if (kind <= CTTS_GEMM_X6TN) return 0;
+  const ctts_gemm_desc& t = L.t;
+  const bool conv = t.conv_T > 0 && kind != CTTS_GEMM_BUF_NARROW;
+  return (kind << 4) | (t.a_kc ? 8 : 0) | (t.b_kc ? 4 : 0) | (conv ? 2 : 0) | (lens_limited(t) ? 1 : 0);
+}
+
+static int tile_launch(int kind, const ctts_gemm_desc* const* ts, int n, hipStream_t st) {
+  const ctts_gemm_desc& t = *ts[0];
+  switch (kind) {
+    case CTTS_GEMM_SCALAR64: return for_layout<true>(t, [&](auto a, auto b, auto c) { return launch_tile<64, 64, a(), b(), c(), Fetch::Scalar>(ts, n, st); });
+#ifndef CTTS_NO_BUF
+    case CTTS_GEMM_BUF128: return for_layout<true>(t, [&](auto a, auto b, auto c) { return launch_tile<128, 128, a(), b(), c(), Fetch::Buffer>(ts, n, st); });
+    case CTTS_GEMM_BUF_K2: return for_layout<true>(t, [&](auto a, auto b, auto c) { return launch_buf_k2<a(), b(), c()>(ts, n, st); });
+    case CTTS_GEMM_BUF_NARROW: return for_layout<false>(t, [&](auto a, auto b, auto c) { return launch_tile<128, 32, a(), b(), c(), Fetch::Buffer>(ts, n, st); });
+    case CTTS_GEMM_BUF64: return for_layout<true>(t, [&](auto a, auto b, auto c) { return launch_tile<64, 64, a(), b(), c(), Fetch::Buffer>(ts, n, st); });
+#endif
+    case CTTS_GEMM_VEC128: return for_layout<true>(t, [&](auto a, auto b, auto c) { return launch_tile<128, 128, a(), b(), c(), Fetch::Vec>(ts, n, st); });
+    default: return for_layout<true>(t, [&](auto a, auto b, auto c) { return launch_tile<64, 64, a(), b(), c(), Fetch::Vec>(ts, n, st); });
+  }
+}
+
+static int gemm_launch_one(const GemmLaunch& L, hipStream_t st) {
+  const ctts_gemm_desc& d = L.d;
+  const GemmRoute& r = L.r;
+  int rc;
   switch (r.info.kind) {
     case CTTS_GEMM_PLANES: return ctts_gemm_pl_launch(d, r.pl, r.grid, st);
     case CTTS_GEMM_PLANES_WGRAD: return ctts_gemm_plw_launch(d, r.plw, r.grid, st);
     case CTTS_GEMM_WEIGHT_STATIONARY: return ctts_gemm_ws_launch(d, r.ws, r.grid, st);
     case CTTS_GEMM_X6: return x6_launch(d, st);
     case CTTS_GEMM_STREAM_K: return ctts_gemm_sk_launch(d, r.sk, r.grid, st);
-    case CTTS_GEMM_SCALAR64: rc = for_layout<true>(t, [&](auto a, auto b, auto c) { return launch_tile<64, 64, a(), b(), c(), Fetch::Scalar>(t, st); }); break;
-#ifndef CTTS_NO_BUF
-    case CTTS_GEMM_BUF128: rc = for_layout<true>(t, [&](auto a, auto b, auto c) { return launch_tile<128, 128, a(), b(), c(), Fetch::Buffer>(t, st); }); break;
-    case CTTS_GEMM_BUF_K2: rc = for_layout<true>(t, [&](auto a, auto b, auto c) { return launch_buf_k2<a(), b(), c()>(t, st); }); break;
-    case CTTS_GEMM_BUF_NARROW: rc = for_layout<false>(t, [&](auto a, auto b, auto c) { return launch_tile<128, 32, a(), b(), c(), Fetch::Buffer>(t, st); }); break;
-    case CTTS_GEMM_BUF64: rc = for_layout<true>(t, [&](auto a, auto b, auto c) { return launch_tile<64, 64, a(), b(), c(), Fetch::Buffer>(t, st); }); break;
-#endif
-    case CTTS_GEMM_VEC128: rc = for_layout<true>(t, [&](auto a, auto b, auto c) { return launch_tile<128, 128, a(), b(), c(), Fetch::Vec>(t, st); }); break;
-    case CTTS_GEMM_X6TN: rc = x6tn_launch(t, st); break;
-    default: rc = for_layout<true>(t, [&](auto a, auto b, auto c) { return launch_tile<64, 64, a(), b(), c(), Fetch::Vec>(t, st); }); break;
-  }
-  if (rc != 0 || !split || d.split_out) return rc;
-  return splitk_reduce(d_user, r.info.tile_m, r.info.k_granule, st);
-}
+    case CTTS_GEMM_X6TN: rc = x6tn_launch(L.t, st); break;
+    default: { const ctts_gemm_desc* one = &L.t; rc = tile_launch(r.info.kind, &one, 1, st); } break;
+  }
+  if (rc != 0 || !L.split || d.split_out) return rc;
+  return splitk_reduce(L.d_user, r.info.tile_m, r.info.k_granule, st);
+}
+
+extern "C" int ctts_gemm(const ctts_gemm_desc* dp, void* stream) {
+  GemmLaunch L;
+  const int rc = gemm_prepare(dp, L);
+  if (rc != 0) return rc < 0 ? rc : 0;
+  return gemm_launch_one(L, reinterpret_cast<hipStream_t>(stream));
+}
+
+extern "C" int ctts_gemm_group(const ctts_gemm_desc* descs, int n, void* stream) {
+  CTTS_REQUIRE(n >= 0 && (descs || n == 0), "ctts_gemm_group: bad arguments");
+  hipStream_t st = reinterpret_cast<hipStream_t>(stream);
+  std::vector<GemmLaunch> Ls;
+  Ls.reserve(n);
+  for (int i = 0; i < n; ++i) {
+    GemmLaunch L;
+    const int rc = gemm_prepare(descs + i, L);
+    if (rc < 0) return rc;
+    if (rc == 0) Ls.push_back(L);
+  }
+  struct Run { int key; std::vector<const ctts_gemm_desc*> ts; const GemmLaunch* first; };
+  std::vector<Run> runs;
+  for (const GemmLaunch& L : Ls) {
+    const int key = (L.split && !L.d.split_out) ? 0 : tile_instance(L);
+    Run* run = nullptr;
+    if (key != 0)
+      for (Run& q : runs)
+        if (q.key == key && (int)q.ts.size() < GEMM_GROUP_MAX) { run = &q; break; }
+    if (!run) { runs.push_back(Run{key, {}, &L}); run = &runs.back(); }
+    run->ts.push_back(&L.t);
+  }
+  for (const Run& q : runs) {
+    const int rc = q.ts.size() == 1 ? gemm_launch_one(*q.first, st) : tile_launch(q.first->r.info.kind, q.ts.data(), (int)q.ts.size(), st);
+    if (rc != 0) return rc;
+  }
+  return 0;
+}
+
+extern "C" int ctts_gemm_group_max(void) { return GEMM_GROUP_MAX; }
 
 extern "C" int ctts_gemm_route(const ctts_gemm_desc* dp, ctts_gemm_route_info* info) {
   CTTS_REQUIRE(info != nullptr, "ctts_gemm_route: null info");
diff --git a/comprehensive-transformer-tts_amd/kernels.py b/comprehensive-transformer-tts_amd/kernels.py
--- a/comprehensive-transformer-tts_amd/kernels.py
+++ b/comprehensive-transformer-tts_amd/kernels.py
@@ -150,6 +150,22 @@
         self.keep = []
         self.pending = 0
         self.streams = []
+        self.gemms = []
+        self.colsums = []
+        self.operands = []
+
+    def _hold(self, tensors):
+        for t in tensors:
+            if isinstance(t, torch.Tensor):
+                self.operands.append((t, t._version))
+
+    def add_gemm(self, d, tensors):
+        self.gemms.append(d)
+        self._hold(tensors)
+
+    def add_colsum(self, x2d, parts, rows, Cc, ld):
+        self.colsums.append((x2d.data_ptr(), parts.data_ptr(), int(rows), int(ld), int(Cc)))
+        self._hold((x2d, parts))
 
     def add(self, src, count, stride, n, dst, alpha, src_off=0, dst_off=0):
         d0 = dst.data_ptr() + 4 * int(dst_off)
@@ -166,23 +182,39 @@
             self.flush()
 
     def flush(self):
-        if not self.tasks:
+        if not (self.tasks or self.gemms or self.colsums):
             return
         arr = (_lib.PsumTask * len(self.tasks))()
         for t, (src, dst, n, stride, count, alpha) in zip(arr, self.tasks):
             t.src, t.dst, t.n, t.stride, t.count, t.alpha = src, dst, n, stride, count, alpha
-        self.tasks = []
+        garr = (GemmDesc * len(self.gemms))(*self.gemms)
+        carr = (_lib.ColsumTask * len(self.colsums))(*self.colsums)
+        operands = self.operands
+        self.tasks, self.gemms, self.colsums, self.operands = [], [], [], []
         self.pending = 0
         producers, self.streams = self.streams, []
         try:
+            for t, version in operands:
+                if t._version != version:
+                    raise _lib.CttsError("PartialSink: an operand of a deferred launch was written in place between its call site and "
+                                         f"the flush (shape {tuple(t.shape)}) - launch that GEMM / column sum immediately instead")
             cur = torch.cuda.current_stream()
             for st in producers:
                 if st != cur:
                     cur.wait_stream(st)
-            _lib.check(_lib.load().ctts_partial_sums(arr, len(arr), _stream()), "ctts_partial_sums")
+            lib = _lib.load()
+            if len(garr):
+                _lib.check(lib.ctts_gemm_group(garr, len(garr), _stream()), "ctts_gemm_group")
+            if len(carr):
+                _lib.check(lib.ctts_colsum_batch(carr, len(carr), _stream()), "ctts_colsum_batch")
+            if len(arr):
+                _lib.check(lib.ctts_partial_sums(arr, len(arr), _stream()), "ctts_partial_sums")
             for src, _ in self.keep:
                 if src.is_cuda:
                     src.record_stream(cur)
+            for t, _ in operands:
+                if t.is_cuda:
+                    t.record_stream(cur)
         finally:
             self.keep = []
 
@@ -191,6 +223,17 @@
 
 _SINK = None
 DEFER_ENABLED = _os.environ.get("CTTS_DEFER_SUMS", "1") != "0"
+GROUP_LAUNCHES = _os.environ.get("CTTS_GROUP_LAUNCHES", "1") != "0"
+CHIP_CUS = 256
+_FIRST_TILE_KIND = _lib.GEMM_KINDS.index("scalar64")
+
+
+def launch_underfills(info, M, N, batches=1):
+    if info.kind < _FIRST_TILE_KIND:
+        return False
+    resident = 2 if info.tile_m * info.tile_n >= 128 * 128 else 6
+    tiles = -(-M // info.tile_m) * -(-N // info.tile_n)
+    return tiles * max(1, info.split_k) * batches < CHIP_CUS * resident
 
 
 def set_partial_sink(sink):
@@ -259,7 +302,13 @@
         if lib.ctts_gemm_split_plan(C.byref(d), C.byref(cnt), C.byref(stride)) == 1:
             P = torch.empty(d.split_k * stride.value, dtype=torch.float32, device=A.device)
             d.split_out, d.split_out_floats = P.data_ptr(), P.numel()
-            _lib.check(lib.ctts_gemm(C.byref(d), _stream()), "ctts_gemm")
+            info = _lib.GemmRouteInfo()
+            if GROUP_LAUNCHES:
+                _lib.check(lib.ctts_gemm_route(C.byref(d), C.byref(info)), "ctts_gemm_route")
+            if launch_underfills(info, d.M, d.N):
+                _SINK.add_gemm(d, (A, B, P, gemm_workspace(A.device)) + tuple(kw.values()))
+            else:
+                _lib.check(lib.ctts_gemm(C.byref(d), _stream()), "ctts_gemm")
             _SINK.add(P, cnt.value, stride.value, M * N, Cout, d.alpha, dst_off=kw.get("c_off", 0))
             return Cout
     _lib.check(lib.ctts_gemm(C.byref(d), _stream()), "ctts_gemm")
@@ -662,7 +711,10 @@
     nparts = lib.ctts_reduce_parts(0, rows, Cc) if sink is not None else 0
     if nparts > 1:
         parts = torch.empty(nparts, Cc, dtype=torch.float32, device=x2d.device)
-        _lib.check(lib.ctts_colsum(_p(x2d), None, rows, Cc, ld if ld is not None else Cc, 1.0, 1, None, _p(parts), _stream()), "ctts_colsum")
+        if GROUP_LAUNCHES:
+            sink.add_colsum(x2d, parts, rows, Cc, ld if ld is not None else Cc)
+        else:
+            _lib.check(lib.ctts_colsum(_p(x2d), None, rows, Cc, ld if ld is not None else Cc, 1.0, 1, None, _p(parts), _stream()), "ctts_colsum")
         sink.add(parts, nparts, Cc, Cc, out, scale)
         return out
     ldv = ld if ld is not None else Cc
diff --git a/include/ctts.h b/include/ctts.h
--- a/include/ctts.h
+++ b/include/ctts.h
@@ -43,6 +43,8 @@
 } ctts_gemm_desc;
 
 int ctts_gemm(const ctts_gemm_desc* d, void* stream);
+int ctts_gemm_group(const ctts_gemm_desc* descs, int n, void* stream);
+int ctts_gemm_group_max(void);
 int ctts_gemm_split_plan(const ctts_gemm_desc* d, int32_t* count, int64_t* stride);
 typedef enum ctts_gemm_kind {
   CTTS_GEMM_NONE = 0,
@@ -63,6 +65,8 @@
                       int64_t rows, int C, float p_drop, const uint64_t* seed, uint32_t drop_offset, int accumulate, void* ws, void* stream);
 typedef struct ctts_psum_task { const float* src; float* dst; int64_t n; int64_t stride; int32_t count; float alpha; } ctts_psum_task;
 int ctts_partial_sums(const ctts_psum_task* tasks, int ntasks, void* stream);
+typedef struct ctts_colsum_task { const float* src; float* parts; int64_t rows; int64_t ld; int32_t C; } ctts_colsum_task;
+int ctts_colsum_batch(const ctts_colsum_task* tasks, int ntasks, void* stream);
 int ctts_reduce_parts(int kind, int64_t rows, int C);
 size_t ctts_workspace_bytes(void);
 size_t ctts_gemm_workspace_bytes(void);
```

New measurement: 679,000 mel-frames/s (median of 6 runs). About the same (+0.5%).
